# AdamBeedell/MLX8-WS-Audio-Transformer

Measured on AMD Instinct MI355X. Metric: 4s@16kHz clips/sec through mel+Whisper-small encoder, higher is better.
Workload: dtype fp16; 1 GPU; int16 PCM [B,64000] in HBM -> Whisper log-mel [B,80,3000] -> Whisper-small encoder -> hidden [B,1500,768] fp32; mode=parity (clip zero-padded to 30 s, as the reference computes), precision=f16f8, fp16_exact_projection_matrices=0 of 48 (found by the library at upload), parallelism=dp1 (clip shards, no data-path collective)

## Files before the change

### include/awt.h

```cpp
#ifndef AWT_H_
#define AWT_H_

#include <stddef.h>
#include <stdint.h>

#ifdef __cplusplus
extern "C" {
#endif

typedef enum awt_status {
  AWT_OK = 0,
  AWT_ERR_INVALID = -1,
  AWT_ERR_HIP = -2,
  AWT_ERR_WORKSPACE = -3,
  AWT_ERR_STATE = -4,
  AWT_ERR_VALUE = -5
} awt_status;

typedef struct awt_ctx awt_ctx;
typedef struct awt_encoder awt_encoder;

const char* awt_last_error(void);
const char* awt_version(void);

int awt_ctx_create(int device, awt_ctx** out);
void awt_ctx_destroy(awt_ctx* c);

size_t awt_logmel_workspace_bytes(int B);
int awt_logmel_whisper(awt_ctx* c, const void* pcm, int pcm_is_i16, int64_t pcm_stride, const int32_t* n_valid,
                       int max_valid, int B, int n_frames_out, float* out, void* workspace, size_t ws_bytes,
                       void* stream);
int awt_logmel_whisper_mels(awt_ctx* c, const void* pcm, int pcm_is_i16, int64_t pcm_stride, const int32_t* n_valid,
                            int max_valid, int B, int n_frames_out, int n_mels, float* out, void* workspace, size_t ws_bytes,
                            void* stream);
int awt_logmel_whisper_signal(awt_ctx* c, const void* pcm, int pcm_is_i16, int64_t pcm_stride, const int32_t* n_valid,
                              int max_valid, int B, int n_signal, int n_mels, float* out, void* workspace, size_t ws_bytes,
                              void* stream);

int awt_logmel_generic(awt_ctx* c, const float* pcm, int64_t pcm_stride, int B, int n_samples, int sample_rate,
                       int n_fft, int hop, int n_mels, float f_min, float f_max, float log_eps, float* out,
                       void* stream);

int awt_logmel_prepare(awt_ctx* c, int n_fft, int n_mels, float f_min, float f_max, int sample_rate, int slaney);
int awt_resample_prepare(awt_ctx* c, int sr_in, int sr_out);
int64_t awt_resampled_length(int n_in, int sr_in, int sr_out);
int awt_prepare_waveform(awt_ctx* c, const void* pcm, int pcm_is_i16, int channels, int64_t channel_stride,
                         int64_t sample_stride, int n_in, int sr_in, int sr_out, float* out, int n_out, void* stream);

typedef struct awt_encoder_cfg {
  int32_t d_model;
  int32_t n_layers;
  int32_t n_heads;
  int32_t ffn_dim;
  int32_t n_mels;
  int32_t n_ctx;
  int32_t mfma_terms;
  int32_t lora_rank;
  float lora_alpha;
  uint32_t lora_targets;
  int32_t chunk_clips;
  int32_t training;
  int32_t backward_terms;
  int32_t train_base;
} awt_encoder_cfg;

enum { AWT_LORA_Q = 1, AWT_LORA_K = 2, AWT_LORA_V = 4, AWT_LORA_OUT = 8, AWT_LORA_FC1 = 16, AWT_LORA_FC2 = 32 };

int awt_encoder_create(awt_ctx* c, const awt_encoder_cfg* cfg, awt_encoder** out);
void awt_encoder_destroy(awt_encoder* e);

int awt_encoder_set_weight(awt_encoder* e, const char* hf_name, const float* data, const int64_t* shape, int rank,
                           void* stream);

int awt_encoder_exact16_matrices(const awt_encoder* e, int* n_exact, int* n_total);

size_t awt_encoder_workspace_bytes(const awt_encoder* e, int B);

int awt_encoder_forward(awt_encoder* e, const float* input_features, int B, int n_frames, float* last_hidden_state,
                        void* workspace, size_t ws_bytes, void* stream);

int awt_encoder_set_grad_scale_log2(awt_encoder* e, int k);
size_t awt_encoder_train_workspace_bytes(const awt_encoder* e, int B);
size_t awt_encoder_lora_grad_count(const awt_encoder* e);
int awt_encoder_forward_train(awt_encoder* e, const float* input_features, int B, int n_frames, float* last_hidden_state,
                              void* saved, size_t saved_bytes, void* stream);
int awt_encoder_backward(awt_encoder* e, const float* d_last_hidden_state, int B, void* saved, size_t saved_bytes,
                         float* lora_grads, size_t n_grads, void* stream);
enum { AWT_BWD_ACCUMULATE = 1, AWT_BWD_ALLREDUCE = 2 };
int awt_encoder_backward_ex(awt_encoder* e, const float* d_last_hidden_state, int B, void* saved, size_t saved_bytes,
                            float* lora_grads, size_t n_grads, uint32_t flags, void* stream);

size_t awt_encoder_base_grad_count(const awt_encoder* e);
int awt_encoder_base_grad_params(const awt_encoder* e);
int awt_encoder_base_grad_param(const awt_encoder* e, int index, const char** name, size_t* offset, int64_t* shape , int* rank);

typedef struct awt_comm awt_comm;
enum { AWT_COMM_ID_BYTES = 128 };
int awt_comm_unique_id(void* id_out );
int awt_comm_create(awt_ctx* c, const void* id , int rank, int world, awt_comm** out);
void awt_comm_destroy(awt_comm* m);
int awt_comm_world(const awt_comm* m);
int awt_allreduce_sum_f32(awt_comm* m, float* buf, size_t n, void* stream);
int awt_allreduce_mean_f32(awt_comm* m, float* buf, size_t n, void* stream);
int awt_comm_bucket_stats(awt_comm* m, int enable, double* ms, int64_t* bytes, int max, int* n_out);
int awt_encoder_set_comm(awt_encoder* e, awt_comm* m, int groups);

size_t awt_audio_encode_workspace_bytes(const awt_encoder* e, int B);
int awt_audio_encode(awt_encoder* e, const void* pcm, int pcm_is_i16, int64_t pcm_stride, const int32_t* n_valid,
                     int max_valid, int B, float* input_features_out, float* last_hidden_state, void* workspace,
                     size_t ws_bytes, void* stream);

int awt_op_linear(awt_ctx* c, const float* x , const float* w , const float* bias ,
                  float* y , int M, int N, int K, int terms, void* workspace, size_t ws_bytes, void* stream);
size_t awt_op_linear_workspace_bytes(int M, int N, int K);
int awt_op_layernorm(awt_ctx* c, const float* x , const float* gamma, const float* beta, float* y, int M, int d,
                     float eps, void* stream);
int awt_op_attention(awt_ctx* c, const float* q, const float* k, const float* v, float* o, int B, int H, int S,
                     int terms, void* workspace, size_t ws_bytes, void* stream);
size_t awt_op_attention_workspace_bytes(int B, int H, int S);

typedef struct awt_weight awt_weight;
int awt_weight_create(awt_ctx* c, const float* w, const float* bias, int N, int K, int precision, int with_transpose, void* stream,
                      awt_weight** out);
void awt_weight_destroy(awt_weight* w);
int awt_weight_padded_rows(const awt_weight* w);
size_t awt_linear_workspace_bytes(const awt_weight* w, int M, int backward);
int awt_linear_forward(awt_ctx* c, const awt_weight* w, const float* x, const float* resid, float* y, int M, void* workspace,
                       size_t ws_bytes, void* stream);
int awt_linear_backward_input(awt_ctx* c, const awt_weight* w, const float* dy, float* dx, int M, void* workspace, size_t ws_bytes,
                              void* stream);
size_t awt_bmm_packed_bytes(int batch, int N, int K);
int awt_bmm_pack(awt_ctx* c, const float* b, int64_t ldb, int64_t stride_b, int batch, int N, int K, void* packed, size_t packed_bytes, void* stream);
size_t awt_bmm_workspace_bytes(int batch, int M, int K);
int awt_bmm(awt_ctx* c, const float* a, int64_t lda, int64_t stride_a, const void* packed_b, const float* resid, float* out, int64_t ldo,
            int64_t stride_o, int batch, int M, int N, int K, void* workspace, size_t ws_bytes, void* stream);
int awt_bmm_pack_kmajor(awt_ctx* c, const float* b1, const float* b2, int K1, int64_t ldb, int64_t stride_b, int batch, int N, int K, void* packed,
                        size_t packed_bytes, void* stream);
int awt_bmm_kmajor(awt_ctx* c, const float* a1, const float* a2, int K1, int64_t lda, int64_t stride_a, const void* packed_b, const float* resid, float* out,
                   int64_t ldo, int64_t stride_o, int batch, int M, int N, int K, void* workspace, size_t ws_bytes, void* stream);
int awt_op_softmax_rows(awt_ctx* c, const float* s, float* p, int rows, int cols, int64_t ld, float scale, void* stream);
int awt_op_softmax_rows_backward(awt_ctx* c, const float* p, const float* dp, float* ds, int rows, int cols, int64_t ld, float scale, void* stream);
int awt_op_embed(awt_ctx* c, const int64_t* ids, const float* tok, const float* pos, float* x, int M, int L, int d, int pos0, int vocab,
                 void* stream);
int awt_op_gelu(awt_ctx* c, const float* x, float* y, int64_t n, void* stream);
int awt_op_gelu_backward(awt_ctx* c, const float* x, const float* dy, float* dx, int64_t n, void* stream);
int awt_op_layernorm_backward(awt_ctx* c, const float* dy, const float* x, const float* gamma, const float* dres, float* dx, int M, int d,
                              float eps, void* stream);
size_t awt_op_param_grad_workspace_bytes(int M, int d);
int awt_op_layernorm_param_grad(awt_ctx* c, const float* dy, const float* x, float* dgamma, float* dbeta, int M, int d, float eps,
                                void* workspace, size_t ws_bytes, void* stream);
int awt_op_column_sums(awt_ctx* c, const float* a, float* sums, int M, int d, void* workspace, size_t ws_bytes, void* stream);
size_t awt_op_weight_grad_workspace_bytes(int M, int rows_x, int ldy, int ldx, int N, int K);
int awt_op_weight_grad(awt_ctx* c, const float* dy, int ldy, int ycol, int N, const float* x, int rows_x, int ldx, int xcol, int K, int M,
                       int rows_out, int rows_in, int row_mul, int row_add, int terms, float scale, int accumulate, float* out, int64_t sn,
                       int64_t sk, void* workspace, size_t ws_bytes, void* stream);
int awt_op_cross_entropy(awt_ctx* c, const float* logits, const int64_t* labels, int M, int vocab, int ld, float* loss, float* dlogits,
                         void* scratch, void* stream);
int awt_op_attention_small(awt_ctx* c, const float* q, int ldq, const float* k, int ldk, const float* v, int ldv, float* o, int ldo,
                           float* lse, int B, int H, int Lq, int Sk, int causal, int causal_off, void* stream);
int awt_op_attention_small_backward(awt_ctx* c, const float* q, int ldq, const float* k, int ldk, const float* v, int ldv, const float* o,
                                    const float* dout, int ldo, const float* lse, float* delta, float* dq, float* dk, float* dv, int B,
                                    int H, int Lq, int Sk, int causal, int causal_off, void* stream);
int awt_op_attention_small_dropout(awt_ctx* c, const float* q, int ldq, const float* k, int ldk, const float* v, int ldv, float* o, int ldo,
                                   float* lse, int B, int H, int Lq, int Sk, int causal, int causal_off, float drop_p, uint64_t seed, void* stream);
int awt_op_attention_small_backward_dropout(awt_ctx* c, const float* q, int ldq, const float* k, int ldk, const float* v, int ldv, const float* o,
                                            const float* dout, int ldo, const float* lse, float* delta, float* dq, float* dk, float* dv, int B,
                                            int H, int Lq, int Sk, int causal, int causal_off, float drop_p, uint64_t seed, void* stream);

int awt_op_attention_cached(awt_ctx* c, const float* q, int ldq, const float* k, const float* v, int ldkv, int64_t kv_batch_stride, float* o,
                            int ldo, int B, int H, int Lq, int T, void* stream);
size_t awt_select_tokens_workspace_bytes(int rows, int vocab, int k);
int awt_op_select_tokens(awt_ctx* c, const float* logits, int ld, int rows, int vocab, int beams, const uint32_t* banned, const float* beam_scores,
                         int log_softmax, int k, float* top_scores, int64_t* top_tokens, int32_t* top_parent, void* workspace, size_t ws_bytes,
                         void* stream);
typedef struct awt_ts_rules {
  const int64_t* history;
  int64_t hist_ld;
  int begin, cur_len;
  int eos_token_id, no_timestamps_token_id;
  int max_initial_timestamp_index;
} awt_ts_rules;
size_t awt_select_tokens_ts_workspace_bytes(int rows, int vocab, int k);
int awt_op_select_tokens_ts(awt_ctx* c, const float* logits, int ld, int rows, int vocab, int beams, const uint32_t* banned, const float* beam_scores,
                            int log_softmax, int k, const awt_ts_rules* rules, float* top_scores, int64_t* top_tokens, int32_t* top_parent,
                            void* workspace, size_t ws_bytes, void* stream);
int awt_op_kv_gather(awt_ctx* c, const float* src, float* dst, const int32_t* parent, int layers, int src_rows, int dst_rows, int T, int Tmax,
                     int width, void* stream);

int awt_op_alignment_weights(awt_ctx* c, const float* q, int n_slots, int rows, int Tmax, int d, int group, const float* cross_kv, int n_layers,
                             int S, const int32_t* heads, int n_sel, const int32_t* src_row, int clips, int t0, int T, float* out, int frames,
                             void* stream);
int awt_op_alignment_matrix(awt_ctx* c, const float* weights, int clips, int n_sel, int T, int frames, const int32_t* num_frames, int width,
                            float* out, void* stream);
size_t awt_dtw_workspace_bytes(int clips, int T, int frames);
int awt_op_dtw(awt_ctx* c, const float* matrix, int clips, int T, int frames, const int32_t* num_frames, int negate, int32_t* jump_frame,
               int32_t* text_idx, int32_t* time_idx, int32_t* path_start, void* workspace, size_t ws_bytes, void* stream);

int awt_tuning_set(const char* key, int value);

enum { AWT_PROF_LOGMEL = 0, AWT_PROF_GEMM = 1, AWT_PROF_ATTENTION = 2, AWT_PROF_LAYERNORM = 3, AWT_PROF_OTHER = 4,
       AWT_PROF_ATTENTION_BWD = 5,
       AWT_PROF_WGRAD = 6,
       AWT_PROF_NCLASSES = 7 };
int awt_prof_enable(awt_ctx* c, int mask);
int awt_prof_collect(awt_ctx* c, int klass, double* total_ms, int64_t* launches, double* flops);

#ifdef __cplusplus
}
#endif
#endif
```

### mlx8-ws-audio-transformer_amd/_lib.py

```python
from __future__ import annotations

import ctypes as C
import os
import re
import threading
from typing import Optional

import torch

HERE = os.path.dirname(os.path.abspath(__file__))
LIB_PATH = os.environ.get("AWT_LIB") or os.path.join(HERE, "libawt.so")
HEADER_PATH = os.path.join(os.path.dirname(HERE), "include", "awt.h")

AWT_OK = 0
AWT_ERR_VALUE = -5


class AwtError(RuntimeError):
    def __init__(self, code: int, msg: str):
        super().__init__(f"libawt error {code}: {msg}")
        self.code = code
        self.msg = msg


class EncoderCfg(C.Structure):
    _fields_ = [("d_model", C.c_int32), ("n_layers", C.c_int32), ("n_heads", C.c_int32), ("ffn_dim", C.c_int32),
                ("n_mels", C.c_int32), ("n_ctx", C.c_int32), ("mfma_terms", C.c_int32), ("lora_rank", C.c_int32),
                ("lora_alpha", C.c_float), ("lora_targets", C.c_uint32), ("chunk_clips", C.c_int32), ("training", C.c_int32), ("backward_terms", C.c_int32),
                ("train_base", C.c_int32)]


MFMA_PER_PAIR = {"bf16": 1, "fp16": 1, "bf16x3": 3, "fp16x3": 3, "f16f8": 2}
BWD_ACCUMULATE, BWD_ALLREDUCE = 1, 2
COMM_ID_BYTES = 128
LORA_BITS = {"q_proj": 1, "k_proj": 2, "v_proj": 4, "out_proj": 8, "fc1": 16, "fc2": 32}
PROF_CLASSES = {"logmel": 0, "gemm": 1, "attention": 2, "layernorm": 3, "other": 4, "attention_bwd": 5,
                "wgrad": 6}

_vp, _i, _i64, _sz, _f = C.c_void_p, C.c_int, C.c_int64, C.c_size_t, C.c_float
_SIGNATURES = {
    "awt_last_error": (C.c_char_p, []),
    "awt_version": (C.c_char_p, []),
    "awt_ctx_create": (_i, [_i, C.POINTER(_vp)]),
    "awt_ctx_destroy": (None, [_vp]),
    "awt_logmel_workspace_bytes": (_sz, [_i]),
    "awt_logmel_whisper": (_i, [_vp, _vp, _i, _i64, _vp, _i, _i, _i, _vp, _vp, _sz, _vp]),
    "awt_logmel_whisper_mels": (_i, [_vp, _vp, _i, _i64, _vp, _i, _i, _i, _i, _vp, _vp, _sz, _vp]),
    "awt_logmel_whisper_signal": (_i, [_vp, _vp, _i, _i64, _vp, _i, _i, _i, _i, _vp, _vp, _sz, _vp]),
    "awt_logmel_generic": (_i, [_vp, _vp, _i64, _i, _i, _i, _i, _i, _i, _f, _f, _f, _vp, _vp]),
    "awt_logmel_prepare": (_i, [_vp, _i, _i, _f, _f, _i, _i]),
    "awt_resample_prepare": (_i, [_vp, _i, _i]),
    "awt_resampled_length": (_i64, [_i, _i, _i]),
    "awt_prepare_waveform": (_i, [_vp, _vp, _i, _i, _i64, _i64, _i, _i, _i, _vp, _i, _vp]),
    "awt_encoder_create": (_i, [_vp, C.POINTER(EncoderCfg), C.POINTER(_vp)]),
    "awt_encoder_destroy": (None, [_vp]),
    "awt_encoder_set_weight": (_i, [_vp, C.c_char_p, _vp, C.POINTER(_i64), _i, _vp]),
    "awt_encoder_exact16_matrices": (_i, [_vp, C.POINTER(_i), C.POINTER(_i)]),
    "awt_encoder_workspace_bytes": (_sz, [_vp, _i]),
    "awt_encoder_forward": (_i, [_vp, _vp, _i, _i, _vp, _vp, _sz, _vp]),
    "awt_encoder_train_workspace_bytes": (_sz, [_vp, _i]),
    "awt_encoder_lora_grad_count": (_sz, [_vp]),
    "awt_encoder_base_grad_count": (_sz, [_vp]),
    "awt_encoder_base_grad_params": (_i, [_vp]),
    "awt_encoder_base_grad_param": (_i, [_vp, _i, C.POINTER(C.c_char_p), C.POINTER(_sz), C.POINTER(_i64), C.POINTER(_i)]),
    "awt_encoder_forward_train": (_i, [_vp, _vp, _i, _i, _vp, _vp, _sz, _vp]),
    "awt_encoder_backward": (_i, [_vp, _vp, _i, _vp, _sz, _vp, _sz, _vp]),
    "awt_encoder_backward_ex": (_i, [_vp, _vp, _i, _vp, _sz, _vp, _sz, C.c_uint32, _vp]),
    "awt_comm_unique_id": (_i, [_vp]),
    "awt_comm_create": (_i, [_vp, _vp, _i, _i, C.POINTER(_vp)]),
    "awt_comm_destroy": (None, [_vp]),
    "awt_comm_world": (_i, [_vp]),
    "awt_allreduce_sum_f32": (_i, [_vp, _vp, _sz, _vp]),
    "awt_allreduce_mean_f32": (_i, [_vp, _vp, _sz, _vp]),
    "awt_comm_bucket_stats": (_i, [_vp, _i, C.POINTER(C.c_double), C.POINTER(C.c_int64), _i, C.POINTER(_i)]),
    "awt_encoder_set_comm": (_i, [_vp, _vp, _i]),
    "awt_audio_encode_workspace_bytes": (_sz, [_vp, _i]),
    "awt_audio_encode": (_i, [_vp, _vp, _i, _i64, _vp, _i, _i, _vp, _vp, _vp, _sz, _vp]),
    "awt_op_linear": (_i, [_vp, _vp, _vp, _vp, _vp, _i, _i, _i, _i, _vp, _sz, _vp]),
    "awt_op_linear_workspace_bytes": (_sz, [_i, _i, _i]),
    "awt_op_layernorm": (_i, [_vp, _vp, _vp, _vp, _vp, _i, _i, _f, _vp]),
    "awt_op_attention": (_i, [_vp, _vp, _vp, _vp, _vp, _i, _i, _i, _i, _vp, _sz, _vp]),
    "awt_op_attention_workspace_bytes": (_sz, [_i, _i, _i]),
    "awt_weight_create": (_i, [_vp, _vp, _vp, _i, _i, _i, _i, _vp, C.POINTER(_vp)]),
    "awt_weight_destroy": (None, [_vp]),
    "awt_weight_padded_rows": (_i, [_vp]),
    "awt_linear_workspace_bytes": (_sz, [_vp, _i, _i]),
    "awt_linear_forward": (_i, [_vp, _vp, _vp, _vp, _vp, _i, _vp, _sz, _vp]),
    "awt_linear_backward_input": (_i, [_vp, _vp, _vp, _vp, _i, _vp, _sz, _vp]),
    "awt_encoder_set_grad_scale_log2": (_i, [_vp, _i]),
    "awt_bmm_packed_bytes": (_sz, [_i, _i, _i]),
    "awt_bmm_pack": (_i, [_vp, _vp, _i64, _i64, _i, _i, _i, _vp, _sz, _vp]),
    "awt_bmm_workspace_bytes": (_sz, [_i, _i, _i]),
    "awt_bmm": (_i, [_vp, _vp, _i64, _i64, _vp, _vp, _vp, _i64, _i64, _i, _i, _i, _i, _vp, _sz, _vp]),
    "awt_bmm_pack_kmajor": (_i, [_vp, _vp, _vp, _i, _i64, _i64, _i, _i, _i, _vp, _sz, _vp]),
    "awt_bmm_kmajor": (_i, [_vp, _vp, _vp, _i, _i64, _i64, _vp, _vp, _vp, _i64, _i64, _i, _i, _i, _i, _vp, _sz, _vp]),
    "awt_op_softmax_rows": (_i, [_vp, _vp, _vp, _i, _i, _i64, _f, _vp]),
    "awt_op_softmax_rows_backward": (_i, [_vp, _vp, _vp, _vp, _i, _i, _i64, _f, _vp]),
    "awt_op_embed": (_i, [_vp, _vp, _vp, _vp, _vp, _i, _i, _i, _i, _i, _vp]),
    "awt_op_gelu": (_i, [_vp, _vp, _vp, _i64, _vp]),
    "awt_op_gelu_backward": (_i, [_vp, _vp, _vp, _vp, _i64, _vp]),
    "awt_op_layernorm_backward": (_i, [_vp, _vp, _vp, _vp, _vp, _vp, _i, _i, _f, _vp]),
    "awt_op_param_grad_workspace_bytes": (_sz, [_i, _i]),
    "awt_op_layernorm_param_grad": (_i, [_vp, _vp, _vp, _vp, _vp, _i, _i, _f, _vp, _sz, _vp]),
    "awt_op_column_sums": (_i, [_vp, _vp, _vp, _i, _i, _vp, _sz, _vp]),
    "awt_op_weight_grad_workspace_bytes": (_sz, [_i, _i, _i, _i, _i, _i]),
    "awt_op_weight_grad": (_i, [_vp, _vp, _i, _i, _i, _vp, _i, _i, _i, _i, _i, _i, _i, _i, _i, _i, _f, _i, _vp, _i64, _i64, _vp, _sz, _vp]),
    "awt_op_cross_entropy": (_i, [_vp, _vp, _vp, _i, _i, _i, _vp, _vp, _vp, _vp]),
    "awt_op_attention_small": (_i, [_vp, _vp, _i, _vp, _i, _vp, _i, _vp, _i, _vp, _i, _i, _i, _i, _i, _i, _vp]),
    "awt_op_attention_small_backward": (_i, [_vp, _vp, _i, _vp, _i, _vp, _i, _vp, _vp, _i, _vp, _vp, _vp, _vp, _vp, _i, _i, _i, _i, _i, _i, _vp]),
    "awt_op_attention_small_dropout": (_i, [_vp, _vp, _i, _vp, _i, _vp, _i, _vp, _i, _vp, _i, _i, _i, _i, _i, _i, C.c_float, C.c_uint64, _vp]),
    "awt_op_attention_small_backward_dropout": (_i, [_vp, _vp, _i, _vp, _i, _vp, _i, _vp, _vp, _i, _vp, _vp, _vp, _vp, _vp, _i, _i, _i, _i, _i, _i, C.c_float, C.c_uint64, _vp]),
    "awt_op_attention_cached": (_i, [_vp, _vp, _i, _vp, _vp, _i, _i64, _vp, _i, _i, _i, _i, _i, _vp]),
    "awt_select_tokens_workspace_bytes": (_sz, [_i, _i, _i]),
    "awt_op_select_tokens": (_i, [_vp, _vp, _i, _i, _i, _i, _vp, _vp, _i, _i, _vp, _vp, _vp, _vp, _sz, _vp]),
    "awt_select_tokens_ts_workspace_bytes": (_sz, [_i, _i, _i]),
    "awt_op_select_tokens_ts": (_i, [_vp, _vp, _i, _i, _i, _i, _vp, _vp, _i, _i, _vp, _vp, _vp, _vp, _vp, _sz, _vp]),
    "awt_op_kv_gather": (_i, [_vp, _vp, _vp, _vp, _i, _i, _i, _i, _i, _i, _vp]),
    "awt_op_alignment_weights": (_i, [_vp, _vp, _i, _i, _i, _i, _i, _vp, _i, _i, _vp, _i, _vp, _i, _i, _i, _vp, _i, _vp]),
    "awt_op_alignment_matrix": (_i, [_vp, _vp, _i, _i, _i, _i, _vp, _i, _vp, _vp]),
    "awt_dtw_workspace_bytes": (_sz, [_i, _i, _i]),
    "awt_op_dtw": (_i, [_vp, _vp, _i, _i, _i, _vp, _i, _vp, _vp, _vp, _vp, _vp, _sz, _vp]),
    "awt_tuning_set": (_i, [C.c_char_p, _i]),
    "awt_prof_enable": (_i, [_vp, _i]),
    "awt_prof_collect": (_i, [_vp, _i, C.POINTER(C.c_double), C.POINTER(_i64), C.POINTER(C.c_double)]),
}

_lib = None
_lock = threading.Lock()
_ctx = {}


def declared_symbols() -> list:
    text = open(HEADER_PATH).read()
    text = re.sub(r"/\*.*?\*/", "", text, flags=re.S)
    return sorted(set(re.findall(r"\b(awt_[a-z0-9_]+)\s*\(", text)))


def lib() -> C.CDLL:
    global _lib
    with _lock:
        if _lib is None:
            if not os.path.exists(LIB_PATH):
                raise ImportError(f"{LIB_PATH} is missing: run `python -m mlx8_ws_audio_transformer_amd.build` "
                                  "(there is no CPU fallback for this path)")
            l = C.CDLL(LIB_PATH)
            for name, (res, args) in _SIGNATURES.items():
                fn = getattr(l, name)
                fn.restype = res
                fn.argtypes = args
            _lib = l
    return _lib


def check(rc: int) -> None:
    if rc != AWT_OK:
        msg = lib().awt_last_error().decode("utf-8", "replace")
        if rc == AWT_ERR_VALUE:
            raise ValueError(msg)
        raise AwtError(rc, msg)


def ctx(device: Optional[torch.device] = None) -> int:
    if not torch.cuda.is_available():
        raise RuntimeError("mlx8_ws_audio_transformer_amd needs an MI355X (gfx950) GPU: torch.cuda.is_available() is False "
                           "and this package has no CPU fallback")
    idx = torch.cuda.current_device() if device is None or device.index is None else device.index
    with _lock:
        h = _ctx.get(idx)
    if h is None:
        out = _vp()
        check(lib().awt_ctx_create(idx, C.byref(out)))
        with _lock:
            _ctx[idx] = out.value
        h = out.value
    return h


def ptr(t: Optional[torch.Tensor]) -> Optional[int]:
    if t is None:
        return None
    if not t.is_cuda or not t.is_contiguous():
        raise ValueError("libawt needs contiguous device tensors")
    return t.data_ptr()


def stream_handle() -> int:
    return torch.cuda.current_stream().cuda_stream


def workspace(nbytes: int, device) -> torch.Tensor:
    return torch.empty(max(int(nbytes), 256), dtype=torch.uint8, device=device)


def prof_enable(on, classes=None) -> None:
    mask = 0
    if on:
        for k in (classes or [c for c in PROF_CLASSES if c != "wgrad"]):
            mask |= 1 << PROF_CLASSES[k]
    check(lib().awt_prof_enable(ctx(), mask))


def prof_collect(klass: str):
    ms, n, fl = C.c_double(), _i64(), C.c_double()
    check(lib().awt_prof_collect(ctx(), PROF_CLASSES[klass], C.byref(ms), C.byref(n), C.byref(fl)))
    return ms.value, n.value, fl.value


def tuning_set(key: str, value: int) -> None:
    check(lib().awt_tuning_set(key.encode(), int(value)))
```

### mlx8-ws-audio-transformer_amd/csrc/awt_api.hip

```cpp
#include <string.h>
#include <algorithm>
#include <string>
#include <vector>

#include "common.h"
#include "comm.h"
#include "wgrad.h"

static thread_local std::string g_err;
void awt_set_error(const std::string& msg) { g_err = msg; }
int awt_fail(int code, const std::string& msg) { g_err = msg; return code; }
extern "C" const char* awt_last_error(void) { return g_err.c_str(); }
extern "C" const char* awt_version(void) { return "awt 0.1 (gfx950)"; }

struct awt_prof_state {
  struct Span { hipEvent_t a, b; };
  std::vector<Span> spans[AWT_PROF_NCLASSES];
  std::vector<Span> pool;
  double flops[AWT_PROF_NCLASSES] = {};
  Span open[AWT_PROF_NCLASSES];
};

void awt_prof_begin(awt_ctx* c, int klass, hipStream_t s, double flops) {
  awt_prof_state* p = c->prof;
  awt_prof_state::Span sp;
  if (!p->pool.empty()) { sp = p->pool.back(); p->pool.pop_back(); }
  else { (void)hipEventCreate(&sp.a); (void)hipEventCreate(&sp.b); }
  (void)hipEventRecord(sp.a, s);
  p->open[klass] = sp;
  p->flops[klass] += flops;
}
void awt_prof_end(awt_ctx* c, int klass, hipStream_t s) {
  awt_prof_state* p = c->prof;
  (void)hipEventRecord(p->open[klass].b, s);
  p->spans[klass].push_back(p->open[klass]);
}

static int g_pp_mask = 12;
extern "C" int awt_tuning_set(const char* key, int value) {
  AWT_REQUIRE(key, AWT_ERR_INVALID, "tuning_set: null key");
  if (!strcmp(key, "gemm_tile")) {
    AWT_REQUIRE(value == 0 || value == 64 || value == 128 || value == 256, AWT_ERR_INVALID, "tuning_set: gemm_tile must be 0 (auto), 64, 128 or 256");
    awt_gemm_force_tile(value);
    return AWT_OK;
  }
  if (!strcmp(key, "gemm_gm")) {
    AWT_REQUIRE(value >= 0 && value <= 64, AWT_ERR_INVALID, "tuning_set: gemm_gm must be 0 (default) .. 64");
    awt_gemm_set_gm(value);
    return AWT_OK;
  }
  if (!strcmp(key, "gemm_pp")) {
    AWT_REQUIRE(value >= 0 && value <= 2, AWT_ERR_INVALID, "tuning_set: gemm_pp must be 0 (off), 1 (automatic, default) or 2 (wherever supported)");
    awt_gemm_set_pp_mode(value);
    return AWT_OK;
  }
  if (!strcmp(key, "gemm_pp_mask")) {
    AWT_REQUIRE(value >= 0 && value <= 15, AWT_ERR_INVALID, "tuning_set: gemm_pp_mask is a bit set 0 .. 15 (1 qkv, 2 out_proj, 4 fc1, 8 fc2; fc2 only together with fc1)");
    g_pp_mask = value;
    return AWT_OK;
  }
  if (!strcmp(key, "gemm_mfma16")) {
    AWT_REQUIRE(value == 0 || value == 1, AWT_ERR_INVALID, "tuning_set: gemm_mfma16 must be 1 (default: the f16f8 GEMM's 16 x 16 MFMA form where it applies) or 0 (32 x 32 only)");
    awt_gemm_set_mfma16(value);
    return AWT_OK;
  }
  if (!strcmp(key, "attn_shape")) {
    AWT_REQUIRE(value == 0 || (value >= 4 && value <= 6), AWT_ERR_INVALID, "tuning_set: attn_shape must be 0 (auto), 4, 5 or 6");
    awt_attn_force_shape(value);
    return AWT_OK;
  }
  if (!strcmp(key, "attn_qt")) {
    AWT_REQUIRE(value >= 0 && value <= 2, AWT_ERR_INVALID, "tuning_set: attn_qt must be 0 (auto), 1 or 2");
    awt_attn_force_qt(value);
    return AWT_OK;
  }
  AWT_REQUIRE(false, AWT_ERR_INVALID, "tuning_set: unknown key");
}

extern "C" int awt_prof_enable(awt_ctx* c, int on) {
  AWT_REQUIRE(c, AWT_ERR_INVALID, "prof_enable: null ctx");
  if (!c->prof) c->prof = new awt_prof_state();
  c->prof_on = on;
  return AWT_OK;
}
extern "C" int awt_prof_collect(awt_ctx* c, int klass, double* total_ms, int64_t* launches, double* flops) {
  AWT_REQUIRE(c && c->prof && klass >= 0 && klass < AWT_PROF_NCLASSES, AWT_ERR_INVALID, "prof_collect: bad argument");
  awt_prof_state* p = c->prof;
  double ms = 0;
  for (auto& sp : p->spans[klass]) {
    AWT_HIP_CHECK(hipEventSynchronize(sp.b));
    float t = 0;
    AWT_HIP_CHECK(hipEventElapsedTime(&t, sp.a, sp.b));
    ms += t;
    p->pool.push_back(sp);
  }
  if (total_ms) *total_ms = ms;
  if (launches) *launches = (int64_t)p->spans[klass].size();
  if (flops) *flops = p->flops[klass];
  p->spans[klass].clear();
  p->flops[klass] = 0;
  return AWT_OK;
}

extern "C" int awt_ctx_create(int device, awt_ctx** out) {
  AWT_REQUIRE(out, AWT_ERR_INVALID, "ctx_create: null out");
  int n = 0;
  AWT_HIP_CHECK(hipGetDeviceCount(&n));
  AWT_REQUIRE(device >= 0 && device < n, AWT_ERR_INVALID, "ctx_create: no such device");
  AWT_HIP_CHECK(hipSetDevice(device));
  hipDeviceProp_t prop;
  AWT_HIP_CHECK(hipGetDeviceProperties(&prop, device));
  AWT_REQUIRE(strncmp(prop.gcnArchName, "gfx950", 6) == 0, AWT_ERR_INVALID,
              std::string("libawt is built for gfx950 (MI355X) only; device is ") + prop.gcnArchName);
  awt_ctx* c = new awt_ctx();
  c->device = device;
  if (hipMalloc(&c->zeros, 256) != hipSuccess || hipMemset(c->zeros, 0, 256) != hipSuccess) {
    delete c;
    AWT_REQUIRE(false, AWT_ERR_HIP, "ctx_create: could not allocate the zero page");
  }
  int rc = logmel_prepare_impl(c, 400, 80, 0.0, 8000.0, 16000, 1);
  if (!rc) rc = logmel_prepare_impl(c, 400, 128, 0.0, 8000.0, 16000, 1);
  if (rc) { awt_ctx_destroy(c); return rc; }
  *out = c;
  return AWT_OK;
}
extern "C" int awt_logmel_prepare(awt_ctx* c, int n_fft, int n_mels, float f_min, float f_max, int sample_rate, int slaney) {
  return logmel_prepare_impl(c, n_fft, n_mels, (double)f_min, (double)f_max, sample_rate, slaney);
}
extern "C" int awt_resample_prepare(awt_ctx* c, int sr_in, int sr_out) { return resample_prepare_impl(c, sr_in, sr_out); }
extern "C" void awt_ctx_destroy(awt_ctx* c) {
  if (!c) return;
  awt_free_tables(c);
  if (c->zeros) (void)hipFree(c->zeros);
  if (c->prof) {
    for (int k = 0; k < AWT_PROF_NCLASSES; ++k)
      for (auto& sp : c->prof->spans[k]) { (void)hipEventDestroy(sp.a); (void)hipEventDestroy(sp.b); }
    for (auto& sp : c->prof->pool) { (void)hipEventDestroy(sp.a); (void)hipEventDestroy(sp.b); }
    delete c->prof;
  }
  delete c;
}

extern "C" int awt_logmel_whisper(awt_ctx* c, const void* pcm, int pcm_is_i16, int64_t pcm_stride, const int32_t* n_valid,
                                  int max_valid, int B, int n_frames_out, float* out, void* workspace, size_t ws_bytes,
                                  void* stream) {
  return logmel_whisper_impl(c, pcm, pcm_is_i16, pcm_stride, n_valid, max_valid, B, n_frames_out, 80, out, workspace, ws_bytes,
                             (hipStream_t)stream);
}
extern "C" int awt_logmel_whisper_mels(awt_ctx* c, const void* pcm, int pcm_is_i16, int64_t pcm_stride, const int32_t* n_valid,
                                       int max_valid, int B, int n_frames_out, int n_mels, float* out, void* workspace, size_t ws_bytes,
                                       void* stream) {
  return logmel_whisper_impl(c, pcm, pcm_is_i16, pcm_stride, n_valid, max_valid, B, n_frames_out, n_mels, out, workspace, ws_bytes,
                             (hipStream_t)stream);
}
extern "C" int awt_logmel_whisper_signal(awt_ctx* c, const void* pcm, int pcm_is_i16, int64_t pcm_stride, const int32_t* n_valid,
                                         int max_valid, int B, int n_signal, int n_mels, float* out, void* workspace, size_t ws_bytes,
                                         void* stream) {
  return logmel_whisper_impl(c, pcm, pcm_is_i16, pcm_stride, n_valid, max_valid, B, 0, n_mels, out, workspace, ws_bytes, (hipStream_t)stream,
                             n_signal);
}
extern "C" int awt_logmel_generic(awt_ctx* c, const float* pcm, int64_t pcm_stride, int B, int n_samples, int sample_rate,
                                  int n_fft, int hop, int n_mels, float f_min, float f_max, float log_eps, float* out,
                                  void* stream) {
  return logmel_generic_impl(c, pcm, pcm_stride, B, n_samples, sample_rate, n_fft, hop, n_mels, f_min, f_max, log_eps, out,
                             (hipStream_t)stream);
}

extern "C" int64_t awt_resampled_length(int n_in, int sr_in, int sr_out) {
  if (n_in <= 0 || sr_in <= 0 || sr_out <= 0) return 0;
  return resampled_length(n_in, sr_in, sr_out);
}
extern "C" int awt_prepare_waveform(awt_ctx* c, const void* pcm, int pcm_is_i16, int channels, int64_t channel_stride,
                                    int64_t sample_stride, int n_in, int sr_in, int sr_out, float* out, int n_out, void* stream) {
  return prepare_waveform_impl(c, pcm, pcm_is_i16, channels, channel_stride, sample_stride, n_in, sr_in, sr_out, out, n_out,
                               (hipStream_t)stream);
}

namespace {

struct Planes {
  bf16_t* hi = nullptr; bf16_t* lo = nullptr; uint8_t* x8 = nullptr; int64_t rows = 0, ld = 0;
  int* d_inexact = nullptr; bool exact16 = false;
  int64_t s_rows = 0;
  bf16_t* s16 = nullptr; uint8_t* s8 = nullptr;
  char* pp = nullptr;
};
struct Linear {
  Planes w; float* bias = nullptr; int N = 0, K = 0;
};
struct LoraGroup {
  bool active = false;
  Planes a;
  Planes b;
  Planes bT;
  Planes aT;
  int kp = 0;
};
struct Layer {
  Linear qkv, out, fc1, fc2;
  Planes qkvT, outT, fc1T, fc2T;
  Planes fc1T8, fc2T8;
  Planes fc1_8, fc2_8;
  float *ln1_g = nullptr, *ln1_b = nullptr, *ln2_g = nullptr, *ln2_b = nullptr;
  LoraGroup lq, lo_, l1, l2;
};

int conv1_k(int n_mels) { return (3 * n_mels + 63) / 64 * 64; }
constexpr size_t kAlign = 256;
size_t align_up(size_t x) { return (x + kAlign - 1) & ~(kAlign - 1); }

}

struct awt_encoder {
  awt_ctx* ctx = nullptr;
  awt_encoder_cfg cfg{};
  int planes = 1;
  int prec = PREC_BF16X3;
  Linear conv1, conv2;
  float* pos = nullptr;
  float *lnf_g = nullptr, *lnf_b = nullptr;
  std::vector<Layer> layers;
  std::vector<void*> allocs;
  std::vector<std::string> seen;
  int chunk = 16;
  awt_comm* comm = nullptr;
  int comm_groups = 2;
  bool mlp_f8 = false;
  float* wt_tmp = nullptr;
  int grad_scale_log2 = 0;
  bool train_base = false;
  Planes conv2T[3];
  struct GradEntry { std::string name; size_t offset; int64_t shape[3]; int rank; };
  std::vector<GradEntry> glayout;
  size_t g_head = 0, g_per_layer = 0;
};

namespace {

int dev_alloc(awt_encoder* e, void** p, size_t bytes) {
  AWT_HIP_CHECK(hipMalloc(p, bytes));
  AWT_HIP_CHECK(hipMemset(*p, 0, bytes));
  e->allocs.push_back(*p);
  return AWT_OK;
}
int alloc_planes(awt_encoder* e, Planes* pl, int64_t rows, int64_t ld) {
  pl->rows = rows; pl->ld = ld;
  int rc = dev_alloc(e, (void**)&pl->hi, (size_t)rows * ld * 2); if (rc) return rc;
  if (e->planes == 2) { rc = dev_alloc(e, (void**)&pl->lo, (size_t)rows * ld * 2); if (rc) return rc; }
  if (e->prec == PREC_F16F8) {
    pl->x8 = (uint8_t*)pl->lo + (size_t)rows * ld;
    pl->s_rows = (rows + 255) / 256 * 256;
    rc = dev_alloc(e, (void**)&pl->s16, (size_t)pl->s_rows * ld * 2); if (rc) return rc;
    rc = dev_alloc(e, (void**)&pl->s8, (size_t)pl->s_rows * ld * 2); if (rc) return rc;
  }
  return AWT_OK;
}
int alloc_planes_f8(awt_encoder* e, Planes* pl, int64_t rows, int64_t ld) {
  pl->rows = rows; pl->ld = ld;
  int rc = dev_alloc(e, (void**)&pl->hi, (size_t)rows * ld * 2); if (rc) return rc;
  rc = dev_alloc(e, (void**)&pl->lo, (size_t)rows * ld * 2); if (rc) return rc;
  pl->x8 = (uint8_t*)pl->lo + (size_t)rows * ld;
  pl->s_rows = (rows + 255) / 256 * 256;
  rc = dev_alloc(e, (void**)&pl->s16, (size_t)pl->s_rows * ld * 2); if (rc) return rc;
  rc = dev_alloc(e, (void**)&pl->s8, (size_t)pl->s_rows * ld * 2); if (rc) return rc;
  return AWT_OK;
}
int alloc_linear(awt_encoder* e, Linear* l, int N, int K) {
  l->N = N; l->K = K;
  int rc = alloc_planes(e, &l->w, N, K); if (rc) return rc;
  return dev_alloc(e, (void**)&l->bias, (size_t)N * 4);
}
int alloc_lora(awt_encoder* e, LoraGroup* g, int slots, int K_in, int N_out) {
  g->active = true;
  g->kp = (int)(((int64_t)slots * e->cfg.lora_rank + 63) / 64 * 64);
  int rc = alloc_planes(e, &g->a, 128, K_in); if (rc) return rc;
  rc = alloc_planes(e, &g->b, N_out, g->kp); if (rc) return rc;
  if (e->cfg.training) {
    rc = alloc_planes(e, &g->bT, 128, N_out); if (rc) return rc;
    rc = alloc_planes(e, &g->aT, K_in, g->kp); if (rc) return rc;
  }
  return AWT_OK;
}

struct Workspace {
  float* x; bf16_t *ln[2], *qkv[2], *att[2], *ff[2], *u[2], *a1[2], *h1[2];
  size_t bytes;
};

Workspace carve(const awt_encoder* e, char* base, int Bc) {
  const awt_encoder_cfg& c = e->cfg;
  const size_t P = e->planes, S = c.n_ctx, T = 2 * S, d = c.d_model, f = c.ffn_dim;
  const size_t M = (size_t)Bc * S, Mt = (size_t)Bc * T;
  Workspace w{};
  size_t off = 0;
  auto take = [&](size_t bytes) { char* p = base ? base + off : nullptr; off += align_up(bytes); return p; };
  w.x = (float*)take(M * d * 4);
  for (size_t p = 0; p < P; ++p) w.ln[p] = (bf16_t*)take(M * d * 2);
  for (size_t p = 0; p < P; ++p) w.u[p] = (bf16_t*)take(M * 128 * 2);
  const size_t layer_start = off;
  for (size_t p = 0; p < P; ++p) w.qkv[p] = (bf16_t*)take(3 * M * d * 2);
  for (size_t p = 0; p < P; ++p) w.att[p] = (bf16_t*)take(M * d * 2);
  for (size_t p = 0; p < P; ++p) w.ff[p] = (bf16_t*)take(M * f * 2);
  const size_t layer_end = off;
  off = layer_start;
  for (size_t p = 0; p < P; ++p) w.a1[p] = (bf16_t*)take(Mt * conv1_k(c.n_mels) * 2);
  for (size_t p = 0; p < P; ++p) w.h1[p] = (bf16_t*)take(Mt * d * 2);
  w.bytes = std::max(off, layer_end);
  if (e->prec == PREC_F16F8 && !c.training) w.bytes += align_up((size_t)256 * std::max(f, (size_t)conv1_k(c.n_mels)) * 4);
  return w;
}

Act make_act(bf16_t* p0, bf16_t* p1, size_t elems, int prec) {
  Act a;
  a.p16 = p0;
  if (prec == PREC_F16F8) { a.hi8 = (uint8_t*)p1; a.lo8 = a.hi8 ? a.hi8 + elems : nullptr; }
  else a.lo16 = p1;
  return a;
}
Act act_offset(const Act& a, int64_t elems) {
  Act r;
  r.p16 = a.p16 + elems;
  r.lo16 = a.lo16 ? a.lo16 + elems : nullptr;
  r.hi8 = a.hi8 ? a.hi8 + elems : nullptr;
  r.lo8 = a.lo8 ? a.lo8 + elems : nullptr;
  return r;
}
void set_out(GemmOut& o, const Act& a) { o.hi = a.p16; o.lo = a.lo16; o.hi8 = a.hi8; o.lo8 = a.lo8; o.ilv = a.ilv; }
Act make_ilv(bf16_t* p0) { Act a; a.ilv = (char*)p0; return a; }

GemmSeg seg_plain(const Act& a, int64_t lda, const Planes& w, int64_t wcol, int K, int M) {
  GemmSeg s{};
  s.a_hi = a.p16; s.a_lo = a.lo16; s.a8 = a.hi8; s.al8 = a.lo8; s.lda = lda;
  s.w_hi = w.hi; s.w_lo = w.lo; s.w8 = (const uint8_t*)w.lo; s.wl8 = w.x8;
  s.w_ksteps = (int)(w.ld / 32); s.w_k0 = (int)(wcol / 32); s.K = K;
  s.rows_out = M; s.rows_in = M; s.row_mul = 1; s.row_add = 0;
  s.w_exact16 = w.exact16 ? 1 : 0;
  s.a_ilv = a.ilv; s.w_pp = w.pp;
  s.ws16 = w.s16; s.ws8 = w.s8; s.ws_rows = (int)w.s_rows;
  return s;
}
GemmSeg seg_plain(const bf16_t* a_hi, const bf16_t* a_lo, int64_t lda, const Planes& w, int64_t wcol, int K, int M) {
  Act a; a.p16 = const_cast<bf16_t*>(a_hi); a.lo16 = const_cast<bf16_t*>(a_lo);
  return seg_plain(a, lda, w, wcol, K, M);
}

int linear_with_lora(awt_encoder* e, bf16_t* const u[2], bf16_t* const in[2], int64_t ld_in, const Linear& lin, const LoraGroup& lg,
                     int M, GemmEpilogue epi, GemmOut out, hipStream_t s) {
  const int terms = e->prec;
  const Act ain = make_act(in[0], in[1], (size_t)M * ld_in, terms);
  GemmSeg segs[2];
  int nseg = 1;
  segs[0] = seg_plain(ain, ld_in, lin.w, 0, lin.K, M);
  if (lg.active) {
    GemmSeg us = seg_plain(ain, ld_in, lg.a, 0, lin.K, M);
    const Act au = make_act(u[0], u[1], (size_t)M * 128, terms);
    GemmOut uo{};
    set_out(uo, au); uo.ldo = lg.kp; uo.n_valid = lg.kp;
    uo.scale = e->cfg.lora_alpha / (float)e->cfg.lora_rank;
    int rc = launch_gemm(e->ctx, M, 128, &us, 1, terms, EPI_BF16, uo, s); if (rc) return rc;
    segs[1] = seg_plain(au, lg.kp, lg.b, 0, lg.kp, M);
    nseg = 2;
  }
  out.bias = lin.bias;
  out.n_valid = lin.N;
  return launch_gemm(e->ctx, M, lin.N, segs, nseg, terms, epi, out, s);
}

int linear_pp(awt_encoder* e, bf16_t* in0, const Linear& lin, int M, GemmEpilogue epi, GemmOut out, hipStream_t s) {
  GemmSeg sg = seg_plain(make_ilv(in0), lin.K, lin.w, 0, lin.K, M);
  out.bias = lin.bias;
  out.n_valid = lin.N;
  return launch_gemm_pp(e->ctx, M, lin.N, sg, epi, out, s);
}
bool use_pp(const awt_encoder* e, const Linear& lin, const LoraGroup& lg, int M, int epi) {
  const int mode = awt_gemm_pp_mode();
  if (mode == 0 || e->prec != PREC_F16F8 || !lin.w.pp || lg.active || !gemm_pp_supported(M, lin.N, lin.K, epi)) return false;
  if (mode == 2) return true;
  const int64_t t = (int64_t)((M + 255) / 256) * (lin.N / 256), c = gemm_pp_slots();
  return !lin.w.exact16 && c > 0 && t >= c && ((t + c - 1) / c) * c * 5 <= t * 6;
}

struct LayerBufs {
  float *x_in, *x_mid, *x_out;
  bf16_t *ln1[2], *qkv[2], *att[2], *ln2[2], *pre[2], *ff[2], *u[2];
  bf16_t *uo[2], *u1[2], *u2[2];
  float* lse;
};

struct TrainWs {
  std::vector<LayerBufs> layer;
  bf16_t *a1[2], *h1[2], *ff[2];
  bf16_t* pre1[2];
  float* x_final;
  float *dx_a, *dx_b, *dln, *delta, *partial;
  bf16_t *dxp[2], *dpre[2], *datt[2], *dqkv[2], *du[2];
  size_t partial_bytes, bytes;
};

TrainWs carve_train(const awt_encoder* e, char* base, int B) {
  const awt_encoder_cfg& c = e->cfg;
  const size_t P = e->planes, S = c.n_ctx, T = 2 * S, d = c.d_model, f = c.ffn_dim, H = c.n_heads;
  const size_t M = (size_t)B * S, Mt = (size_t)B * T;
  TrainWs w{};
  size_t off = 0;
  auto take = [&](size_t bytes) { char* p = base ? base + off : nullptr; off += align_up(bytes); return p; };
  auto planes = [&](bf16_t* (&dst)[2], size_t elems) { dst[0] = dst[1] = nullptr; for (size_t p = 0; p < P; ++p) dst[p] = (bf16_t*)take(elems * 2); };
  w.layer.resize(c.n_layers);
  float* x = (float*)take(M * d * 4);
  for (int li = 0; li < c.n_layers; ++li) {
    LayerBufs& L = w.layer[li];
    L.x_in = x;
    L.x_mid = (float*)take(M * d * 4);
    L.x_out = (float*)take(M * d * 4);
    x = L.x_out;
    planes(L.ln1, M * d); planes(L.qkv, 3 * M * d); planes(L.att, M * d); planes(L.ln2, M * d); planes(L.pre, M * f);
    planes(L.u, M * 128);
    const bool has_o = e->layers[li].lo_.active, has_1 = e->layers[li].l1.active, has_2 = e->layers[li].l2.active;
    if (has_o) planes(L.uo, M * 128); else { L.uo[0] = L.u[0]; L.uo[1] = L.u[1]; }
    if (has_1) planes(L.u1, M * 128); else { L.u1[0] = L.u[0]; L.u1[1] = L.u[1]; }
    if (has_2) { planes(L.u2, M * 128); planes(L.ff, M * f); } else { L.u2[0] = L.u[0]; L.u2[1] = L.u[1]; L.ff[0] = L.ff[1] = nullptr; }
    if (e->train_base) planes(L.ff, M * f);
    L.lse = (float*)take((size_t)B * H * S * 4);
  }
  w.x_final = x;
  if (e->train_base) w.ff[0] = w.ff[1] = nullptr;
  else planes(w.ff, M * f);
  w.pre1[0] = w.pre1[1] = nullptr;
  if (e->train_base) { planes(w.a1, Mt * conv1_k(e->cfg.n_mels)); planes(w.h1, Mt * d); planes(w.pre1, Mt * d); }
  const size_t mark = off;
  if (!e->train_base) { planes(w.a1, Mt * conv1_k(e->cfg.n_mels)); planes(w.h1, Mt * d); }
  const size_t conv_end = off;
  off = mark;
  w.dx_a = (float*)take(M * d * 4); w.dx_b = (float*)take(M * d * 4); w.dln = (float*)take(M * d * 4);
  w.delta = (float*)take((size_t)B * H * S * 4);
  planes(w.dxp, M * d); planes(w.dpre, M * f); planes(w.datt, M * d); planes(w.dqkv, 3 * M * d); planes(w.du, M * 128);
  w.partial_bytes = outer_reduce_partial_bytes((int)M, c.lora_rank > 0 ? c.lora_rank : 1, 1024);
  if (e->train_base) {
    const int Mi = (int)M, Mti = (int)Mt, di = (int)d, fi = (int)f;
    size_t pb = std::max({wgrad_partial_bytes(Mi, 3 * di, di), wgrad_partial_bytes(Mi, di, di), wgrad_partial_bytes(Mi, fi, di), wgrad_partial_bytes(Mi, di, fi),
                          wgrad_partial_bytes(Mti, di, c.n_mels), param_grad_partial_bytes(Mti, di)});
    w.partial_bytes = std::max(w.partial_bytes, pb);
  }
  w.partial = (float*)take(w.partial_bytes);
  w.bytes = std::max(off, conv_end);
  for (int li = 0; li < c.n_layers; ++li) for (int p = 0; p < 2; ++p) if (!w.layer[li].ff[p]) w.layer[li].ff[p] = w.ff[p];
  return w;
}

int conv_stem(awt_encoder* e, const float* mel, int Bc, bf16_t* const a1[2], bf16_t* const h1[2], float* x, hipStream_t s, bf16_t* const* pre1 = nullptr) {
  const awt_encoder_cfg& c = e->cfg;
  const int S = c.n_ctx, T = 2 * S, d = c.d_model, terms = e->prec;
  const int M = Bc * S, Mt = Bc * T;
  const int k1 = conv1_k(c.n_mels);
  const Act aa1 = make_act(a1[0], a1[1], (size_t)Mt * k1, terms), ah1 = make_act(h1[0], h1[1], (size_t)Mt * d, terms);
  int rc = launch_im2col_conv1(e->ctx, mel, Bc, c.n_mels, T, k1, aa1, terms, s); if (rc) return rc;
  {
    GemmSeg sg = seg_plain(aa1, k1, e->conv1.w, 0, k1, Mt);
    GemmOut o{}; set_out(o, ah1); o.ldo = d; o.bias = e->conv1.bias; o.n_valid = d;
    if (pre1) { o.hi2 = pre1[0]; o.lo2 = pre1[1]; }
    rc = launch_gemm(e->ctx, Mt, d, &sg, 1, terms, pre1 ? EPI_BF16_GELU_SAVE : EPI_BF16_GELU, o, s); if (rc) return rc;
  }
  GemmSeg sg[3];
  for (int dt = 0; dt < 3; ++dt) {
    sg[dt] = seg_plain(ah1, d, e->conv2.w, (int64_t)dt * d, d, M);
    sg[dt].rows_out = S; sg[dt].rows_in = T; sg[dt].row_mul = 2; sg[dt].row_add = dt - 1;
  }
  GemmOut o{}; o.f32 = x; o.ldo = d; o.bias = e->conv2.bias; o.n_valid = d; o.pos = e->pos; o.rows_pos = S;
  return launch_gemm(e->ctx, M, d, sg, 3, terms, EPI_F32_GELU_POS, o, s);
}

int encoder_layer(awt_encoder* e, Layer& L, const LayerBufs& b, int Bc, bool save, hipStream_t s) {
  const awt_encoder_cfg& c = e->cfg;
  const int S = c.n_ctx, d = c.d_model, f = c.ffn_dim, H = c.n_heads, terms = e->prec;
  const int M = Bc * S;
  const int64_t plane = (int64_t)M * d;
  const bool pp_qkv = !save && (g_pp_mask & 1) && use_pp(e, L.qkv, L.lq, M, EPI_QKV), pp_out = !save && (g_pp_mask & 2) && use_pp(e, L.out, L.lo_, M, EPI_F32_RESID);
  const bool pp_fc1 = !save && (g_pp_mask & 4) && use_pp(e, L.fc1, L.l1, M, EPI_BF16_GELU), pp_fc2 = pp_fc1 && (g_pp_mask & 8) && use_pp(e, L.fc2, L.l2, M, EPI_F32_RESID);
  auto feeds = [&](Act a, const Linear& lin, const LoraGroup& lg) { if (terms == PREC_F16F8 && lin.w.exact16 && !lg.active) a.hi8 = nullptr; return a; };
  const Act aqkv = make_act(b.qkv[0], b.qkv[1], 3 * (size_t)plane, terms);
  const Act aatt = pp_out ? make_ilv(b.att[0]) : feeds(make_act(b.att[0], b.att[1], (size_t)plane, terms), L.out, L.lo_);
  int rc = launch_layernorm(e->ctx, b.x_in, L.ln1_g, L.ln1_b, M, d, 1e-5f, nullptr,
                            pp_qkv ? make_ilv(b.ln1[0]) : feeds(make_act(b.ln1[0], b.ln1[1], (size_t)plane, terms), L.qkv, L.lq), terms, s); if (rc) return rc;
  {
    GemmOut o{}; set_out(o, aqkv); o.scale = 0.125f * 1.4426950408889634f;
    o.S = S; o.H = H; o.plane_stride = plane;
    o.skip_v8 = terms == PREC_F16F8 && !attention_f16f8_reads_v8(save);
    rc = pp_qkv ? linear_pp(e, b.ln1[0], L.qkv, M, EPI_QKV, o, s) : linear_with_lora(e, b.u, b.ln1, d, L.qkv, L.lq, M, EPI_QKV, o, s);
    if (rc) return rc;
  }
  if (terms == PREC_F16F8) {
    const Act ak = act_offset(aqkv, plane), av = act_offset(aqkv, 2 * plane);
    rc = launch_attention_f16f8(e->ctx, F8Planes{aqkv.p16, aqkv.hi8, aqkv.lo8}, F8Planes{ak.p16, ak.hi8, ak.lo8}, F8Planes{av.p16, av.hi8, av.lo8},
                                F8Planes{aatt.p16, aatt.hi8, aatt.lo8}, nullptr, save ? b.lse : nullptr, Bc, H, S, s, aatt.ilv);
  } else {
    rc = launch_attention(e->ctx, b.qkv[0], b.qkv[1], b.qkv[0] + plane, b.qkv[1] ? b.qkv[1] + plane : nullptr, b.qkv[0] + 2 * plane,
                          b.qkv[1] ? b.qkv[1] + 2 * plane : nullptr, b.att[0], b.att[1], nullptr, save ? b.lse : nullptr, Bc, H, S, terms, s);
  }
  if (rc) return rc;
  {
    GemmOut o{}; o.f32 = b.x_mid; o.resid = b.x_in; o.ldo = d;
    rc = pp_out ? linear_pp(e, b.att[0], L.out, M, EPI_F32_RESID, o, s) : linear_with_lora(e, b.uo, b.att, d, L.out, L.lo_, M, EPI_F32_RESID, o, s);
    if (rc) return rc;
  }
  if (save && e->mlp_f8) {
    const Act aln2 = make_act(b.ln2[0], b.ln2[1], (size_t)plane, PREC_F16F8), aff = make_act(b.ff[0], b.ff[1], (size_t)M * f, PREC_F16F8);
    rc = launch_layernorm(e->ctx, b.x_mid, L.ln2_g, L.ln2_b, M, d, 1e-5f, nullptr, aln2, PREC_F16F8, s); if (rc) return rc;
    GemmSeg s1 = seg_plain(aln2, d, L.fc1_8, 0, d, M);
    GemmOut o1{}; set_out(o1, aff); o1.ldo = f; o1.n_valid = f; o1.bias = L.fc1.bias; o1.hi2 = b.pre[0]; o1.lo2 = b.pre[1]; o1.scale = 1.0f;
    rc = launch_gemm(e->ctx, M, f, &s1, 1, PREC_F16F8, EPI_BF16_GELU_SAVE, o1, s); if (rc) return rc;
    GemmSeg s2 = seg_plain(aff, f, L.fc2_8, 0, f, M);
    GemmOut o2{}; o2.f32 = b.x_out; o2.resid = b.x_mid; o2.ldo = d; o2.n_valid = d; o2.bias = L.fc2.bias;
    return launch_gemm(e->ctx, M, d, &s2, 1, PREC_F16F8, EPI_F32_RESID, o2, s);
  }
  rc = launch_layernorm(e->ctx, b.x_mid, L.ln2_g, L.ln2_b, M, d, 1e-5f, nullptr,
                        pp_fc1 ? make_ilv(b.ln2[0]) : feeds(make_act(b.ln2[0], b.ln2[1], (size_t)plane, terms), L.fc1, L.l1), terms, s); if (rc) return rc;
  {
    GemmOut o{}; set_out(o, pp_fc2 ? make_ilv(b.ff[0]) : feeds(make_act(b.ff[0], b.ff[1], (size_t)M * f, terms), L.fc2, L.l2)); o.ldo = f; o.hi2 = b.pre[0]; o.lo2 = b.pre[1];
    rc = pp_fc1 ? linear_pp(e, b.ln2[0], L.fc1, M, EPI_BF16_GELU, o, s)
                : linear_with_lora(e, b.u1, b.ln2, d, L.fc1, L.l1, M, save ? EPI_BF16_GELU_SAVE : EPI_BF16_GELU, o, s);
    if (rc) return rc;
  }
  GemmOut o{}; o.f32 = b.x_out; o.resid = b.x_mid; o.ldo = d;
  return pp_fc2 ? linear_pp(e, b.ff[0], L.fc2, M, EPI_F32_RESID, o, s) : linear_with_lora(e, b.u2, b.ff, f, L.fc2, L.l2, M, EPI_F32_RESID, o, s);
}

int forward_chunk(awt_encoder* e, const float* mel, int Bc, float* hidden, char* ws_base, hipStream_t s) {
  const awt_encoder_cfg& c = e->cfg;
  const int M = Bc * c.n_ctx, d = c.d_model;
  const bool two = e->planes == 2;
  Workspace w = carve(e, ws_base, Bc);
  bf16_t* a1[2] = {w.a1[0], two ? w.a1[1] : nullptr};
  bf16_t* h1[2] = {w.h1[0], two ? w.h1[1] : nullptr};
  int rc = conv_stem(e, mel, Bc, a1, h1, w.x, s); if (rc) return rc;
  LayerBufs b{};
  b.x_in = b.x_mid = b.x_out = w.x;
  for (int p = 0; p < 2; ++p) {
    const bool on = p == 0 || two;
    b.ln1[p] = b.ln2[p] = on ? w.ln[p] : nullptr; b.qkv[p] = on ? w.qkv[p] : nullptr; b.att[p] = on ? w.att[p] : nullptr;
    b.ff[p] = on ? w.ff[p] : nullptr; b.u[p] = b.uo[p] = b.u1[p] = b.u2[p] = on ? w.u[p] : nullptr; b.pre[p] = nullptr;
  }
  for (int li = 0; li < c.n_layers; ++li) { rc = encoder_layer(e, e->layers[li], b, Bc, false, s); if (rc) return rc; }
  return launch_layernorm(e->ctx, w.x, e->lnf_g, e->lnf_b, M, d, 1e-5f, hidden, Act{}, e->prec, s);
}

bool parse_layer(const char* name, int* idx, const char** rest) {
  if (strncmp(name, "layers.", 7) != 0) return false;
  char* end = nullptr;
  long v = strtol(name + 7, &end, 10);
  if (end == name + 7 || *end != '.') return false;
  *idx = (int)v; *rest = end + 1;
  return true;
}

int check_shape(const char* name, const int64_t* shape, int rank, std::initializer_list<int64_t> want) {
  bool ok = rank == (int)want.size();
  int i = 0;
  for (int64_t w : want) { if (ok && shape[i] != w) ok = false; ++i; }
  if (!ok) {
    std::string m = std::string("set_weight: ") + name + " has shape [";
    for (int j = 0; j < rank; ++j) m += (j ? "," : "") + std::to_string(shape[j]);
    m += "], expected [";
    i = 0;
    for (int64_t w : want) m += (i++ ? "," : "") + std::to_string(w);
    return awt_fail(AWT_ERR_INVALID, m + "]");
  }
  return AWT_OK;
}

int copy_f32(float* dst, const float* src, size_t n, hipStream_t s) {
  AWT_HIP_CHECK(hipMemcpyAsync(dst, src, n * 4, hipMemcpyDeviceToDevice, s));
  return AWT_OK;
}

}

namespace {
void build_grad_layout(awt_encoder* e) {
  const awt_encoder_cfg& c = e->cfg;
  const int64_t d = c.d_model, f = c.ffn_dim;
  size_t off = 0;
  auto add = [&](const std::string& name, std::initializer_list<int64_t> shape) {
    awt_encoder::GradEntry g{name, off, {1, 1, 1}, (int)shape.size()};
    int i = 0; size_t n = 1;
    for (int64_t v : shape) { g.shape[i++] = v; n *= (size_t)v; }
    e->glayout.push_back(g);
    off += n;
  };
  add("conv1.weight", {d, c.n_mels, 3}); add("conv1.bias", {d}); add("conv2.weight", {d, d, 3}); add("conv2.bias", {d});
  add("layer_norm.weight", {d}); add("layer_norm.bias", {d});
  e->g_head = off;
  for (int li = 0; li < c.n_layers; ++li) {
    const std::string p = "layers." + std::to_string(li) + ".";
    add(p + "self_attn.q_proj.weight", {d, d}); add(p + "self_attn.k_proj.weight", {d, d}); add(p + "self_attn.v_proj.weight", {d, d});
    add(p + "self_attn.q_proj.bias", {d}); add(p + "self_attn.v_proj.bias", {d});
    add(p + "self_attn.out_proj.weight", {d, d}); add(p + "self_attn.out_proj.bias", {d});
    add(p + "self_attn_layer_norm.weight", {d}); add(p + "self_attn_layer_norm.bias", {d});
    add(p + "fc1.weight", {f, d}); add(p + "fc1.bias", {f}); add(p + "fc2.weight", {d, f}); add(p + "fc2.bias", {d});
    add(p + "final_layer_norm.weight", {d}); add(p + "final_layer_norm.bias", {d});
    if (li == 0) e->g_per_layer = off - e->g_head;
  }
}
}

extern "C" size_t awt_encoder_base_grad_count(const awt_encoder* e) {
  if (!e || !e->train_base) return 0;
  return e->g_head + (size_t)e->cfg.n_layers * e->g_per_layer;
}
extern "C" int awt_encoder_base_grad_params(const awt_encoder* e) { return (e && e->train_base) ? (int)e->glayout.size() : 0; }
extern "C" int awt_encoder_base_grad_param(const awt_encoder* e, int index, const char** name, size_t* offset, int64_t* shape, int* rank) {
  AWT_REQUIRE(e && e->train_base, AWT_ERR_STATE, "encoder_base_grad_param: encoder was not created with cfg.train_base");
  AWT_REQUIRE(index >= 0 && index < (int)e->glayout.size() && name && offset && shape && rank, AWT_ERR_INVALID, "encoder_base_grad_param: bad argument");
  const awt_encoder::GradEntry& g = e->glayout[index];
  *name = g.name.c_str(); *offset = g.offset; *rank = g.rank;
  for (int i = 0; i < 3; ++i) shape[i] = g.shape[i];
  return AWT_OK;
}

extern "C" int awt_encoder_create(awt_ctx* c, const awt_encoder_cfg* cfg, awt_encoder** out) {
  AWT_REQUIRE(c && cfg && out, AWT_ERR_INVALID, "encoder_create: null argument");
  AWT_REQUIRE(cfg->d_model > 0 && cfg->d_model % 128 == 0 && cfg->d_model <= 1280, AWT_ERR_INVALID, "encoder_create: d_model must be a multiple of 128, <= 1280");
  AWT_REQUIRE(cfg->n_heads > 0 && cfg->d_model == cfg->n_heads * 64, AWT_ERR_INVALID, "encoder_create: head_dim (d_model / n_heads) must be 64");
  AWT_REQUIRE(cfg->ffn_dim > 0 && cfg->ffn_dim % 128 == 0, AWT_ERR_INVALID, "encoder_create: ffn_dim must be a multiple of 128");
  AWT_REQUIRE(cfg->n_mels > 0 && cfg->n_mels % 8 == 0 && cfg->n_mels <= 128, AWT_ERR_INVALID, "encoder_create: n_mels must be a multiple of 8, <= 128");
  AWT_REQUIRE(cfg->n_layers > 0 && cfg->n_ctx > 0, AWT_ERR_INVALID, "encoder_create: n_layers and n_ctx must be positive");
  AWT_REQUIRE(prec_known(cfg->mfma_terms), AWT_ERR_INVALID,
              "encoder_create: mfma_terms must be 1 (bf16), 2 (fp16), 3 (bf16x3), 4 (fp16x3) or 5 (f16f8)");
  AWT_REQUIRE(!cfg->training || cfg->mfma_terms == PREC_BF16 || cfg->mfma_terms == PREC_BF16X3, AWT_ERR_INVALID,
              "encoder_create: training keeps its activations as bf16 planes: mfma_terms must be 1 or 3 (gradients do not fit fp16's range unscaled)");
  AWT_REQUIRE(cfg->backward_terms == 0 || cfg->backward_terms == cfg->mfma_terms || ((cfg->backward_terms == 1 || cfg->backward_terms == PREC_F16F8) && cfg->mfma_terms == 3),
              AWT_ERR_INVALID, "encoder_create: backward_terms must be 0 (= mfma_terms), mfma_terms, 1, or 5 (f16f8 MLP backward) with mfma_terms = 3");
  AWT_REQUIRE(cfg->backward_terms != PREC_F16F8 || (cfg->training && !(cfg->lora_targets & (AWT_LORA_FC1 | AWT_LORA_FC2))), AWT_ERR_INVALID,
              "encoder_create: backward_terms = 5 runs the MLP's backward GEMMs in f16f8: training mode, and no adapters on fc1 / fc2");
  AWT_REQUIRE(cfg->lora_rank >= 0 && cfg->lora_rank <= 32, AWT_ERR_INVALID, "encoder_create: lora_rank must be in 0..32");
  AWT_REQUIRE(cfg->lora_rank == 0 || cfg->lora_targets != 0, AWT_ERR_INVALID, "encoder_create: lora_rank > 0 needs lora_targets");
  AWT_REQUIRE(!cfg->training || cfg->lora_rank > 0 || cfg->train_base, AWT_ERR_INVALID, "encoder_create: training mode needs adapters (lora_rank > 0) or train_base");
  AWT_REQUIRE(!cfg->train_base || cfg->training, AWT_ERR_INVALID, "encoder_create: train_base needs training mode");
  AWT_REQUIRE(!cfg->train_base || cfg->lora_rank == 0, AWT_ERR_INVALID, "encoder_create: train_base trains the base weights themselves: no adapters in this mode (lora_rank must be 0)");
  AWT_REQUIRE(!cfg->train_base || cfg->backward_terms != PREC_F16F8, AWT_ERR_INVALID,
              "encoder_create: train_base forms its weight gradients from bf16 planes: backward_terms = 5 (f16f8 MLP backward) is not available in this mode");
  awt_encoder* e = new awt_encoder();
  e->ctx = c; e->cfg = *cfg; e->prec = cfg->mfma_terms; e->planes = (cfg->mfma_terms == PREC_BF16 || cfg->mfma_terms == PREC_F16) ? 1 : 2;
  e->chunk = cfg->chunk_clips > 0 ? cfg->chunk_clips : 64;
  e->mlp_f8 = cfg->backward_terms == PREC_F16F8;
  e->train_base = cfg->train_base != 0;
  const int d = cfg->d_model, f = cfg->ffn_dim;
  int rc = alloc_linear(e, &e->conv1, d, conv1_k(cfg->n_mels));
  if (!rc && e->mlp_f8) rc = dev_alloc(e, (void**)&e->wt_tmp, (size_t)f * d * 4);
  if (!rc && e->train_base) rc = dev_alloc(e, (void**)&e->wt_tmp, (size_t)d * d * 4);
  for (int dt = 0; dt < 3 && !rc && e->train_base; ++dt) rc = alloc_planes(e, &e->conv2T[dt], d, d);
  if (!rc) rc = alloc_linear(e, &e->conv2, d, 3 * d);
  if (!rc) rc = dev_alloc(e, (void**)&e->pos, (size_t)cfg->n_ctx * d * 4);
  if (!rc) rc = dev_alloc(e, (void**)&e->lnf_g, (size_t)d * 4);
  if (!rc) rc = dev_alloc(e, (void**)&e->lnf_b, (size_t)d * 4);
  e->layers.resize(cfg->n_layers);
  const bool lora = cfg->lora_rank > 0;
  for (int i = 0; i < cfg->n_layers && !rc; ++i) {
    Layer& L = e->layers[i];
    rc = alloc_linear(e, &L.qkv, 3 * d, d);
    if (!rc) rc = alloc_linear(e, &L.out, d, d);
    if (!rc) rc = alloc_linear(e, &L.fc1, f, d);
    if (!rc) rc = alloc_linear(e, &L.fc2, d, f);
    if ((e->prec == PREC_F16F8 || e->prec == PREC_F16X3) && !cfg->training)
      for (Linear* lin : {&L.qkv, &L.out, &L.fc1, &L.fc2}) if (!rc) rc = dev_alloc(e, (void**)&lin->w.d_inexact, 4 * sizeof(int));
    if (e->prec == PREC_F16F8 && !cfg->training)
      for (Linear* lin : {&L.qkv, &L.out, &L.fc1, &L.fc2})
        if (!rc && lin->N % 256 == 0 && lin->K % 64 == 0 && lin->K >= 128) rc = dev_alloc(e, (void**)&lin->w.pp, gemm_pp_weight_bytes(lin->N, lin->K));
    if (cfg->training) {
      if (!rc) rc = alloc_planes(e, &L.qkvT, d, 3 * d);
      if (!rc) rc = alloc_planes(e, &L.outT, d, d);
      if (!rc) rc = alloc_planes(e, &L.fc1T, d, f);
      if (!rc) rc = alloc_planes(e, &L.fc2T, f, d);
      if (!rc && e->mlp_f8) rc = alloc_planes_f8(e, &L.fc1T8, d, f);
      if (!rc && e->mlp_f8) rc = alloc_planes_f8(e, &L.fc2T8, f, d);
      if (!rc && e->mlp_f8) rc = alloc_planes_f8(e, &L.fc1_8, f, d);
      if (!rc && e->mlp_f8) rc = alloc_planes_f8(e, &L.fc2_8, d, f);
    }
    float** lnp[4] = {&L.ln1_g, &L.ln1_b, &L.ln2_g, &L.ln2_b};
    for (int k = 0; k < 4 && !rc; ++k) rc = dev_alloc(e, (void**)lnp[k], (size_t)d * 4);
    if (lora && !rc && (cfg->lora_targets & (AWT_LORA_Q | AWT_LORA_K | AWT_LORA_V))) rc = alloc_lora(e, &L.lq, 3, d, 3 * d);
    if (lora && !rc && (cfg->lora_targets & AWT_LORA_OUT)) rc = alloc_lora(e, &L.lo_, 1, d, d);
    if (lora && !rc && (cfg->lora_targets & AWT_LORA_FC1)) rc = alloc_lora(e, &L.l1, 1, d, f);
    if (lora && !rc && (cfg->lora_targets & AWT_LORA_FC2)) rc = alloc_lora(e, &L.l2, 1, f, d);
  }
  if (rc) { awt_encoder_destroy(e); return rc; }
  if (e->train_base) build_grad_layout(e);
  *out = e;
  return AWT_OK;
}

extern "C" void awt_encoder_destroy(awt_encoder* e) {
  if (!e) return;
  for (void* p : e->allocs) (void)hipFree(p);
  delete e;
}

extern "C" int awt_encoder_set_weight(awt_encoder* e, const char* name, const float* data, const int64_t* shape, int rank,
                                      void* stream) {
  AWT_REQUIRE(e && name && data && shape && rank >= 1 && rank <= 3, AWT_ERR_INVALID, "set_weight: bad argument");
  hipStream_t s = (hipStream_t)stream;
  const awt_encoder_cfg& c = e->cfg;
  const int d = c.d_model, f = c.ffn_dim, r = c.lora_rank;
  int rc = AWT_ERR_INVALID;
  auto pack = [&](const Planes& pl, int N, int C, int taps, int row_off, int col_off) {
    return launch_pack_weight(e->ctx, data, N, C, taps, pl.ld, row_off, col_off, 1.0f, pl.hi, pl.lo, pl.x8, e->prec, s, nullptr, pl.s16, pl.s8);
  };
  std::string nm(name);
  if (nm == "conv1.weight") { rc = check_shape(name, shape, rank, {d, c.n_mels, 3}); if (!rc) rc = pack(e->conv1.w, d, c.n_mels, 3, 0, 0); }
  else if (nm == "conv1.bias") { rc = check_shape(name, shape, rank, {d}); if (!rc) rc = copy_f32(e->conv1.bias, data, d, s); }
  else if (nm == "conv2.weight") {
    rc = check_shape(name, shape, rank, {d, d, 3}); if (!rc) rc = pack(e->conv2.w, d, d, 3, 0, 0);
    for (int dt = 0; dt < 3 && !rc && e->train_base; ++dt) {
      rc = launch_conv_tap(e->ctx, data, d, d, dt, e->wt_tmp, s);
      if (!rc) rc = launch_pack_weight_t(e->ctx, e->wt_tmp, d, d, e->conv2T[dt].ld, 0, 0, 1.0f, e->conv2T[dt].hi, e->conv2T[dt].lo, s);
    }
  }
  else if (nm == "conv2.bias") { rc = check_shape(name, shape, rank, {d}); if (!rc) rc = copy_f32(e->conv2.bias, data, d, s); }
  else if (nm == "embed_positions.weight") { rc = check_shape(name, shape, rank, {c.n_ctx, d}); if (!rc) rc = copy_f32(e->pos, data, (size_t)c.n_ctx * d, s); }
  else if (nm == "layer_norm.weight") { rc = check_shape(name, shape, rank, {d}); if (!rc) rc = copy_f32(e->lnf_g, data, d, s); }
  else if (nm == "layer_norm.bias") { rc = check_shape(name, shape, rank, {d}); if (!rc) rc = copy_f32(e->lnf_b, data, d, s); }
  else {
    int li = -1; const char* rest = nullptr;
    if (!parse_layer(name, &li, &rest) || li < 0 || li >= c.n_layers)
      return awt_fail(AWT_ERR_INVALID, std::string("set_weight: unknown parameter ") + name);
    Layer& L = e->layers[li];
    std::string rs(rest);
    struct Proj { const char* key; Linear* lin; int row_off; int N; int K; LoraGroup* lg; int slot; uint32_t bit; Planes* wT; Planes* wT8; Planes* w8; };
    Proj projs[] = {
        {"self_attn.q_proj", &L.qkv, 0, d, d, &L.lq, 0, AWT_LORA_Q, &L.qkvT, nullptr, nullptr},   {"self_attn.k_proj", &L.qkv, d, d, d, &L.lq, 1, AWT_LORA_K, &L.qkvT, nullptr, nullptr},
        {"self_attn.v_proj", &L.qkv, 2 * d, d, d, &L.lq, 2, AWT_LORA_V, &L.qkvT, nullptr, nullptr}, {"self_attn.out_proj", &L.out, 0, d, d, &L.lo_, 0, AWT_LORA_OUT, &L.outT, nullptr, nullptr},
        {"fc1", &L.fc1, 0, f, d, &L.l1, 0, AWT_LORA_FC1, &L.fc1T, &L.fc1T8, &L.fc1_8},            {"fc2", &L.fc2, 0, d, f, &L.l2, 0, AWT_LORA_FC2, &L.fc2T, &L.fc2T8, &L.fc2_8}};
    const float lscale = r > 0 ? c.lora_alpha / (float)r : 0.f;
    bool found = false;
    for (const Proj& p : projs) {
      const std::string key(p.key);
      if (rs == key + ".weight") {
        found = true; rc = check_shape(name, shape, rank, {p.N, p.K});
        if (!rc && (e->prec == PREC_F16F8 || e->prec == PREC_F16X3) && !c.training && p.lin->w.d_inexact) {
          Planes& pl = p.lin->w;
          int* flag = pl.d_inexact + p.row_off / p.N;
          int host[4] = {0, 0, 0, 0};
          if (hipMemsetAsync(flag, 0, sizeof(int), s) != hipSuccess) rc = awt_fail(AWT_ERR_HIP, "set_weight: flag reset failed");
          if (!rc) rc = launch_pack_weight(e->ctx, data, p.N, p.K, 1, pl.ld, p.row_off, 0, 1.0f, pl.hi, pl.lo, pl.x8, e->prec, s, flag, pl.s16, pl.s8);
          if (!rc && (hipMemcpyAsync(host, pl.d_inexact, sizeof(host), hipMemcpyDeviceToHost, s) != hipSuccess || hipStreamSynchronize(s) != hipSuccess))
            rc = awt_fail(AWT_ERR_HIP, "set_weight: flag read-back failed");
          if (!rc) pl.exact16 = !(host[0] | host[1] | host[2] | host[3]);
        } else if (!rc) rc = pack(p.lin->w, p.N, p.K, 1, p.row_off, 0);
        if (!rc && p.lin->w.pp) rc = launch_pack_weight_pp(e->ctx, data, p.N, p.K, p.row_off, p.lin->w.pp, s);
        if (!rc && c.training)
          rc = launch_pack_weight_t(e->ctx, data, p.N, p.K, p.wT->ld, 0, p.row_off, 1.0f, p.wT->hi, p.wT->lo, s);
        if (!rc && e->mlp_f8 && p.wT8) {
          rc = launch_transpose_f32(e->ctx, data, p.N, p.K, e->wt_tmp, s);
          if (!rc) rc = launch_pack_weight(e->ctx, e->wt_tmp, p.K, p.N, 1, p.wT8->ld, 0, 0, 1.0f, p.wT8->hi, p.wT8->lo, p.wT8->x8, PREC_F16F8, s, nullptr, p.wT8->s16, p.wT8->s8);
          if (!rc) rc = launch_pack_weight(e->ctx, data, p.N, p.K, 1, p.w8->ld, 0, 0, 1.0f, p.w8->hi, p.w8->lo, p.w8->x8, PREC_F16F8, s, nullptr, p.w8->s16, p.w8->s8);
        }
      }
      else if (rs == key + ".bias") {
        found = true;
        if (key == "self_attn.k_proj") return awt_fail(AWT_ERR_INVALID, "set_weight: k_proj has no bias (HF:modeling_whisper.py:279)");
        rc = check_shape(name, shape, rank, {p.N}); if (!rc) rc = copy_f32(p.lin->bias + p.row_off, data, p.N, s);
      } else if (rs == key + ".lora_A" || rs == key + ".lora_B") {
        found = true;
        if (r == 0 || !(c.lora_targets & p.bit) || !p.lg->active)
          return awt_fail(AWT_ERR_STATE, std::string("set_weight: ") + name + " given but this adapter is not enabled in awt_encoder_cfg");
        if (rs.back() == 'A') {
          rc = check_shape(name, shape, rank, {r, p.K}); if (!rc) rc = pack(p.lg->a, r, p.K, 1, p.slot * r, 0);
          if (!rc && c.training) rc = launch_pack_weight_t(e->ctx, data, r, p.K, p.lg->aT.ld, 0, p.slot * r, lscale, p.lg->aT.hi, p.lg->aT.lo, s);
        } else {
          rc = check_shape(name, shape, rank, {p.N, r}); if (!rc) rc = pack(p.lg->b, p.N, r, 1, p.row_off, p.slot * r);
          if (!rc && c.training) rc = launch_pack_weight_t(e->ctx, data, p.N, r, p.lg->bT.ld, p.slot * r, p.row_off, 1.0f, p.lg->bT.hi, p.lg->bT.lo, s);
        }
      }
      if (found) break;
    }
    if (!found) {
      struct Vec { const char* key; float* dst; };
      Vec vecs[] = {{"self_attn_layer_norm.weight", L.ln1_g}, {"self_attn_layer_norm.bias", L.ln1_b},
                    {"final_layer_norm.weight", L.ln2_g}, {"final_layer_norm.bias", L.ln2_b}};
      for (const Vec& v : vecs)
        if (rs == v.key) { found = true; rc = check_shape(name, shape, rank, {d}); if (!rc) rc = copy_f32(v.dst, data, d, s); break; }
    }
    if (!found) return awt_fail(AWT_ERR_INVALID, std::string("set_weight: unknown parameter ") + name);
  }
  if (rc == AWT_OK && std::find(e->seen.begin(), e->seen.end(), nm) == e->seen.end()) e->seen.push_back(nm);
  return rc;
}

static int require_weights(const awt_encoder* e) {
  size_t base = 0;
  for (const std::string& n : e->seen) if (n.find("lora_") == std::string::npos) ++base;
  const size_t want = 7 + 15 * (size_t)e->cfg.n_layers;
  if (base < want)
    return awt_fail(AWT_ERR_STATE, "encoder: " + std::to_string(base) + " of " + std::to_string(want) + " parameters uploaded; call awt_encoder_set_weight for every state-dict key first");
  return AWT_OK;
}

extern "C" int awt_encoder_exact16_matrices(const awt_encoder* e, int* n_exact, int* n_total) {
  AWT_REQUIRE(e && n_exact && n_total, AWT_ERR_INVALID, "encoder_exact16_matrices: null argument");
  int ex = 0, tot = 0;
  for (const Layer& L : e->layers)
    for (const Linear* lin : {&L.qkv, &L.out, &L.fc1, &L.fc2}) { ++tot; if (lin->w.exact16) ++ex; }
  *n_exact = ex; *n_total = tot;
  return AWT_OK;
}

extern "C" size_t awt_encoder_workspace_bytes(const awt_encoder* e, int B) {
  if (!e || B <= 0) return 0;
  return carve(e, nullptr, std::min(B, e->chunk)).bytes;
}

extern "C" int awt_encoder_forward(awt_encoder* e, const float* mel, int B, int n_frames, float* hidden, void* workspace,
                                   size_t ws_bytes, void* stream) {
  AWT_REQUIRE(e && mel && hidden && workspace && B > 0, AWT_ERR_INVALID, "encoder_forward: bad argument");
  const int T = 2 * e->cfg.n_ctx;
  if (n_frames != T)
    return awt_fail(AWT_ERR_VALUE, "Whisper expects the mel input features to be of length " + std::to_string(T) + ", but found " +
                                       std::to_string(n_frames) + ". Make sure to pad the input mel features to " + std::to_string(T) + ".");
  int rc = require_weights(e); if (rc) return rc;
  AWT_REQUIRE(ws_bytes >= awt_encoder_workspace_bytes(e, B), AWT_ERR_WORKSPACE, "encoder_forward: workspace too small");
  AWT_REQUIRE(((uintptr_t)workspace & 255) == 0 && ((uintptr_t)mel & 15) == 0 && ((uintptr_t)hidden & 15) == 0, AWT_ERR_INVALID,
              "encoder_forward: workspace must be 256-byte aligned, tensors 16-byte aligned");
  hipStream_t s = (hipStream_t)stream;
  for (int b0 = 0; b0 < B; b0 += e->chunk) {
    const int Bc = std::min(e->chunk, B - b0);
    rc = forward_chunk(e, mel + (size_t)b0 * e->cfg.n_mels * T, Bc, hidden + (size_t)b0 * e->cfg.n_ctx * e->cfg.d_model,
                       (char*)workspace, s);
    if (rc) return rc;
  }
  return AWT_OK;
}

extern "C" size_t awt_audio_encode_workspace_bytes(const awt_encoder* e, int B) {
  if (!e || B <= 0) return 0;
  const int Bc = std::min(B, e->chunk);
  return carve(e, nullptr, Bc).bytes + align_up((size_t)Bc * e->cfg.n_mels * 2 * e->cfg.n_ctx * 4) + awt_logmel_workspace_bytes(Bc);
}

extern "C" int awt_audio_encode(awt_encoder* e, const void* pcm, int pcm_is_i16, int64_t pcm_stride, const int32_t* n_valid,
                                int max_valid, int B, float* features_out, float* hidden, void* workspace, size_t ws_bytes,
                                void* stream) {
  AWT_REQUIRE(e && pcm && hidden && workspace && B > 0, AWT_ERR_INVALID, "audio_encode: bad argument");
  AWT_REQUIRE(e->cfg.n_mels == 80 || e->cfg.n_mels == 128, AWT_ERR_INVALID, "audio_encode: the Whisper front-end has 80 or 128 (large-v3) mel bins");
  int rc = require_weights(e); if (rc) return rc;
  AWT_REQUIRE(ws_bytes >= awt_audio_encode_workspace_bytes(e, B), AWT_ERR_WORKSPACE, "audio_encode: workspace too small");
  AWT_REQUIRE(((uintptr_t)workspace & 255) == 0, AWT_ERR_INVALID, "audio_encode: workspace must be 256-byte aligned");
  hipStream_t s = (hipStream_t)stream;
  const int T = 2 * e->cfg.n_ctx;
  const int chunk = std::min(B, e->chunk);
  char* base = (char*)workspace;
  const size_t enc_bytes = carve(e, nullptr, chunk).bytes;
  float* mel_buf = (float*)(base + enc_bytes);
  void* lm_ws = base + enc_bytes + align_up((size_t)chunk * e->cfg.n_mels * T * 4);
  const size_t esz = pcm_is_i16 ? 2 : 4;
  for (int b0 = 0; b0 < B; b0 += chunk) {
    const int Bc = std::min(chunk, B - b0);
    float* mel = features_out ? features_out + (size_t)b0 * e->cfg.n_mels * T : mel_buf;
    rc = logmel_whisper_impl(e->ctx, (const char*)pcm + (size_t)b0 * pcm_stride * esz, pcm_is_i16, pcm_stride,
                             n_valid ? n_valid + b0 : nullptr, max_valid, Bc, T, e->cfg.n_mels, mel, lm_ws, awt_logmel_workspace_bytes(Bc), s);
    if (rc) return rc;
    rc = forward_chunk(e, mel, Bc, hidden + (size_t)b0 * e->cfg.n_ctx * e->cfg.d_model, base, s);
    if (rc) return rc;
  }
  return AWT_OK;
}

extern "C" size_t awt_op_linear_workspace_bytes(int M, int N, int K) {
  const size_t npad = ((size_t)N + 255) / 256 * 256;
  return 2 * align_up((size_t)M * K * 2) + 2 * align_up((size_t)N * K * 2) + 256 + 2 * align_up(npad * K * 2);
}
extern "C" int awt_op_linear(awt_ctx* c, const float* x, const float* w, const float* bias, float* y, int M, int N, int K,
                             int terms, void* workspace, size_t ws_bytes, void* stream) {
  AWT_REQUIRE(prec_known(terms), AWT_ERR_INVALID, "op_linear: terms must be 1 (bf16), 2 (fp16), 3 (bf16x3), 4 (fp16x3) or 5 (f16f8)");
  AWT_REQUIRE(c && x && w && y && workspace, AWT_ERR_INVALID, "op_linear: null argument");
  AWT_REQUIRE(M > 0 && N > 0 && N % 128 == 0 && K > 0 && K % 64 == 0, AWT_ERR_INVALID, "op_linear: N % 128 == 0 and K % 64 == 0 required");
  AWT_REQUIRE(ws_bytes >= awt_op_linear_workspace_bytes(M, N, K), AWT_ERR_WORKSPACE, "op_linear: workspace too small");
  hipStream_t s = (hipStream_t)stream;
  char* base = (char*)workspace;
  bf16_t* xh = (bf16_t*)base;                 base += align_up((size_t)M * K * 2);
  bf16_t* xl = (bf16_t*)base;                 base += align_up((size_t)M * K * 2);
  bf16_t* wh = (bf16_t*)base;                 base += align_up((size_t)N * K * 2);
  bf16_t* wl = (bf16_t*)base;
  if (terms == PREC_F16F8 && awt_gemm_pp_mode() == 2 && gemm_pp_supported(M, N, K, EPI_F32)) {
    Act ai; ai.ilv = (char*)xh;
    int rcp = launch_split_planes(c, x, (int64_t)M * K, 1.0f, terms, kF8Act, nullptr, nullptr, nullptr, nullptr, s, ai.ilv); if (rcp) return rcp;
    if (hipMemsetAsync(wh, 0, gemm_pp_weight_bytes(N, K), s) != hipSuccess) return awt_fail(AWT_ERR_HIP, "op_linear: weight image reset failed");
    rcp = launch_pack_weight_pp(c, w, N, K, 0, (char*)wh, s); if (rcp) return rcp;
    Planes pwp; pwp.pp = (char*)wh; pwp.rows = N; pwp.ld = K;
    GemmSeg sgp = seg_plain(ai, K, pwp, 0, K, M);
    GemmOut op{}; op.f32 = y; op.ldo = N; op.bias = bias; op.n_valid = N;
    return launch_gemm_pp(c, M, N, sgp, EPI_F32, op, s);
  }
  const Act ax = make_act(xh, xl, (size_t)M * K, terms);
  int rc = launch_split_planes(c, x, (int64_t)M * K, 1.0f, terms, kF8Act, xh, xl, ax.hi8, ax.lo8, s); if (rc) return rc;
  Planes pw; pw.hi = wh; pw.lo = wl; pw.x8 = (uint8_t*)wl + (size_t)N * K; pw.rows = N; pw.ld = K;
  if (terms == PREC_F16F8 || terms == PREC_F16X3) {
    int* flag = (int*)((char*)wl + align_up((size_t)N * K * 2));
    int host = 1;
    if (hipMemsetAsync(flag, 0, sizeof(int), s) != hipSuccess) return awt_fail(AWT_ERR_HIP, "op_linear: flag reset failed");
    if (terms == PREC_F16F8) {
      pw.s_rows = ((int64_t)N + 255) / 256 * 256;
      pw.s16 = (bf16_t*)((char*)flag + 256); pw.s8 = (uint8_t*)pw.s16 + align_up((size_t)pw.s_rows * K * 2);
      if (N % 256 != 0) {
        if (hipMemsetAsync(pw.s16, 0, 2 * align_up((size_t)pw.s_rows * K * 2), s) != hipSuccess) return awt_fail(AWT_ERR_HIP, "op_linear: weight copy reset failed");
      }
    }
    rc = launch_pack_weight(c, w, N, K, 1, K, 0, 0, 1.0f, wh, wl, pw.x8, terms, s, flag, pw.s16, pw.s8); if (rc) return rc;
    if (hipMemcpyAsync(&host, flag, sizeof(int), hipMemcpyDeviceToHost, s) != hipSuccess || hipStreamSynchronize(s) != hipSuccess)
      return awt_fail(AWT_ERR_HIP, "op_linear: flag read-back failed");
    pw.exact16 = host == 0;
  } else {
    rc = launch_pack_weight(c, w, N, K, 1, K, 0, 0, 1.0f, wh, wl, pw.x8, terms, s); if (rc) return rc;
  }
  GemmSeg sg = seg_plain(ax, K, pw, 0, K, M);
  GemmOut o{}; o.f32 = y; o.ldo = N; o.bias = bias; o.n_valid = N;
  return launch_gemm(c, M, N, &sg, 1, terms, EPI_F32, o, s);
}

extern "C" int awt_op_layernorm(awt_ctx* c, const float* x, const float* gamma, const float* beta, float* y, int M, int d,
                                float eps, void* stream) {
  return launch_layernorm(c, x, gamma, beta, M, d, eps, y, Act{}, PREC_BF16X3, (hipStream_t)stream);
}

extern "C" size_t awt_op_attention_workspace_bytes(int B, int H, int S) { return 6 * align_up((size_t)B * H * S * 64 * 2); }
extern "C" int awt_op_attention(awt_ctx* c, const float* q, const float* k, const float* v, float* o, int B, int H, int S,
                                int terms, void* workspace, size_t ws_bytes, void* stream) {
  AWT_REQUIRE(prec_known(terms), AWT_ERR_INVALID, "op_attention: terms must be 1 (bf16), 2 (fp16), 3 (bf16x3), 4 (fp16x3) or 5 (f16f8)");
  AWT_REQUIRE(c && q && k && v && o && workspace, AWT_ERR_INVALID, "op_attention: null argument");
  AWT_REQUIRE(ws_bytes >= awt_op_attention_workspace_bytes(B, H, S), AWT_ERR_WORKSPACE, "op_attention: workspace too small");
  hipStream_t s = (hipStream_t)stream;
  const int64_t n = (int64_t)B * H * S * 64;
  const size_t pb = align_up((size_t)n * 2);
  bf16_t* pl[6];
  for (int i = 0; i < 6; ++i) pl[i] = (bf16_t*)((char*)workspace + i * pb);
  const float* src[3] = {q, k, v};
  const int f8exp[3] = {kF8Q, kF8KV, kF8KV};
  for (int i = 0; i < 3; ++i) {
    uint8_t* b8 = (uint8_t*)pl[2 * i + 1];
    int rc = launch_split_planes(c, src[i], n, i == 0 ? 1.4426950408889634f : 1.0f, terms, f8exp[i], pl[2 * i], pl[2 * i + 1], b8, b8 + n, s);
    if (rc) return rc;
  }
  if (terms == PREC_F16F8) {
    F8Planes P[3];
    for (int i = 0; i < 3; ++i) P[i] = F8Planes{pl[2 * i], (uint8_t*)pl[2 * i + 1], (uint8_t*)pl[2 * i + 1] + n};
    return launch_attention_f16f8(c, P[0], P[1], P[2], F8Planes{nullptr, nullptr, nullptr}, o, nullptr, B, H, S, s);
  }
  return launch_attention(c, pl[0], pl[1], pl[2], pl[3], pl[4], pl[5], nullptr, nullptr, o, nullptr, B, H, S, terms, s);
}

extern "C" int awt_encoder_set_grad_scale_log2(awt_encoder* e, int k) {
  AWT_REQUIRE(e && e->cfg.training, AWT_ERR_STATE, "encoder_set_grad_scale_log2: encoder was not created with cfg.training");
  AWT_REQUIRE(k >= -60 && k <= 60, AWT_ERR_INVALID, "encoder_set_grad_scale_log2: k must be in -60 .. 60");
  e->grad_scale_log2 = k;
  return AWT_OK;
}

extern "C" size_t awt_encoder_train_workspace_bytes(const awt_encoder* e, int B) {
  if (!e || B <= 0 || !e->cfg.training) return 0;
  return carve_train(e, nullptr, B).bytes;
}

namespace {
size_t lora_grads_per_layer(const awt_encoder_cfg& c) {
  const size_t r = c.lora_rank, d = c.d_model, f = c.ffn_dim;
  size_t n = 0;
  for (uint32_t bit : {AWT_LORA_Q, AWT_LORA_K, AWT_LORA_V, AWT_LORA_OUT}) if (c.lora_targets & bit) n += 2 * r * d;
  if (c.lora_targets & AWT_LORA_FC1) n += r * d + f * r;
  if (c.lora_targets & AWT_LORA_FC2) n += r * f + d * r;
  return n;
}
}

extern "C" size_t awt_encoder_lora_grad_count(const awt_encoder* e) {
  if (!e || e->cfg.lora_rank <= 0) return 0;
  return (size_t)e->cfg.n_layers * lora_grads_per_layer(e->cfg);
}

extern "C" int awt_encoder_forward_train(awt_encoder* e, const float* mel, int B, int n_frames, float* hidden, void* saved,
                                         size_t saved_bytes, void* stream) {
  AWT_REQUIRE(e && mel && hidden && saved && B > 0, AWT_ERR_INVALID, "encoder_forward_train: bad argument");
  AWT_REQUIRE(e->cfg.training, AWT_ERR_STATE, "encoder_forward_train: encoder was not created with cfg.training");
  const int T = 2 * e->cfg.n_ctx;
  if (n_frames != T)
    return awt_fail(AWT_ERR_VALUE, "Whisper expects the mel input features to be of length " + std::to_string(T) + ", but found " +
                                       std::to_string(n_frames) + ". Make sure to pad the input mel features to " + std::to_string(T) + ".");
  int rc = require_weights(e); if (rc) return rc;
  AWT_REQUIRE(saved_bytes >= awt_encoder_train_workspace_bytes(e, B), AWT_ERR_WORKSPACE, "encoder_forward_train: saved buffer too small");
  AWT_REQUIRE(((uintptr_t)saved & 255) == 0, AWT_ERR_INVALID, "encoder_forward_train: saved buffer must be 256-byte aligned");
  hipStream_t s = (hipStream_t)stream;
  TrainWs w = carve_train(e, (char*)saved, B);
  rc = conv_stem(e, mel, B, w.a1, w.h1, w.layer[0].x_in, s, e->train_base ? w.pre1 : nullptr); if (rc) return rc;
  for (int li = 0; li < e->cfg.n_layers; ++li) { rc = encoder_layer(e, e->layers[li], w.layer[li], B, true, s); if (rc) return rc; }
  return launch_layernorm(e->ctx, w.x_final, e->lnf_g, e->lnf_b, B * e->cfg.n_ctx, e->cfg.d_model, 1e-5f, hidden, Act{}, e->prec, s);
}

extern "C" int awt_encoder_set_comm(awt_encoder* e, awt_comm* m, int groups) {
  AWT_REQUIRE(e, AWT_ERR_INVALID, "encoder_set_comm: null encoder");
  AWT_REQUIRE(groups >= 1, AWT_ERR_INVALID, "encoder_set_comm: groups must be >= 1");
  AWT_REQUIRE(!m || m->ctx == e->ctx, AWT_ERR_INVALID, "encoder_set_comm: communicator and encoder belong to different contexts");
  e->comm = m;
  e->comm_groups = std::min(std::min(groups, 4), e->cfg.n_layers);
  return AWT_OK;
}

extern "C" int awt_encoder_backward(awt_encoder* e, const float* d_hidden, int B, void* saved, size_t saved_bytes, float* lora_grads,
                                    size_t n_grads, void* stream) {
  return awt_encoder_backward_ex(e, d_hidden, B, saved, saved_bytes, lora_grads, n_grads, 0u, stream);
}

extern "C" int awt_encoder_backward_ex(awt_encoder* e, const float* d_hidden, int B, void* saved, size_t saved_bytes, float* lora_grads,
                                       size_t n_grads, uint32_t flags, void* stream) {
  AWT_REQUIRE(e && d_hidden && saved && lora_grads && B > 0, AWT_ERR_INVALID, "encoder_backward: bad argument");
  AWT_REQUIRE(!(flags & ~(uint32_t)(AWT_BWD_ACCUMULATE | AWT_BWD_ALLREDUCE)), AWT_ERR_INVALID, "encoder_backward: unknown flag");
  AWT_REQUIRE(!(flags & AWT_BWD_ALLREDUCE) || e->comm, AWT_ERR_STATE, "encoder_backward: AWT_BWD_ALLREDUCE needs awt_encoder_set_comm first");
  const int accumulate = (flags & AWT_BWD_ACCUMULATE) ? 1 : 0;
  const bool exchange = (flags & AWT_BWD_ALLREDUCE) != 0;
  AWT_REQUIRE(e->cfg.training, AWT_ERR_STATE, "encoder_backward: encoder was not created with cfg.training");
  AWT_REQUIRE(saved_bytes >= awt_encoder_train_workspace_bytes(e, B), AWT_ERR_WORKSPACE, "encoder_backward: saved buffer too small");
// ... 207 lines not shown
```

### mlx8-ws-audio-transformer_amd/csrc/common.h

```cpp
#pragma once
#include <hip/hip_runtime.h>
#include <stdint.h>
#include <string>

#include "../../include/awt.h"

typedef unsigned short bf16_t;
typedef short bf16x8 __attribute__((ext_vector_type(8)));
typedef short bf16x4 __attribute__((ext_vector_type(4)));
typedef float f32x4 __attribute__((ext_vector_type(4)));
typedef float f32x16 __attribute__((ext_vector_type(16)));
typedef double f64x4 __attribute__((ext_vector_type(4)));

typedef _Float16 f16x8 __attribute__((ext_vector_type(8)));
typedef int i32x8 __attribute__((ext_vector_type(8)));
typedef int i32x2 __attribute__((ext_vector_type(2)));

#define AWT_WAVE 64

enum { PREC_BF16 = 1, PREC_F16 = 2, PREC_BF16X3 = 3, PREC_F16X3 = 4, PREC_F16F8 = 5 };
__host__ __device__ constexpr bool prec_known(int p) { return p >= PREC_BF16 && p <= PREC_F16F8; }
__host__ __device__ constexpr bool prec_is_f16(int p) { return p == PREC_F16 || p == PREC_F16X3 || p == PREC_F16F8; }
__host__ __device__ constexpr int prec_products(int p) { return (p == PREC_BF16 || p == PREC_F16) ? 1 : 3; }
constexpr int kF8Act = -2;
// ... 100 lines not shown
  const float y = 1.0f - p * t * __expf(-ax * ax);
  return copysignf(y, x);
}
__device__ __forceinline__ float gelu_erf(float x) {
  const float t = fabsf(x) * 0.70710678118654752440f, tc = fminf(t, 4.2f);
  float q = fmaf(-0.00010022104106610641f, tc, 0.0004615735961124301f);
  q = fmaf(q, tc, 0.0023022345267236233f);
  q = fmaf(q, tc, -0.029452508315443993f);
  q = fmaf(q, tc, 0.14896366000175476f);
  q = fmaf(q, tc, 0.9183286428451538f);
  q = fmaf(q, tc, 1.6279137134552002f);
  const float e = __builtin_amdgcn_exp2f(fmaf(tc - t, 12.5f, -tc * q));
  const float h = 0.5f * x;
  return fmaf(-fabsf(h), e, h + fabsf(h));
}

__host__ __device__ __forceinline__ int64_t w_frag_index(int n, int k, int ksteps) {
  const int nt = n >> 4, r = n & 15, ks = k >> 5, kq = (k & 31) >> 3, j = k & 7;
  return (((int64_t)nt * ksteps + ks) * 64 + (kq * 16 + r)) * 8 + j;
}

__host__ __device__ __forceinline__ int64_t w16f8_index(int n, int k, int ksteps16) {
  const int nt = n >> 5, r = n & 31, ks = k >> 4, h = (k & 15) >> 3, j = k & 7;
  return (((int64_t)nt * ksteps16 + ks) * 64 + (h * 32 + r)) * 8 + j;
}
__host__ __device__ __forceinline__ int64_t w8_index(int n, int k, int ktiles64) {
  const int nt = n >> 5, r = n & 31, kt = k >> 6, h = (k & 63) >> 5, b = k & 31;
  return (((int64_t)nt * ktiles64 + kt) * 64 + (h * 32 + r)) * 32 + b;
}

__host__ __device__ __forceinline__ int64_t w8s_index(int n, int k, int ktiles64, int is_hi8) {
  const int nt = n >> 4, r = n & 15, kt = k >> 6, kb = ((k & 63) >> 5) + (is_hi8 ? 2 : 0), b = k & 31;
  return (((int64_t)nt * ktiles64 + kt) * 64 + (kb * 16 + r)) * 32 + b;
}

struct Act { bf16_t* p16 = nullptr; bf16_t* lo16 = nullptr; uint8_t* hi8 = nullptr; uint8_t* lo8 = nullptr; char* ilv = nullptr; };
__device__ __forceinline__ void store_ilv4(char* ilv, int64_t off, uint2 h16, unsigned hi8, unsigned lo8) {
  char* line = ilv + (off >> 6) * 256;
  const int e = (int)(off & 63);
  *reinterpret_cast<uint2*>(line + e * 2) = h16;
  *reinterpret_cast<unsigned*>(line + 128 + e) = hi8;
  *reinterpret_cast<unsigned*>(line + 192 + e) = lo8;
}
template <int PREC, int S = kF8Act, bool SAT = false>
__device__ __forceinline__ void store_act4(const Act& o, int64_t off, const float (&v)[4]) {
  if constexpr (PREC == PREC_F16F8) {
    uint2 h16; unsigned hi8, lo8;
    f16f8x4<S, SAT>(v, h16, hi8, lo8);
    if (o.ilv) { store_ilv4(o.ilv, off, h16, hi8, lo8); return; }
    *reinterpret_cast<uint2*>(o.p16 + off) = h16;
    if (o.hi8) *reinterpret_cast<unsigned*>(o.hi8 + off) = hi8;
    *reinterpret_cast<unsigned*>(o.lo8 + off) = lo8;
  } else {
    bf16_t h[4], l[4];
#pragma unroll
    for (int t = 0; t < 4; ++t) split16<PREC == PREC_F16X3>(v[t], h[t], l[t]);
    *reinterpret_cast<uint2*>(o.p16 + off) = make_uint2(pack2(h[0], h[1]), pack2(h[2], h[3]));
    if (o.lo16) *reinterpret_cast<uint2*>(o.lo16 + off) = make_uint2(pack2(l[0], l[1]), pack2(l[2], l[3]));
  }
}

void awt_set_error(const std::string& msg);
int awt_fail(int code, const std::string& msg);

#define AWT_HIP_CHECK(expr)                                                                      \
  do {                                                                                           \
    hipError_t _e = (expr);                                                                      \
    if (_e != hipSuccess)                                                                        \
      return awt_fail(AWT_ERR_HIP, std::string(#expr) + ": " + hipGetErrorString(_e));           \
  } while (0)

#define AWT_REQUIRE(cond, code, msg)         \
  do {                                       \
    if (!(cond)) return awt_fail(code, msg); \
  } while (0)

struct awt_prof_state;
struct awt_ctx {
  int device = 0;
  int prof_on = 0;
  awt_prof_state* prof = nullptr;
  struct Table;
  Table* tables = nullptr;
  void* zeros = nullptr;
};

#define AWT_ONCE_PER_DEVICE(set)                                   \
  do {                                                             \
    static unsigned long long _done = 0;                           \
    int _dev = 0;                                                  \
    AWT_HIP_CHECK(hipGetDevice(&_dev));                            \
    if (!((_done >> (_dev & 63)) & 1ull)) {                        \
      set;                                                         \
      _done |= 1ull << (_dev & 63);                                \
    }                                                              \
  } while (0)

template <auto Kernel, class... Args>
int launch_kernel(dim3 grid, dim3 block, int lds, hipStream_t s, const Args&... args) {
  AWT_ONCE_PER_DEVICE(AWT_HIP_CHECK(hipFuncSetAttribute((const void*)Kernel, hipFuncAttributeMaxDynamicSharedMemorySize, lds)));
  hipLaunchKernelGGL(Kernel, grid, block, lds, s, args...);
  AWT_HIP_CHECK(hipGetLastError());
  return AWT_OK;
}

void awt_prof_begin(awt_ctx* c, int klass, hipStream_t s, double flops);
void awt_prof_end(awt_ctx* c, int klass, hipStream_t s);

struct ProfScope {
  awt_ctx* c; int klass; hipStream_t s;
  ProfScope(awt_ctx* c_, int k, hipStream_t s_, double flops = 0.0) : c(c_), klass(k), s(s_) {
    if (c && (c->prof_on >> klass) & 1) awt_prof_begin(c, klass, s, flops);
  }
  ~ProfScope() { if (c && (c->prof_on >> klass) & 1) awt_prof_end(c, klass, s); }
};

struct GemmSeg {
  const bf16_t* a_hi; const bf16_t* a_lo; int64_t lda;
  const bf16_t* w_hi; const bf16_t* w_lo; int w_ksteps, w_k0;
  const uint8_t* a8; const uint8_t* al8; const uint8_t* w8; const uint8_t* wl8;
  int w_exact16;
  const char* a_ilv; const char* w_pp;
  const bf16_t* ws16; const uint8_t* ws8;
  int ws_rows;
  int K;
  int rows_out, rows_in, row_mul, row_add;
};

enum GemmEpilogue {
  EPI_F32 = 0,
  EPI_F32_RESID = 1,
  EPI_BF16 = 2,
  EPI_BF16_GELU = 3,
  EPI_QKV = 4,
  EPI_F32_GELU_POS = 5,
  EPI_BF16_GELU_SAVE = 6,
  EPI_BF16_DGELU = 7
};

struct GemmOut {
  float* f32; const float* resid; int64_t ldo;
  bf16_t* hi; bf16_t* lo;
  uint8_t* hi8; uint8_t* lo8;
  char* ilv;
  bf16_t* hi2; bf16_t* lo2;
  const bf16_t* pre_hi; const bf16_t* pre_lo;
  const float* bias;
  const float* pos; int rows_pos;
  float scale;
  int n_valid;
  int S, H;
  int64_t plane_stride;
  int skip_v8;
};

int launch_gemm(awt_ctx* c, int M, int N, const GemmSeg* segs, int nseg, int prec, GemmEpilogue epi, const GemmOut& out,
                hipStream_t s);
bool gemm_pp_supported(int M, int N, int K, int epi);
int gemm_pp_slots();
int launch_gemm_pp(awt_ctx* c, int M, int N, const GemmSeg& seg, GemmEpilogue epi, const GemmOut& out, hipStream_t s);
size_t gemm_pp_weight_bytes(int N, int K);
int launch_pack_weight_pp(awt_ctx* c, const float* src, int N, int K, int row_off, char* dst, hipStream_t s);
int awt_gemm_pp_mode();
void awt_gemm_set_pp_mode(int v);
void awt_gemm_set_mfma16(int v);

int launch_layernorm(awt_ctx* c, const float* x, const float* gamma, const float* beta, int M, int d, float eps,
                     float* out_f32, const Act& out, int prec, hipStream_t s);
int launch_attention(awt_ctx* c, const bf16_t* q_hi, const bf16_t* q_lo, const bf16_t* k_hi, const bf16_t* k_lo,
                     const bf16_t* v_hi, const bf16_t* v_lo, bf16_t* o_hi, bf16_t* o_lo, float* o_f32, float* lse, int B, int H,
                     int S, int terms, hipStream_t s);
int launch_split_f32(awt_ctx* c, const float* x, int64_t n, float scale, bf16_t* hi, bf16_t* lo, hipStream_t s);
struct F8Planes { bf16_t* p16; uint8_t* hi8; uint8_t* lo8; };
int launch_split_planes(awt_ctx* c, const float* x, int64_t n, float scale, int prec, int f8_exp, bf16_t* p16, bf16_t* lo16, uint8_t* hi8,
                        uint8_t* lo8, hipStream_t s, char* ilv = nullptr);
int launch_attention_f16f8(awt_ctx* c, const F8Planes& q, const F8Planes& k, const F8Planes& v, const F8Planes& o, float* o_f32,
                           float* lse, int B, int H, int S, hipStream_t s, char* o_ilv = nullptr);
int launch_pack_weight(awt_ctx* c, const float* src, int N, int C, int taps, int64_t ld, int row_off, int col_off, float scale,
                       bf16_t* hi, bf16_t* lo, uint8_t* lo8, int prec, hipStream_t s, int* inexact = nullptr,
                       bf16_t* s16 = nullptr, uint8_t* s8 = nullptr);
int launch_im2col_conv1(awt_ctx* c, const float* mel, int B, int C, int T, int K_dst, const Act& out, int prec, hipStream_t s);

int logmel_whisper_impl(awt_ctx* c, const void* pcm, int pcm_is_i16, int64_t pcm_stride, const int32_t* n_valid,
                        int max_valid, int B, int n_frames_out, int n_mels, float* out, void* workspace, size_t ws_bytes, hipStream_t s,
                        int n_signal = 0);
int logmel_generic_impl(awt_ctx* c, const float* pcm, int64_t pcm_stride, int B, int n_samples, int sample_rate, int n_fft,
                        int hop, int n_mels, float f_min, float f_max, float log_eps, float* out, hipStream_t s);
int prepare_waveform_impl(awt_ctx* c, const void* pcm, int pcm_is_i16, int channels, int64_t channel_stride, int64_t sample_stride,
                          int n_in, int sr_in, int sr_out, float* out, int n_out, hipStream_t s);
int64_t resampled_length(int n_in, int sr_in, int sr_out);
int logmel_prepare_impl(awt_ctx* c, int n_fft, int n_mels, double f_min, double f_max, int sample_rate, int slaney);
int resample_prepare_impl(awt_ctx* c, int sr_in, int sr_out);
void awt_free_tables(awt_ctx* c);
void awt_attn_force_shape(int v);
void awt_attn_force_qt(int v);
void awt_gemm_set_gm(int v);
bool attention_f16f8_reads_v8(bool with_lse);
void awt_gemm_force_tile(int t);

int launch_attention_bwd(awt_ctx* c, const bf16_t* q_hi, const bf16_t* q_lo, const bf16_t* k_hi, const bf16_t* k_lo,
                         const bf16_t* v_hi, const bf16_t* v_lo, const bf16_t* o_hi, const bf16_t* o_lo, const bf16_t* do_hi,
                         const bf16_t* do_lo, const float* lse2, float* delta, bf16_t* g_hi, bf16_t* g_lo, int B, int H, int S,
                         float qscale, int terms, int grad_terms, hipStream_t s);
int launch_layernorm_bwd(awt_ctx* c, const float* dy, const float* x, const float* gamma, const float* dres, int M, int d, float eps,
                         float* dx, bf16_t* dx_hi, bf16_t* dx_lo, hipStream_t s, float gscale = 1.0f, const Act* out8 = nullptr);
int launch_transpose_f32(awt_ctx* c, const float* src, int N, int C, float* dst, hipStream_t s);
int launch_pack_weight_t(awt_ctx* c, const float* src, int N, int C, int64_t ld, int row_off, int col_off, float scale, bf16_t* hi,
                         bf16_t* lo, hipStream_t s);
int launch_outer_reduce(awt_ctx* c, const bf16_t* x_hi, const bf16_t* x_lo, int64_t ldx, int xcol, int r, const bf16_t* y_hi,
                        const bf16_t* y_lo, int64_t ldy, int ycol, int ny, int M, float scale, float* out, int64_t sj, int64_t sn,
                        float* partial, size_t partial_bytes, int accumulate, hipStream_t s);
size_t outer_reduce_partial_bytes(int M, int r, int ny);
```

### mlx8-ws-audio-transformer_amd/csrc/elementwise.hip

```cpp
#include "common.h"
#include "gemm_pp.h"

namespace {

__device__ __forceinline__ float4 ldg_once(const float4* p) {
  const f32x4 t = __builtin_nontemporal_load(reinterpret_cast<const f32x4*>(p));
  return make_float4(t[0], t[1], t[2], t[3]);
}

constexpr int kLnMaxChunks = 5;

template <int PREC>
__global__ __launch_bounds__(256) void layernorm_kernel(const float* __restrict__ x, const float* __restrict__ gamma,
                                                        const float* __restrict__ beta, int M, int d, float eps,
                                                        float* out_f32, Act out) {
  const int lane = threadIdx.x & 63;
  const int row = blockIdx.x * 4 + (threadIdx.x >> 6);
  if (row >= M) return;
  const int nchunk = d >> 2;
  const float4* xr = reinterpret_cast<const float4*>(x + (int64_t)row * d);
  float4 v[kLnMaxChunks];
  float sum = 0.f;
#pragma unroll
  for (int i = 0; i < kLnMaxChunks; ++i) {
    const int c = lane + 64 * i;
    if (c < nchunk) v[i] = ldg_once(xr + c);
    else v[i] = make_float4(0.f, 0.f, 0.f, 0.f);
    sum += (v[i].x + v[i].y) + (v[i].z + v[i].w);
  }
#pragma unroll
  for (int o = 32; o > 0; o >>= 1) sum += __shfl_xor(sum, o);
  const float mean = sum / (float)d;
  float sq = 0.f;
#pragma unroll
  for (int i = 0; i < kLnMaxChunks; ++i) {
    const int c = lane + 64 * i;
    if (c < nchunk) {
      const float a = v[i].x - mean, b = v[i].y - mean, cc = v[i].z - mean, dd = v[i].w - mean;
      sq += (a * a + b * b) + (cc * cc + dd * dd);
    }
  }
#pragma unroll
  for (int o = 32; o > 0; o >>= 1) sq += __shfl_xor(sq, o);
  const float rstd = 1.0f / sqrtf(sq / (float)d + eps);
  const float4* g4 = reinterpret_cast<const float4*>(gamma);
  const float4* b4 = reinterpret_cast<const float4*>(beta);
#pragma unroll
  for (int i = 0; i < kLnMaxChunks; ++i) {
    const int c = lane + 64 * i;
    if (c >= nchunk) continue;
    const float4 g = g4[c], bb = b4[c];
    float y[4] = {(v[i].x - mean) * rstd * g.x + bb.x, (v[i].y - mean) * rstd * g.y + bb.y,
                  (v[i].z - mean) * rstd * g.z + bb.z, (v[i].w - mean) * rstd * g.w + bb.w};
    if (out_f32) reinterpret_cast<float4*>(out_f32 + (int64_t)row * d)[c] = make_float4(y[0], y[1], y[2], y[3]);
    else store_act4<PREC>(out, (int64_t)row * d + 4 * c, y);
  }
}

__global__ __launch_bounds__(256) void split_kernel(const float* __restrict__ x, int64_t n4, float scale, bf16_t* hi, bf16_t* lo) {
  for (int64_t i = (int64_t)blockIdx.x * blockDim.x + threadIdx.x; i < n4; i += (int64_t)gridDim.x * blockDim.x) {
    const float4 v = reinterpret_cast<const float4*>(x)[i];
    bf16_t h[4], l[4];
    split_bf16(v.x * scale, h[0], l[0]); split_bf16(v.y * scale, h[1], l[1]); split_bf16(v.z * scale, h[2], l[2]); split_bf16(v.w * scale, h[3], l[3]);
    reinterpret_cast<uint2*>(hi)[i] = make_uint2(pack2(h[0], h[1]), pack2(h[2], h[3]));
    if (lo) reinterpret_cast<uint2*>(lo)[i] = make_uint2(pack2(l[0], l[1]), pack2(l[2], l[3]));
  }
}

template <int PREC>
__global__ __launch_bounds__(256) void split_planes_kernel(const float* __restrict__ x, int64_t n4, float scale, float f8_scale, bf16_t* p16,
                                                           bf16_t* lo16, uint8_t* hi8, uint8_t* lo8, char* ilv) {
  for (int64_t i = (int64_t)blockIdx.x * blockDim.x + threadIdx.x; i < n4; i += (int64_t)gridDim.x * blockDim.x) {
    const float4 q = reinterpret_cast<const float4*>(x)[i];
    const float v[4] = {q.x * scale, q.y * scale, q.z * scale, q.w * scale};
    bf16_t h[4], l[4];
    if constexpr (PREC == PREC_F16F8) {
      float lo[4];
#pragma unroll
      for (int t = 0; t < 4; ++t) { h[t] = f32_to_f16(v[t]); lo[t] = (v[t] - f16_to_f32(h[t])) * (f8_scale * pow2f(kF8Lo)); }
      const uint2 h16 = make_uint2(pack2(h[0], h[1]), pack2(h[2], h[3]));
      const unsigned b_hi = fp8x4<0>(v[0] * f8_scale, v[1] * f8_scale, v[2] * f8_scale, v[3] * f8_scale), b_lo = fp8x4<0>(lo[0], lo[1], lo[2], lo[3]);
      if (ilv) { store_ilv4(ilv, i * 4, h16, b_hi, b_lo); continue; }
      reinterpret_cast<uint2*>(p16)[i] = h16;
      reinterpret_cast<unsigned*>(hi8)[i] = b_hi;
      reinterpret_cast<unsigned*>(lo8)[i] = b_lo;
    } else {
#pragma unroll
      for (int t = 0; t < 4; ++t) split16<PREC == PREC_F16X3>(v[t], h[t], l[t]);
      reinterpret_cast<uint2*>(p16)[i] = make_uint2(pack2(h[0], h[1]), pack2(h[2], h[3]));
      if (lo16) reinterpret_cast<uint2*>(lo16)[i] = make_uint2(pack2(l[0], l[1]), pack2(l[2], l[3]));
    }
  }
}

template <int PREC>
__global__ __launch_bounds__(256) void pack_weight_kernel(const float* __restrict__ src, int N, int C, int taps, int64_t ld,
                                                          int row_off, int col_off, float scale, bf16_t* hi, bf16_t* lo, uint8_t* lo8,
                                                          int* inexact, bf16_t* s16, uint8_t* s8) {
  const int K = C * taps;
  bool any_inexact = false;
  const int64_t total = (int64_t)N * K;
  for (int64_t i = (int64_t)blockIdx.x * blockDim.x + threadIdx.x; i < total; i += (int64_t)gridDim.x * blockDim.x) {
    const int n = (int)(i / K), k = (int)(i - (int64_t)n * K);
    const int dt = k / C, c = k - dt * C;
    const float v = src[((int64_t)n * C + c) * taps + dt] * scale;
    if constexpr (PREC == PREC_F16F8) {
      const bf16_t h = f32_to_f16(v);
      hi[w16f8_index(row_off + n, col_off + k, (int)(ld >> 4))] = h;
      const int64_t o8 = w8_index(row_off + n, col_off + k, (int)(ld >> 6));
      reinterpret_cast<uint8_t*>(lo)[o8] = (uint8_t)(fp8x4<kF8Wgt>(v, 0.f, 0.f, 0.f) & 0xFF);
      lo8[o8] = (uint8_t)(fp8x4<kF8Wgt + kF8Lo>(v - f16_to_f32(h), 0.f, 0.f, 0.f) & 0xFF);
      if (s16) {
        s16[w_frag_index(row_off + n, col_off + k, (int)(ld >> 5))] = h;
        s8[w8s_index(row_off + n, col_off + k, (int)(ld >> 6), 1)] = reinterpret_cast<uint8_t*>(lo)[o8];
        s8[w8s_index(row_off + n, col_off + k, (int)(ld >> 6), 0)] = lo8[o8];
      }
      any_inexact |= (v != f16_to_f32(h));
    } else {
      bf16_t h, l; split16<PREC == PREC_F16X3>(v, h, l);
      if (PREC == PREC_F16X3) any_inexact |= ((l & 0x7FFF) != 0);
      const int64_t o = w_frag_index(row_off + n, col_off + k, (int)(ld >> 5));
      hi[o] = h;
      if (lo) lo[o] = l;
    }
  }
  if ((PREC == PREC_F16F8 || PREC == PREC_F16X3) && inexact && __builtin_amdgcn_ballot_w64(any_inexact) != 0 && (threadIdx.x & 63) == 0) atomicOr(inexact, 1);
}

__global__ __launch_bounds__(256) void pack_weight_pp_kernel(const float* __restrict__ src, int N, int K, int row_off, char* dst) {
  const int nk = K >> 5;
  const int64_t total = (int64_t)N * (K >> 2);
  for (int64_t i = (int64_t)blockIdx.x * blockDim.x + threadIdx.x; i < total; i += (int64_t)gridDim.x * blockDim.x) {
    const int n = (int)(i / (K >> 2)), k = (int)(i - (int64_t)n * (K >> 2)) * 4;
    const float4 q = *reinterpret_cast<const float4*>(src + (int64_t)n * K + k);
    const float v[4] = {q.x, q.y, q.z, q.w};
    uint2 h16; unsigned hi8, lo8;
    f16f8x4<kF8Wgt>(v, h16, hi8, lo8);
    const int row = row_off + n, bn = row >> 8, nin = row & 255, sgrp = (nin >> 5) & 1, grp = k >> 6, e = k & 63;
    char* rx = dst + pp::w_region_offset(bn, 2 * grp, sgrp, nk);
    char* ry = dst + pp::w_region_offset(bn, 2 * grp + 1, sgrp, nk);
    *reinterpret_cast<uint2*>(rx + pp::w_row_offset(nin, e >> 3) + (e & 7) * 2) = h16;
    *reinterpret_cast<unsigned*>(ry + pp::w_row_offset(nin, e >> 4) + (e & 15)) = lo8;
    *reinterpret_cast<unsigned*>(ry + pp::w_row_offset(nin, 4 + (e >> 4)) + (e & 15)) = hi8;
  }
}

constexpr int kImTile = 64;
template <int PREC>
__global__ __launch_bounds__(256) void im2col_conv1_kernel(const float* __restrict__ mel, int C, int T, int K_dst, Act out) {
  extern __shared__ __attribute__((aligned(16))) char smem[];
  float* tile = reinterpret_cast<float*>(smem);
  const int pitch = kImTile + 3;
  const int b = blockIdx.y, t0 = blockIdx.x * kImTile;
  const float* mb = mel + (int64_t)b * C * T;
  for (int i = threadIdx.x; i < C * (kImTile + 2); i += 256) {
    const int c = i / (kImTile + 2), tt = i - c * (kImTile + 2);
    const int t = t0 + tt - 1;
    tile[c * pitch + tt] = (t >= 0 && t < T) ? mb[(int64_t)c * T + t] : 0.f;
  }
  __syncthreads();
  const int groups = K_dst / 8;
  const int cg = C / 8;
  for (int i = threadIdx.x; i < kImTile * groups; i += 256) {
    const int tl = i / groups, g = i - tl * groups;
    const int t = t0 + tl;
    if (t >= T) continue;
    const int dt = g / cg, c0 = (g - dt * cg) * 8;
    float v[2][4];
#pragma unroll
    for (int j = 0; j < 8; ++j) v[j >> 2][j & 3] = dt < 3 ? tile[(c0 + j) * pitch + tl + dt] : 0.f;
    const int64_t off = ((int64_t)b * T + t) * K_dst + g * 8;
    store_act4<PREC>(out, off, v[0]);
    store_act4<PREC>(out, off + 4, v[1]);
  }
}

__global__ __launch_bounds__(256) void layernorm_bwd_kernel(const float* __restrict__ dy, const float* __restrict__ x,
                                                            const float* __restrict__ gamma, const float* dres, int M, int d,
                                                            float eps, float* dx, bf16_t* dx_hi, bf16_t* dx_lo, float gscale, Act out8) {
  const int lane = threadIdx.x & 63;
  const int row = blockIdx.x * 4 + (threadIdx.x >> 6);
  if (row >= M) return;
  const int nchunk = d >> 2;
  const float4* xr = reinterpret_cast<const float4*>(x + (int64_t)row * d);
  const float4* dyr = reinterpret_cast<const float4*>(dy + (int64_t)row * d);
  const float4* g4 = reinterpret_cast<const float4*>(gamma);
  float4 v[kLnMaxChunks], g[kLnMaxChunks];
  float sum = 0.f;
#pragma unroll
  for (int i = 0; i < kLnMaxChunks; ++i) {
    const int c = lane + 64 * i;
    v[i] = c < nchunk ? ldg_once(xr + c) : make_float4(0.f, 0.f, 0.f, 0.f);
    sum += (v[i].x + v[i].y) + (v[i].z + v[i].w);
  }
#pragma unroll
  for (int o = 32; o > 0; o >>= 1) sum += __shfl_xor(sum, o);
  const float mean = sum / (float)d;
  float sq = 0.f;
#pragma unroll
  for (int i = 0; i < kLnMaxChunks; ++i) {
    const int c = lane + 64 * i;
    if (c < nchunk) {
      v[i].x -= mean; v[i].y -= mean; v[i].z -= mean; v[i].w -= mean;
      sq += (v[i].x * v[i].x + v[i].y * v[i].y) + (v[i].z * v[i].z + v[i].w * v[i].w);
    }
  }
#pragma unroll
  for (int o = 32; o > 0; o >>= 1) sq += __shfl_xor(sq, o);
  const float rstd = 1.0f / sqrtf(sq / (float)d + eps);
  float s1 = 0.f, s2 = 0.f;
#pragma unroll
  for (int i = 0; i < kLnMaxChunks; ++i) {
    const int c = lane + 64 * i;
    g[i] = make_float4(0.f, 0.f, 0.f, 0.f);
    if (c < nchunk) {
      const float4 gy = ldg_once(dyr + c), gm = g4[c];
      v[i].x *= rstd; v[i].y *= rstd; v[i].z *= rstd; v[i].w *= rstd;
      g[i] = make_float4(gy.x * gscale * gm.x, gy.y * gscale * gm.y, gy.z * gscale * gm.z, gy.w * gscale * gm.w);
      s1 += (g[i].x + g[i].y) + (g[i].z + g[i].w);
      s2 += (g[i].x * v[i].x + g[i].y * v[i].y) + (g[i].z * v[i].z + g[i].w * v[i].w);
    }
  }
#pragma unroll
  for (int o = 32; o > 0; o >>= 1) { s1 += __shfl_xor(s1, o); s2 += __shfl_xor(s2, o); }
  const float c1 = s1 / (float)d, c2 = s2 / (float)d;
#pragma unroll
  for (int i = 0; i < kLnMaxChunks; ++i) {
    const int c = lane + 64 * i;
    if (c >= nchunk) continue;
    float y[4] = {rstd * (g[i].x - c1 - v[i].x * c2), rstd * (g[i].y - c1 - v[i].y * c2),
                  rstd * (g[i].z - c1 - v[i].z * c2), rstd * (g[i].w - c1 - v[i].w * c2)};
    if (dres) {
      const float4 r = ldg_once(reinterpret_cast<const float4*>(dres + (int64_t)row * d) + c);
      y[0] += r.x; y[1] += r.y; y[2] += r.z; y[3] += r.w;
    }
    reinterpret_cast<float4*>(dx + (int64_t)row * d)[c] = make_float4(y[0], y[1], y[2], y[3]);
    if (dx_hi) {
      bf16_t hi[4], lo[4];
#pragma unroll
      for (int j = 0; j < 4; ++j) split_bf16(y[j], hi[j], lo[j]);
      reinterpret_cast<uint2*>(dx_hi + (int64_t)row * d)[c] = make_uint2(pack2(hi[0], hi[1]), pack2(hi[2], hi[3]));
      if (dx_lo) reinterpret_cast<uint2*>(dx_lo + (int64_t)row * d)[c] = make_uint2(pack2(lo[0], lo[1]), pack2(lo[2], lo[3]));
    }
    if (out8.p16) store_act4<PREC_F16F8, kF8Act, true>(out8, (int64_t)row * d + 4 * c, y);
  }
}

__global__ __launch_bounds__(256) void transpose_f32_kernel(const float* __restrict__ src, int N, int C, float* __restrict__ dst) {
  __shared__ float tile[32][33];
  const int n0 = blockIdx.x * 32, c0 = blockIdx.y * 32;
  const int tx = threadIdx.x & 31, ty = threadIdx.x >> 5;
  for (int r = ty; r < 32; r += 8) {
    const int n = n0 + r, c = c0 + tx;
    tile[r][tx] = (n < N && c < C) ? src[(int64_t)n * C + c] : 0.f;
  }
  __syncthreads();
  for (int r = ty; r < 32; r += 8) {
    const int c = c0 + r, n = n0 + tx;
    if (c < C && n < N) dst[(int64_t)c * N + n] = tile[tx][r];
  }
}

__global__ __launch_bounds__(256) void pack_weight_t_kernel(const float* __restrict__ src, int N, int C, int64_t ld, int row_off,
                                                            int col_off, float scale, bf16_t* hi, bf16_t* lo) {
  __shared__ float tile[32][33];
  const int n0 = blockIdx.x * 32, c0 = blockIdx.y * 32;
  const int tx = threadIdx.x & 31, ty = threadIdx.x >> 5;
  for (int r = ty; r < 32; r += 8) {
    const int n = n0 + r, c = c0 + tx;
    tile[r][tx] = (n < N && c < C) ? src[(int64_t)n * C + c] : 0.f;
  }
  __syncthreads();
  for (int r = ty; r < 32; r += 8) {
    const int c = c0 + r, n = n0 + tx;
    if (c < C && n < N) {
      bf16_t h, l; split_bf16(tile[tx][r] * scale, h, l);
      const int64_t o = w_frag_index(row_off + c, col_off + n, (int)(ld >> 5));
      hi[o] = h;
      if (lo) lo[o] = l;
    }
  }
}

constexpr int kOrRows = 256;
constexpr int kOrMaxBlocks = 512;
template <int R>
__global__ __launch_bounds__(256) void outer_reduce_kernel(const bf16_t* x_hi, const bf16_t* x_lo, int64_t ldx, int xcol,
                                                           const bf16_t* y_hi, const bf16_t* y_lo, int64_t ldy, int ycol, int ny, int M,
                                                           float* partial) {
  __shared__ float xs[kOrRows][R];
  const int n = threadIdx.x * 4;
  float acc[R][4];
#pragma unroll
  for (int j = 0; j < R; ++j) { acc[j][0] = acc[j][1] = acc[j][2] = acc[j][3] = 0.f; }
  const int nslab = (M + kOrRows - 1) / kOrRows;
  for (int slab = blockIdx.x; slab < nslab; slab += gridDim.x) {
    const int m0 = slab * kOrRows;
    const int rows = min(kOrRows, M - m0);
    __syncthreads();
    for (int i = threadIdx.x; i < rows * R; i += 256) {
      const int mm = i / R, j = i - mm * R;
      const int64_t o = (int64_t)(m0 + mm) * ldx + xcol + j;
      xs[mm][j] = bf16_to_f32(x_hi[o]) + (x_lo ? bf16_to_f32(x_lo[o]) : 0.f);
    }
    __syncthreads();
    if (n < ny) {
      auto load_y = [&](int mm, float (&y)[4]) {
        const int64_t o = (int64_t)(m0 + mm) * ldy + ycol + n;
        const uint2 yh = *reinterpret_cast<const uint2*>(y_hi + o);
        uint2 yl = make_uint2(0u, 0u);
        if (y_lo) yl = *reinterpret_cast<const uint2*>(y_lo + o);
        y[0] = bf16_to_f32((bf16_t)(yh.x & 0xFFFF)) + bf16_to_f32((bf16_t)(yl.x & 0xFFFF));
        y[1] = bf16_to_f32((bf16_t)(yh.x >> 16)) + bf16_to_f32((bf16_t)(yl.x >> 16));
        y[2] = bf16_to_f32((bf16_t)(yh.y & 0xFFFF)) + bf16_to_f32((bf16_t)(yl.y & 0xFFFF));
        y[3] = bf16_to_f32((bf16_t)(yh.y >> 16)) + bf16_to_f32((bf16_t)(yl.y >> 16));
      };
      auto fma_row = [&](int mm, const float (&y)[4]) {
#pragma unroll
        for (int j = 0; j < R; ++j) {
          const float xv = xs[mm][j];
          acc[j][0] += xv * y[0]; acc[j][1] += xv * y[1]; acc[j][2] += xv * y[2]; acc[j][3] += xv * y[3];
        }
      };
      int mm = 0;
      for (; mm + 4 <= rows; mm += 4) {
        float y0[4], y1[4], y2[4], y3[4];
        load_y(mm, y0); load_y(mm + 1, y1); load_y(mm + 2, y2); load_y(mm + 3, y3);
        fma_row(mm, y0); fma_row(mm + 1, y1); fma_row(mm + 2, y2); fma_row(mm + 3, y3);
      }
      for (; mm < rows; ++mm) { float y[4]; load_y(mm, y); fma_row(mm, y); }
    }
  }
  if (n < ny) {
    float* p = partial + (int64_t)blockIdx.x * R * ny;
#pragma unroll
    for (int j = 0; j < R; ++j) *reinterpret_cast<float4*>(p + (int64_t)j * ny + n) = make_float4(acc[j][0], acc[j][1], acc[j][2], acc[j][3]);
  }
}

__global__ __launch_bounds__(256) void outer_reduce_final_kernel(const float* __restrict__ partial, int nslab, int R, int r, int ny, float scale,
                                                                 float* out, int64_t sj, int64_t sn, int accumulate) {
  __shared__ float red[8][32];
  const int col = threadIdx.x & 31, grp = threadIdx.x >> 5;
  const int idx = blockIdx.x * 32 + col;
  const bool live = idx < r * ny;
  const int j = live ? idx / ny : 0, n = live ? idx - j * ny : 0;
  const float* p = partial + (int64_t)j * ny + n;
  const int64_t step = (int64_t)R * ny;
  float a0 = 0.f, a1 = 0.f, a2 = 0.f, a3 = 0.f;
  int s = grp;
  for (; s + 24 < nslab; s += 32) {
    a0 += p[(int64_t)s * step]; a1 += p[(int64_t)(s + 8) * step]; a2 += p[(int64_t)(s + 16) * step]; a3 += p[(int64_t)(s + 24) * step];
  }
  for (; s < nslab; s += 8) a0 += p[(int64_t)s * step];
  red[grp][col] = (a0 + a1) + (a2 + a3);
  __syncthreads();
  if (grp == 0 && live) {
    const float acc = ((red[0][col] + red[1][col]) + (red[2][col] + red[3][col])) + ((red[4][col] + red[5][col]) + (red[6][col] + red[7][col]));
    float* o = out + j * sj + n * sn;
    *o = accumulate ? *o + acc * scale : acc * scale;
  }
}

}

int launch_layernorm(awt_ctx* c, const float* x, const float* gamma, const float* beta, int M, int d, float eps,
                     float* out_f32, const Act& out, int prec, hipStream_t s) {
  AWT_REQUIRE(x && gamma && beta && (out_f32 || out.p16 || out.ilv), AWT_ERR_INVALID, "layernorm: null argument");
  AWT_REQUIRE(out_f32 || prec != PREC_F16F8 || out.lo8 || out.ilv, AWT_ERR_INVALID, "layernorm: f16f8 output needs its lo8 plane (hi8 may be null: not consumed)");
  AWT_REQUIRE(!out.ilv || out_f32 || (prec == PREC_F16F8 && d % 64 == 0), AWT_ERR_INVALID, "layernorm: split lines are an f16f8 format of whole 64-element line pairs");
  AWT_REQUIRE(M > 0 && d > 0 && d % 4 == 0 && d <= 64 * 4 * kLnMaxChunks, AWT_ERR_INVALID, "layernorm: d must be a multiple of 4 and <= 1280");
  ProfScope prof(c, AWT_PROF_LAYERNORM, s, 0.0);
  const dim3 grid((M + 3) / 4), block(256);
  if (prec == PREC_F16F8) hipLaunchKernelGGL(layernorm_kernel<PREC_F16F8>, grid, block, 0, s, x, gamma, beta, M, d, eps, out_f32, out);
  else if (prec == PREC_F16X3 || prec == PREC_F16) hipLaunchKernelGGL(layernorm_kernel<PREC_F16X3>, grid, block, 0, s, x, gamma, beta, M, d, eps, out_f32, out);
  else hipLaunchKernelGGL(layernorm_kernel<PREC_BF16X3>, grid, block, 0, s, x, gamma, beta, M, d, eps, out_f32, out);
  AWT_HIP_CHECK(hipGetLastError());
  return AWT_OK;
}

int launch_split_f32(awt_ctx* c, const float* x, int64_t n, float scale, bf16_t* hi, bf16_t* lo, hipStream_t s) {
  AWT_REQUIRE(x && hi && n > 0 && n % 4 == 0, AWT_ERR_INVALID, "split: n must be a positive multiple of 4");
  ProfScope prof(c, AWT_PROF_OTHER, s, 0.0);
  const int64_t n4 = n / 4;
  int grid = (int)((n4 + 255) / 256); if (grid > 4096) grid = 4096;
  hipLaunchKernelGGL(split_kernel, dim3(grid), dim3(256), 0, s, x, n4, scale, hi, lo);
  AWT_HIP_CHECK(hipGetLastError());
  return AWT_OK;
}

int launch_split_planes(awt_ctx* c, const float* x, int64_t n, float scale, int prec, int f8_exp, bf16_t* p16, bf16_t* lo16, uint8_t* hi8,
                        uint8_t* lo8, hipStream_t s, char* ilv) {
  AWT_REQUIRE(x && (p16 || ilv) && n > 0 && n % 4 == 0, AWT_ERR_INVALID, "split: n must be a positive multiple of 4");
  AWT_REQUIRE(prec_known(prec), AWT_ERR_INVALID, "split: unknown precision");
  AWT_REQUIRE(prec != PREC_F16F8 || (hi8 && lo8) || ilv, AWT_ERR_INVALID, "split: f16f8 needs both e4m3 planes");
  AWT_REQUIRE(!ilv || (prec == PREC_F16F8 && n % 64 == 0), AWT_ERR_INVALID, "split: split lines are an f16f8 format of whole 64-element line pairs");
  AWT_REQUIRE(f8_exp >= -20 && f8_exp <= 20, AWT_ERR_INVALID, "split: bad e4m3 exponent");
  ProfScope prof(c, AWT_PROF_OTHER, s, 0.0);
  const int64_t n4 = n / 4;
  int grid = (int)((n4 + 255) / 256); if (grid > 4096) grid = 4096;
  const float f8s = f8_exp >= 0 ? (float)(1u << f8_exp) : 1.0f / (float)(1u << -f8_exp);
  if (prec == PREC_F16F8) hipLaunchKernelGGL(split_planes_kernel<PREC_F16F8>, dim3(grid), dim3(256), 0, s, x, n4, scale, f8s, p16, lo16, hi8, lo8, ilv);
  else if (prec == PREC_F16X3 || prec == PREC_F16) hipLaunchKernelGGL(split_planes_kernel<PREC_F16X3>, dim3(grid), dim3(256), 0, s, x, n4, scale, f8s, p16, prec == PREC_F16 ? nullptr : lo16, hi8, lo8, nullptr);
  else hipLaunchKernelGGL(split_planes_kernel<PREC_BF16X3>, dim3(grid), dim3(256), 0, s, x, n4, scale, f8s, p16, prec == PREC_BF16 ? nullptr : lo16, hi8, lo8, nullptr);
  AWT_HIP_CHECK(hipGetLastError());
  return AWT_OK;
}

size_t gemm_pp_weight_bytes(int N, int K) { return (size_t)((N + 255) / 256 * 256) * K * 4; }
int launch_pack_weight_pp(awt_ctx* c, const float* src, int N, int K, int row_off, char* dst, hipStream_t s) {
  AWT_REQUIRE(src && dst && N > 0 && K > 0 && K % 64 == 0 && row_off >= 0, AWT_ERR_INVALID, "pack_weight_pp: K must be a multiple of 64");
  const int64_t total = (int64_t)N * (K / 4);
  int grid = (int)((total + 255) / 256); if (grid > 4096) grid = 4096;
  hipLaunchKernelGGL(pack_weight_pp_kernel, dim3(grid), dim3(256), 0, s, src, N, K, row_off, dst);
  AWT_HIP_CHECK(hipGetLastError());
  return AWT_OK;
}

int launch_pack_weight(awt_ctx* c, const float* src, int N, int C, int taps, int64_t ld, int row_off, int col_off, float scale,
                       bf16_t* hi, bf16_t* lo, uint8_t* lo8, int prec, hipStream_t s, int* inexact, bf16_t* s16, uint8_t* s8) {
  AWT_REQUIRE(src && hi && N > 0 && C > 0 && taps > 0 && ld >= col_off + (int64_t)C * taps && ld % 32 == 0, AWT_ERR_INVALID, "pack_weight: bad shape");
  AWT_REQUIRE(prec != PREC_F16F8 || (lo && lo8 && ld % 64 == 0), AWT_ERR_INVALID, "pack_weight: f16f8 needs both e4m3 planes and K a multiple of 64");
  const int64_t total = (int64_t)N * C * taps;
  int grid = (int)((total + 255) / 256); if (grid > 4096) grid = 4096;
  if (prec == PREC_F16F8) hipLaunchKernelGGL(pack_weight_kernel<PREC_F16F8>, dim3(grid), dim3(256), 0, s, src, N, C, taps, ld, row_off, col_off, scale, hi, lo, lo8, inexact, s8 ? s16 : nullptr, s8);
  else if (prec == PREC_F16X3 || prec == PREC_F16) hipLaunchKernelGGL(pack_weight_kernel<PREC_F16X3>, dim3(grid), dim3(256), 0, s, src, N, C, taps, ld, row_off, col_off, scale, hi, prec == PREC_F16 ? nullptr : lo, lo8, inexact, nullptr, nullptr);
  else hipLaunchKernelGGL(pack_weight_kernel<PREC_BF16X3>, dim3(grid), dim3(256), 0, s, src, N, C, taps, ld, row_off, col_off, scale, hi, lo, lo8, inexact, nullptr, nullptr);
  AWT_HIP_CHECK(hipGetLastError());
  return AWT_OK;
}

int launch_im2col_conv1(awt_ctx* c, const float* mel, int B, int C, int T, int K_dst, const Act& out, int prec, hipStream_t s) {
  AWT_REQUIRE(mel && out.p16 && B > 0 && C > 0 && C % 8 == 0 && T > 0 && K_dst % 8 == 0 && K_dst >= 3 * C, AWT_ERR_INVALID, "im2col: bad shape");
  AWT_REQUIRE(prec != PREC_F16F8 || (out.hi8 && out.lo8), AWT_ERR_INVALID, "im2col: f16f8 output needs both e4m3 planes");
  ProfScope prof(c, AWT_PROF_OTHER, s, 0.0);
  const size_t lds = (size_t)C * (kImTile + 3) * sizeof(float);
  const dim3 grid((T + kImTile - 1) / kImTile, B), block(256);
  if (prec == PREC_F16F8) hipLaunchKernelGGL(im2col_conv1_kernel<PREC_F16F8>, grid, block, lds, s, mel, C, T, K_dst, out);
  else if (prec == PREC_F16X3 || prec == PREC_F16) hipLaunchKernelGGL(im2col_conv1_kernel<PREC_F16X3>, grid, block, lds, s, mel, C, T, K_dst, out);
  else hipLaunchKernelGGL(im2col_conv1_kernel<PREC_BF16X3>, grid, block, lds, s, mel, C, T, K_dst, out);
  AWT_HIP_CHECK(hipGetLastError());
  return AWT_OK;
}

int launch_layernorm_bwd(awt_ctx* c, const float* dy, const float* x, const float* gamma, const float* dres, int M, int d, float eps,
                         float* dx, bf16_t* dx_hi, bf16_t* dx_lo, hipStream_t s, float gscale, const Act* out8) {
  AWT_REQUIRE(dy && x && gamma && dx, AWT_ERR_INVALID, "layernorm_bwd: null argument");
  AWT_REQUIRE(M > 0 && d > 0 && d % 4 == 0 && d <= 64 * 4 * kLnMaxChunks, AWT_ERR_INVALID, "layernorm_bwd: d must be a multiple of 4 and <= 1280");
  AWT_REQUIRE(!out8 || (out8->p16 && out8->hi8 && out8->lo8), AWT_ERR_INVALID, "layernorm_bwd: the f16f8 output needs all three planes");
  ProfScope prof(c, AWT_PROF_LAYERNORM, s, 0.0);
  hipLaunchKernelGGL(layernorm_bwd_kernel, dim3((M + 3) / 4), dim3(256), 0, s, dy, x, gamma, dres, M, d, eps, dx, dx_hi, dx_lo, gscale, out8 ? *out8 : Act{});
  AWT_HIP_CHECK(hipGetLastError());
  return AWT_OK;
}

int launch_transpose_f32(awt_ctx* c, const float* src, int N, int C, float* dst, hipStream_t s) {
  AWT_REQUIRE(src && dst && N > 0 && C > 0, AWT_ERR_INVALID, "transpose_f32: bad argument");
  hipLaunchKernelGGL(transpose_f32_kernel, dim3((N + 31) / 32, (C + 31) / 32), dim3(256), 0, s, src, N, C, dst);
  AWT_HIP_CHECK(hipGetLastError());
  return AWT_OK;
}

int launch_pack_weight_t(awt_ctx* c, const float* src, int N, int C, int64_t ld, int row_off, int col_off, float scale, bf16_t* hi,
                         bf16_t* lo, hipStream_t s) {
  AWT_REQUIRE(src && hi && N > 0 && C > 0 && ld >= col_off + N && ld % 32 == 0, AWT_ERR_INVALID, "pack_weight_t: bad shape");
  hipLaunchKernelGGL(pack_weight_t_kernel, dim3((N + 31) / 32, (C + 31) / 32), dim3(256), 0, s, src, N, C, ld, row_off, col_off, scale, hi, lo);
  AWT_HIP_CHECK(hipGetLastError());
  return AWT_OK;
}

size_t outer_reduce_partial_bytes(int M, int r, int ny) {
  const int R = r <= 8 ? 8 : (r <= 16 ? 16 : 32);
  ny = ny < 1024 ? ny : 1024;
  const int nslab = (M + kOrRows - 1) / kOrRows;
  return (size_t)(nslab < kOrMaxBlocks ? nslab : kOrMaxBlocks) * R * ny * sizeof(float);
}

static int launch_outer_reduce_1(awt_ctx* c, const bf16_t* x_hi, const bf16_t* x_lo, int64_t ldx, int xcol, int r, const bf16_t* y_hi,
                        const bf16_t* y_lo, int64_t ldy, int ycol, int ny, int M, float scale, float* out, int64_t sj, int64_t sn,
                        float* partial, size_t partial_bytes, int accumulate, hipStream_t s) {
  AWT_REQUIRE(x_hi && y_hi && out && partial && r > 0 && r <= 32 && ny > 0 && ny % 4 == 0 && ny <= 1024, AWT_ERR_INVALID, "outer_reduce: bad shape");
  AWT_REQUIRE(ldy % 4 == 0 && ycol % 4 == 0, AWT_ERR_INVALID, "outer_reduce: Y columns must be 8-byte aligned");
  AWT_REQUIRE(partial_bytes >= outer_reduce_partial_bytes(M, r, ny), AWT_ERR_WORKSPACE, "outer_reduce: partial buffer too small");
  ProfScope prof(c, AWT_PROF_OTHER, s, 0.0);
  const int nslab_all = (M + kOrRows - 1) / kOrRows;
  const int nslab = nslab_all < kOrMaxBlocks ? nslab_all : kOrMaxBlocks;
  const int R = r <= 8 ? 8 : (r <= 16 ? 16 : 32);
  AWT_REQUIRE(xcol + R <= ldx, AWT_ERR_INVALID, "outer_reduce: X block exceeds its row");
  if (R == 8) hipLaunchKernelGGL(outer_reduce_kernel<8>, dim3(nslab), dim3(256), 0, s, x_hi, x_lo, ldx, xcol, y_hi, y_lo, ldy, ycol, ny, M, partial);
  else if (R == 16) hipLaunchKernelGGL(outer_reduce_kernel<16>, dim3(nslab), dim3(256), 0, s, x_hi, x_lo, ldx, xcol, y_hi, y_lo, ldy, ycol, ny, M, partial);
  else hipLaunchKernelGGL(outer_reduce_kernel<32>, dim3(nslab), dim3(256), 0, s, x_hi, x_lo, ldx, xcol, y_hi, y_lo, ldy, ycol, ny, M, partial);
  AWT_HIP_CHECK(hipGetLastError());
  hipLaunchKernelGGL(outer_reduce_final_kernel, dim3((r * ny + 31) / 32), dim3(256), 0, s, partial, nslab, R, r, ny, scale, out, sj, sn, accumulate);
  AWT_HIP_CHECK(hipGetLastError());
  return AWT_OK;
}

int launch_outer_reduce(awt_ctx* c, const bf16_t* x_hi, const bf16_t* x_lo, int64_t ldx, int xcol, int r, const bf16_t* y_hi,
                        const bf16_t* y_lo, int64_t ldy, int ycol, int ny, int M, float scale, float* out, int64_t sj, int64_t sn,
                        float* partial, size_t partial_bytes, int accumulate, hipStream_t s) {
  for (int n0 = 0; n0 < ny; n0 += 1024) {
    const int nc = ny - n0 < 1024 ? ny - n0 : 1024;
    int rc = launch_outer_reduce_1(c, x_hi, x_lo, ldx, xcol, r, y_hi, y_lo, ldy, ycol + n0, nc, M, scale, out + (int64_t)n0 * sn, sj, sn,
                                   partial, partial_bytes, accumulate, s);
    if (rc) return rc;
  }
  return AWT_OK;
}
```

### mlx8-ws-audio-transformer_amd/csrc/gemm.hip

```cpp
#include <algorithm>
#include <type_traits>
#include "common.h"
#include "gemm_pp.h"

#ifndef AWT_GEMM_GM
#define AWT_GEMM_GM 8
#endif

namespace {

int g_gm = AWT_GEMM_GM;
constexpr int kMaxSeg = 3;
typedef int i32x4_t __attribute__((ext_vector_type(4)));

struct GemmArgs {
  int M, N, nseg, tiles_m, tiles_n;
  int gm;
  GemmSeg seg[kMaxSeg];
  GemmOut out;
  const bf16_t* zeros;
  int64_t bs_a, bs_w, bs_o;
};

struct Cfg64 { static constexpr int WM = 2, WN = 2, TM = 2, TN = 4; };
// ... 901 lines not shown
  const int c8 = (lane & 7) * 8, r8 = lane >> 3;
  const int em0 = m0, en = n0 + wc * 64 + c8;
  float4 b0 = make_float4(0.f, 0.f, 0.f, 0.f), b1 = b0;
  if (g.out.bias && en < g.out.n_valid) { b0 = *reinterpret_cast<const float4*>(g.out.bias + en); b1 = *reinterpret_cast<const float4*>(g.out.bias + en + 4); }
  constexpr bool SIDE = EPI == EPI_F32_RESID || EPI == EPI_F32_GELU_POS || EPI == EPI_BF16_DGELU;
  auto strips = [&](auto full_t) {
    constexpr bool FULL = decltype(full_t)::value;
    float4 side[4][2], side_next[4][2];
    auto load_sides = [&](float4 (&d)[4][2], int i) {
#pragma unroll
      for (int it = 0; it < 4; ++it) {
        d[it][0] = load_side4<EPI, FULL>(g.out, em0 + i * 32 + r8 + 8 * it, en, g.M);
        d[it][1] = load_side4<EPI, FULL>(g.out, em0 + i * 32 + r8 + 8 * it, en + 4, g.M);
      }
    };
    if constexpr (SIDE) load_sides(side, 0);
#pragma unroll
    for (int i = 0; i < TM / 2; ++i) {
#pragma unroll
      for (int rt = 0; rt < 2; ++rt)
#pragma unroll
        for (int ct = 0; ct < TN; ++ct)
#pragma unroll
          for (int reg = 0; reg < 4; ++reg) patch[(rt * 16 + 4 * kq + reg) * PITCH + ct * 16 + r16] = acc[2 * i + rt][ct][reg];
      __builtin_amdgcn_wave_barrier();
      asm volatile("s_waitcnt lgkmcnt(0)" ::: "memory");
      if constexpr (SIDE) { if (i + 1 < TM / 2) load_sides(side_next, i + 1); }
#pragma unroll
      for (int it = 0; it < 4; ++it) {
        const int rl = r8 + 8 * it;
        const float4 v0 = *reinterpret_cast<const float4*>(patch + rl * PITCH + c8), v1 = *reinterpret_cast<const float4*>(patch + rl * PITCH + c8 + 4);
        store_out8_f8<EPI, FULL>(g.out, em0 + i * 32 + rl, en, v0, v1, side[it][0], side[it][1], b0, b1, g.M);
      }
      if constexpr (SIDE) {
#pragma unroll
        for (int it = 0; it < 4; ++it) { side[it][0] = side_next[it][0]; side[it][1] = side_next[it][1]; }
      }
      __builtin_amdgcn_wave_barrier();
      asm volatile("s_waitcnt lgkmcnt(0)" ::: "memory");
    }
  };
  if (m0 + BM <= g.M && n0 + BN <= g.out.n_valid) strips(std::true_type{}); else strips(std::false_type{});
}

template <auto Kernel>
int launch_tiles(GemmArgs a, int bm, int bn, int threads, int lds, hipStream_t s, int batch = 1) {
  a.tiles_m = (a.M + bm - 1) / bm;
  a.tiles_n = (a.N + bn - 1) / bn;
  a.gm = g_gm;
  return launch_kernel<Kernel>(dim3(a.tiles_m * a.tiles_n, batch), dim3(threads), lds, s, a);
}

int g_mfma16 = 1;
template <int EPI>
int launch_f8s(GemmArgs a, hipStream_t s) {
  return launch_tiles<gemm_f8s_kernel<EPI, false>>(a, 128, 256, 256, 2 * (128 * 64 * 2 + 2 * 128 * 64), s);
}

template <int EPI, class CFG>
int launch_f8(GemmArgs a, hipStream_t s) {
  constexpr int BM = CFG::WM * CFG::TM * 32, BN = CFG::WN * CFG::TN * 32, NT = CFG::WM * CFG::WN * 64;
  constexpr int lds = 2 * (BM * 64 * 2 + 2 * BM * 64);
  if (a.nseg == 1 && a.seg[0].w_exact16) return launch_tiles<gemm_f8_kernel<EPI, CFG, false, true>>(a, BM, BN, NT, lds, s);
  if (a.nseg == 1) return launch_tiles<gemm_f8_kernel<EPI, CFG, false>>(a, BM, BN, NT, lds, s);
  return launch_tiles<gemm_f8_kernel<EPI, CFG, true>>(a, BM, BN, NT, lds, s);
}

template <int EPI, bool ILV>
__global__ __launch_bounds__(512, 2) void gemm_pp_kernel(pp::Args g, GemmOut out) {
  extern __shared__ __attribute__((aligned(16))) char smem[];
  const int lane = threadIdx.x & 63;
  const int wave = __builtin_amdgcn_readfirstlane(threadIdx.x >> 6);
  const int wr = wave >> 2, wc = wave & 3, r16 = lane & 15, kq = lane >> 4;
  float* patch = reinterpret_cast<float*>(smem + pp::PATCH_BASE + wave * 8192);
  const int c8 = (lane & 7) * 8, r8 = lane >> 3;
  constexpr bool SIDE = EPI == EPI_F32_RESID;
  pp::kloop<pp::FMT_F16F8S>(g, smem, [&](int tm, int tn, pp::Acc<pp::FMT_F16F8S>& accs) {
    auto& acc = accs.t;
    const int m0 = tm * pp::BM, n0 = tn * pp::BN;
    const int em0 = m0 + wr * 128, en = n0 + wc * 64 + c8;
    float4 b0 = make_float4(0.f, 0.f, 0.f, 0.f), b1 = b0;
    if (out.bias && en < out.n_valid) { b0 = *reinterpret_cast<const float4*>(out.bias + en); b1 = *reinterpret_cast<const float4*>(out.bias + en + 4); }
    auto strips = [&](auto full_t) {
      constexpr bool FULL = decltype(full_t)::value;
      float4 side[4][2], side_next[4][2];
      auto load_sides = [&](float4 (&d)[4][2], int i) {
#pragma unroll
        for (int it = 0; it < 4; ++it) {
          d[it][0] = load_side4<EPI, FULL>(out, em0 + i * 32 + r8 + 8 * it, en, g.M);
          d[it][1] = load_side4<EPI, FULL>(out, em0 + i * 32 + r8 + 8 * it, en + 4, g.M);
        }
      };
      if constexpr (SIDE) load_sides(side, 0);
#pragma unroll
      for (int i = 0; i < 4; ++i) {
#pragma unroll
        for (int rt = 0; rt < 2; ++rt)
#pragma unroll
          for (int ct = 0; ct < 4; ++ct)
#pragma unroll
            for (int reg = 0; reg < 4; ++reg) {
              const int row = rt * 16 + 4 * kq + reg;
              patch[row * 64 + (((ct * 16 + r16 + 16 * kq) & 63) ^ ((reg & 1) << 2))] = acc[2 * i + rt][ct][reg];
            }
        __builtin_amdgcn_wave_barrier();
        asm volatile("s_waitcnt lgkmcnt(0)" ::: "memory");
        if constexpr (SIDE) { if (i + 1 < 4) load_sides(side_next, i + 1); }
#pragma unroll
        for (int it = 0; it < 4; ++it) {
          const int rl = r8 + 8 * it, sw = (rl & 1) << 2, rot = 16 * ((rl >> 2) & 3);
          const float4 v0 = *reinterpret_cast<const float4*>(patch + rl * 64 + (((c8 + rot) & 63) ^ sw)), v1 = *reinterpret_cast<const float4*>(patch + rl * 64 + (((c8 + 4 + rot) & 63) ^ sw));
          store_out8_f8<EPI, FULL, ILV>(out, em0 + i * 32 + rl, en, v0, v1, side[it][0], side[it][1], b0, b1, g.M);
        }
        if constexpr (SIDE) {
#pragma unroll
          for (int it = 0; it < 4; ++it) { side[it][0] = side_next[it][0]; side[it][1] = side_next[it][1]; }
        }
        __builtin_amdgcn_wave_barrier();
        asm volatile("s_waitcnt lgkmcnt(0)" ::: "memory");
      }
    };
    if (m0 + pp::BM <= g.M && n0 + pp::BN <= out.n_valid) strips(std::true_type{}); else strips(std::false_type{});
  });
}

template <int EPI, bool ILV>
int launch_pp(const pp::Args& a, const GemmOut& o, int grid, hipStream_t s) {
  return launch_kernel<gemm_pp_kernel<EPI, ILV>>(dim3(grid), dim3(pp::NT), pp::LDS_BYTES, s, a, o);
}

int g_force_tile = 0;

template <int TERMS, int BK, int EPI, class CFG, bool F16 = false, bool WX = false>
int launch_one(GemmArgs a, hipStream_t s) {
  using T = Tile<TERMS, BK, CFG, WX>;
  return launch_tiles<gemm_kernel<TERMS, BK, EPI, CFG, F16, WX>>(a, T::BM, T::BN, T::THREADS, T::LDS_BYTES, s);
}
template <int TERMS, int BK, int EPI, class CFG>
int launch_batched_one(GemmArgs a, int batch, hipStream_t s) {
  using T = Tile<TERMS, BK, CFG, false>;
  return launch_tiles<gemm_kernel<TERMS, BK, EPI, CFG, false, false, true>>(a, T::BM, T::BN, T::THREADS, T::LDS_BYTES, s, batch);
}

constexpr int kSlots = 512;
int pick_tile(int M, int N, int batch = 1) {
  const int64_t panels = (int64_t)((M + 127) / 128) * batch;
  int tile = g_force_tile;
  if (!tile) tile = (N % 256 == 0 && panels * (N / 256) >= kSlots) ? 256 : (panels * (N / 128) >= kSlots ? 128 : 64);
  return (tile == 256 && N % 256 != 0) ? 128 : tile;
}

template <int EPI>
int launch_epi(GemmArgs a, int prec, hipStream_t s) {
  if (prec == PREC_F16F8) {
    const int n256 = (a.N + 255) / 256 * 256;
    const bool f8s_ok = g_mfma16 && a.nseg == 1 && a.seg[0].ws16 && a.seg[0].ws8 && a.seg[0].a8 && !a.seg[0].w_exact16 &&
                        (a.N % 256 == 0 || (a.seg[0].ws_rows >= n256 && (int64_t)n256 * 3 <= (int64_t)a.N * 4));
    const int64_t t256f = (int64_t)((a.M + 127) / 128) * (f8s_ok ? n256 / 256 : a.N / 256);
    int tile = g_force_tile;
    if (!tile) tile = ((a.N % 256 == 0 || f8s_ok) && t256f >= kSlots) ? 256 : 128;
    if (tile == 256 && f8s_ok) return launch_f8s<EPI>(a, s);
    if (tile == 256 && a.N % 256 == 0) return launch_f8<EPI, CfgF8W4>(a, s);
    return launch_f8<EPI, CfgF8Sq>(a, s);
  }
  const int tile = pick_tile(a.M, a.N);
  if (prec == PREC_F16X3) {
    if (a.nseg == 1 && a.seg[0].w_exact16) {
      if (tile == 256) return launch_one<3, 32, EPI, CfgW4, true, true>(a, s);
      if (tile == 128) return launch_one<3, 32, EPI, Cfg128, true, true>(a, s);
      return launch_one<3, 64, EPI, Cfg64, true, true>(a, s);
    }
    if (tile == 256) return launch_one<3, 32, EPI, CfgW4, true>(a, s);
    if (tile == 128) return launch_one<3, 32, EPI, Cfg128, true>(a, s);
    return launch_one<3, 64, EPI, Cfg64, true>(a, s);
  }
  if (prec == PREC_F16) {
    if (tile == 256) return launch_one<1, 64, EPI, CfgW4, true>(a, s);
    if (tile == 128) return launch_one<1, 64, EPI, Cfg128, true>(a, s);
    return launch_one<1, 64, EPI, Cfg64, true>(a, s);
  }
  const int terms = prec_products(prec);
  if (tile == 256) return terms == 3 ? launch_one<3, 32, EPI, CfgW4>(a, s) : launch_one<1, 64, EPI, CfgW4>(a, s);
  if (tile == 128) return terms == 3 ? launch_one<3, 32, EPI, Cfg128>(a, s) : launch_one<1, 64, EPI, Cfg128>(a, s);
  return terms == 3 ? launch_one<3, 64, EPI, Cfg64>(a, s) : launch_one<1, 64, EPI, Cfg64>(a, s);
}


template <int EPI>
int launch_batched_epi(GemmArgs a, int batch, hipStream_t s) {
  const int tail = a.M % 128;
  const int tile = (!g_force_tile && tail > 0 && tail <= 64 && a.M < 1024) ? 64 : pick_tile(a.M, a.N, batch);
  if (tile == 256) return launch_batched_one<3, 32, EPI, CfgW4>(a, batch, s);
  if (tile == 128) return launch_batched_one<3, 32, EPI, Cfg128>(a, batch, s);
  return launch_batched_one<3, 64, EPI, Cfg64>(a, batch, s);
}

}

int launch_gemm_batched(awt_ctx* c, int batch, int M, int N, int K, const bf16_t* a_hi, const bf16_t* a_lo, int64_t lda, int64_t bs_a, const bf16_t* w_hi,
                        const bf16_t* w_lo, int64_t bs_w, float* out, const float* resid, int64_t ldo, int64_t bs_o, int n_valid, hipStream_t s) {
  AWT_REQUIRE(c && c->zeros && batch > 0 && batch <= 65535 && M > 0 && N > 0 && N % 128 == 0 && K > 0 && K % 64 == 0, AWT_ERR_INVALID,
              "gemm (batched): 1..65535 matrices, N % 128 == 0 and K % 64 == 0 required");
  AWT_REQUIRE(a_hi && a_lo && w_hi && w_lo && out && lda % 8 == 0 && lda >= K && ldo % 4 == 0 && n_valid > 0 && n_valid <= N && n_valid % 4 == 0 && ldo >= n_valid, AWT_ERR_INVALID,
              "gemm (batched): null plane, lda not a multiple of 8, or output columns / pitch not a multiple of 4");
  AWT_REQUIRE(bs_a % 8 == 0 && bs_w % 8 == 0 && bs_o % 4 == 0, AWT_ERR_INVALID, "gemm (batched): matrix strides must keep 16-byte alignment");
  GemmArgs a{};
  a.M = M; a.N = N; a.nseg = 1; a.zeros = (const bf16_t*)c->zeros;
  GemmSeg& sg = a.seg[0];
  sg.a_hi = a_hi; sg.a_lo = a_lo; sg.lda = lda; sg.w_hi = w_hi; sg.w_lo = w_lo; sg.w_ksteps = K / 32; sg.w_k0 = 0; sg.K = K;
  sg.rows_out = sg.rows_in = M; sg.row_mul = 1; sg.row_add = 0;
  a.out.f32 = out; a.out.resid = resid; a.out.ldo = ldo; a.out.n_valid = n_valid;
  a.bs_a = bs_a; a.bs_w = bs_w; a.bs_o = bs_o;
  ProfScope prof(c, AWT_PROF_GEMM, s, 2.0 * (double)batch * (double)M * (double)n_valid * (double)K);
  return resid ? launch_batched_epi<EPI_F32_RESID>(a, batch, s) : launch_batched_epi<EPI_F32>(a, batch, s);
}

int g_pp_mode = 1;
int awt_gemm_pp_mode() { return g_pp_mode; }
void awt_gemm_set_pp_mode(int v) { g_pp_mode = v; }
int gemm_pp_slots() {
  static int n_cu[64] = {};
  int dev = 0;
  if (hipGetDevice(&dev) != hipSuccess) return 0;
  if (!n_cu[dev & 63]) { hipDeviceProp_t p; if (hipGetDeviceProperties(&p, dev) != hipSuccess) return 0; n_cu[dev & 63] = p.multiProcessorCount > 0 ? p.multiProcessorCount : 256; }
  return n_cu[dev & 63];
}
bool gemm_pp_supported(int M, int N, int K, int epi) {
  return M > 0 && N > 0 && N % 256 == 0 && K >= 128 && K % 64 == 0 &&
         (epi == EPI_F32 || epi == EPI_F32_RESID || epi == EPI_BF16 || epi == EPI_BF16_GELU || epi == EPI_QKV);
}
int launch_gemm_pp(awt_ctx* c, int M, int N, const GemmSeg& seg, GemmEpilogue epi, const GemmOut& out, hipStream_t s) {
  AWT_REQUIRE(c && gemm_pp_supported(M, N, seg.K, epi), AWT_ERR_INVALID, "gemm (ping-pong): N % 256 == 0, K % 64 == 0, K >= 128 and a supported epilogue required");
  AWT_REQUIRE(seg.a_ilv && seg.w_pp && seg.rows_out == M && seg.rows_in == M && seg.row_mul == 1 && seg.row_add == 0 && seg.w_k0 == 0 && seg.w_ksteps == seg.K / 32 && seg.lda == seg.K,
              AWT_ERR_INVALID, "gemm (ping-pong): one plain, dense K segment over split-line activations and a packed weight image");
  AWT_REQUIRE(!out.ilv || ((epi == EPI_BF16 || epi == EPI_BF16_GELU) && out.ldo == N && out.n_valid == N), AWT_ERR_INVALID, "gemm (ping-pong): a split-line output is a dense [M, N] activation");
  pp::Args a{};
  a.A = seg.a_ilv; a.a_row_bytes = (int64_t)seg.lda * 4; a.W = seg.w_pp;
  a.M = M; a.N = N; a.K = seg.K; a.nk = seg.K / 32;
  a.tiles_m = (M + pp::BM - 1) / pp::BM; a.tiles_n = N / pp::BN; a.ntiles = a.tiles_m * a.tiles_n; a.gm = g_gm;
  const int grid = std::min(a.ntiles, gemm_pp_slots());
  ProfScope prof(c, AWT_PROF_GEMM, s, 2.0 * (double)M * (double)out.n_valid * (double)seg.K);
  switch (epi) {
    case EPI_F32: return launch_pp<EPI_F32, false>(a, out, grid, s);
    case EPI_F32_RESID: return launch_pp<EPI_F32_RESID, false>(a, out, grid, s);
    case EPI_BF16: return out.ilv ? launch_pp<EPI_BF16, true>(a, out, grid, s) : launch_pp<EPI_BF16, false>(a, out, grid, s);
    case EPI_BF16_GELU: return out.ilv ? launch_pp<EPI_BF16_GELU, true>(a, out, grid, s) : launch_pp<EPI_BF16_GELU, false>(a, out, grid, s);
    case EPI_QKV: return launch_pp<EPI_QKV, false>(a, out, grid, s);
    default: break;
  }
  return awt_fail(AWT_ERR_INVALID, "gemm (ping-pong): unsupported epilogue");
}

void awt_gemm_set_mfma16(int v) { g_mfma16 = v; }
void awt_gemm_force_tile(int t) { g_force_tile = t; }
void awt_gemm_set_gm(int v) { g_gm = v > 0 ? v : AWT_GEMM_GM; }

int launch_gemm(awt_ctx* c, int M, int N, const GemmSeg* segs, int nseg, int prec, GemmEpilogue epi, const GemmOut& out,
                hipStream_t s) {
  AWT_REQUIRE(M > 0 && N > 0 && N % 128 == 0, AWT_ERR_INVALID, "gemm: N must be a positive multiple of 128");
  AWT_REQUIRE(nseg >= 1 && nseg <= kMaxSeg, AWT_ERR_INVALID, "gemm: 1..3 K-segments");
  AWT_REQUIRE(prec_known(prec), AWT_ERR_INVALID, "gemm: unknown operand precision");
  const int terms = prec_products(prec);
  AWT_REQUIRE(c && c->zeros, AWT_ERR_INVALID, "gemm: context without a zero page");
  GemmArgs a{};
  a.M = M; a.N = N; a.nseg = nseg; a.out = out; a.zeros = (const bf16_t*)c->zeros;
  double ksum = 0;
  for (int i = 0; i < nseg; ++i) {
    a.seg[i] = segs[i];
    AWT_REQUIRE(segs[i].K > 0 && segs[i].K % 64 == 0, AWT_ERR_INVALID, "gemm: every K-segment must be a positive multiple of 64");
    if (prec == PREC_F16F8) AWT_REQUIRE(segs[i].a_hi && segs[i].w_hi && (segs[i].a8 || (segs[i].w_exact16 && nseg == 1)) && segs[i].al8 && segs[i].w8 && segs[i].wl8 && segs[i].w_ksteps % 2 == 0 && segs[i].w_k0 % 2 == 0,
                                        AWT_ERR_INVALID, "gemm (f16f8): null operand plane or a K-segment that is not 64-aligned in its weight matrix");
    else AWT_REQUIRE(segs[i].a_hi && segs[i].w_hi && (terms == 1 || (segs[i].a_lo && segs[i].w_lo)), AWT_ERR_INVALID, "gemm: null operand plane");
    AWT_REQUIRE(segs[i].lda % 8 == 0 && segs[i].w_ksteps > 0 && segs[i].w_k0 >= 0 && segs[i].w_k0 + segs[i].K / 32 <= segs[i].w_ksteps, AWT_ERR_INVALID,
                "gemm: lda must be a multiple of 8 and the segment must lie inside its fragment-major weight matrix");
    AWT_REQUIRE(segs[i].rows_out > 0 && segs[i].rows_in > 0, AWT_ERR_INVALID, "gemm: bad row map");
    ksum += segs[i].K;
  }
  ProfScope prof(c, AWT_PROF_GEMM, s, 2.0 * (double)M * (double)out.n_valid * ksum);
  switch (epi) {
    case EPI_F32: return launch_epi<EPI_F32>(a, prec, s);
    case EPI_F32_RESID: return launch_epi<EPI_F32_RESID>(a, prec, s);
    case EPI_BF16: return launch_epi<EPI_BF16>(a, prec, s);
    case EPI_BF16_GELU: return launch_epi<EPI_BF16_GELU>(a, prec, s);
    case EPI_QKV: return launch_epi<EPI_QKV>(a, prec, s);
    case EPI_F32_GELU_POS: return launch_epi<EPI_F32_GELU_POS>(a, prec, s);
    case EPI_BF16_GELU_SAVE: return launch_epi<EPI_BF16_GELU_SAVE>(a, prec, s);
    case EPI_BF16_DGELU: return launch_epi<EPI_BF16_DGELU>(a, prec, s);
  }
  return awt_fail(AWT_ERR_INVALID, "gemm: unknown epilogue");
}
```

### mlx8-ws-audio-transformer_amd/csrc/logmel.hip

```cpp
#include <math.h>
#include <vector>
#include <map>
#include <tuple>
#include "common.h"

namespace {

constexpr int kThreads = 256;
constexpr int kWaves = kThreads / 64;

struct LogmelParams {
  const void* pcm; int pcm_is_i16; int64_t pcm_stride;
  const int32_t* n_valid; int max_valid;
  int L;
  int n_fft, hop, n_bins, n_bin_tiles, nbp;
  int n_mels, T_out;
  const double* basis;
  const int* mel_start; const int* mel_count; const int* mel_off; const double* mel_w;
  int log_mode;
  double log_eps;
  float* out; unsigned* clip_max;
};

__device__ __forceinline__ unsigned float_order_key(float f) {
// ... 136 lines not shown
__global__ __launch_bounds__(256) void logmel_finalize_rows_kernel(float* out, const unsigned* clip_max, const int32_t* n_valid,
                                                                   int max_valid, int L, int n_fft, int hop, int n_mels, int T_out) {
  const int b = blockIdx.y;
  int nv = n_valid ? n_valid[b] : max_valid;
  nv = nv < L ? nv : L;
  const int n_live = live_frames(nv, n_fft, hop, T_out);
  const float thr = float_from_key(clip_max[b]) - 8.0f;
  float* o = out + (int64_t)b * n_mels * T_out;
  for (int i = blockIdx.x * blockDim.x + threadIdx.x; i < n_mels * T_out; i += gridDim.x * blockDim.x) {
    const float v = (i % T_out) < n_live ? o[i] : -10.f;
    o[i] = (fmaxf(v, thr) + 4.0f) * 0.25f;
  }
}

double hz_to_mel(double f, bool slaney) {
  if (!slaney) return 2595.0 * log10(1.0 + f / 700.0);
  if (f >= 1000.0) return 15.0 + log(f / 1000.0) * (27.0 / log(6.4));
  return 3.0 * f / 200.0;
}
double mel_to_hz(double m, bool slaney) {
  if (!slaney) return 700.0 * (pow(10.0, m / 2595.0) - 1.0);
  if (m >= 15.0) return 1000.0 * exp((log(6.4) / 27.0) * (m - 15.0));
  return 200.0 * m / 3.0;
}
std::vector<double> linspace(double a, double b, int n) {
  std::vector<double> v(n);
  const double step = (b - a) / (n - 1);
  for (int i = 0; i < n; ++i) v[i] = a + i * step;
  v[n - 1] = b;
  return v;
}

struct MelTable { int* start; int* count; int* off; double* w; };
struct BasisTable { double* basis; int n_bin_tiles; };
struct ResampleTable { float* taps; int* first; int* count; int orig, out, width, K; };

}

struct awt_ctx::Table {
  std::map<int, BasisTable> basis;
  std::map<std::tuple<int, int, int, int, int, int>, MelTable> mel;
  std::map<std::pair<int, int>, ResampleTable> resample;
  std::vector<void*> allocs;
};

void awt_free_tables(awt_ctx* c) {
  if (!c->tables) return;
  for (void* p : c->tables->allocs) (void)hipFree(p);
  delete c->tables;
  c->tables = nullptr;
}

namespace {

int get_basis(awt_ctx* c, int n_fft, hipStream_t s, BasisTable* out) {
  if (!c->tables) c->tables = new awt_ctx::Table();
  auto it = c->tables->basis.find(n_fft);
  if (it != c->tables->basis.end()) { *out = it->second; return AWT_OK; }
  const int n_bins = n_fft / 2 + 1;
  const int nbt = (n_bins + 15) / 16;
  const int ksteps = n_fft / 4;
  std::vector<double> h((size_t)nbt * 2 * ksteps * 64);
  for (int bt = 0; bt < nbt; ++bt)
    for (int ks = 0; ks < ksteps; ++ks)
      for (int lane = 0; lane < 64; ++lane) {
        const int n = 4 * ks + (lane >> 4);
        const int bin = 16 * bt + (lane & 15);
        double vc = 0.0, vs = 0.0;
        if (bin < n_bins) {
          const double w = 0.5 - 0.5 * cos(2.0 * M_PI * n / n_fft);
          const long long ph = ((long long)bin * n) % n_fft;
          const double ang = 2.0 * M_PI * (double)ph / n_fft;
          vc = w * cos(ang);
          vs = -w * sin(ang);
        }
        h[((size_t)(bt * 2 + 0) * ksteps + ks) * 64 + lane] = vc;
        h[((size_t)(bt * 2 + 1) * ksteps + ks) * 64 + lane] = vs;
      }
  BasisTable t{};
  t.n_bin_tiles = nbt;
  AWT_HIP_CHECK(hipMalloc((void**)&t.basis, h.size() * sizeof(double)));
  c->tables->allocs.push_back(t.basis);
  AWT_HIP_CHECK(hipMemcpy(t.basis, h.data(), h.size() * sizeof(double), hipMemcpyHostToDevice));
  c->tables->basis[n_fft] = t;
  *out = t;
  return AWT_OK;
}

int get_mel(awt_ctx* c, int n_bins, int n_mels, double fmin, double fmax, int sr, bool slaney, MelTable* out) {
  if (!c->tables) c->tables = new awt_ctx::Table();
  auto key = std::make_tuple(n_bins, n_mels, (int)lrint(fmin * 8), (int)lrint(fmax * 8), sr, (int)slaney);
  auto it = c->tables->mel.find(key);
  if (it != c->tables->mel.end()) { *out = it->second; return AWT_OK; }
  std::vector<double> mel_f = linspace(hz_to_mel(fmin, slaney), hz_to_mel(fmax, slaney), n_mels + 2);
  std::vector<double> ff(n_mels + 2);
  for (int i = 0; i < n_mels + 2; ++i) ff[i] = mel_to_hz(mel_f[i], slaney);
  std::vector<double> fft_f = linspace(0.0, (double)(sr / 2), n_bins);
  std::vector<int> start(n_mels), count(n_mels), off(n_mels);
  std::vector<double> w;
  for (int m = 0; m < n_mels; ++m) {
    int first = -1, last = -1;
    std::vector<double> col(n_bins);
    const double enorm = slaney ? 2.0 / (ff[m + 2] - ff[m]) : 1.0;
    for (int k = 0; k < n_bins; ++k) {
      const double down = -(ff[m] - fft_f[k]) / (ff[m + 1] - ff[m]);
      const double up = (ff[m + 2] - fft_f[k]) / (ff[m + 2] - ff[m + 1]);
      double v = down < up ? down : up;
      v = v > 0.0 ? v : 0.0;
      col[k] = v * enorm;
      if (v > 0.0) { if (first < 0) first = k; last = k; }
    }
    if (first < 0) { first = 0; last = -1; }
    start[m] = first; count[m] = last - first + 1; off[m] = (int)w.size();
    for (int k = first; k <= last; ++k) w.push_back(col[k]);
  }
  if (w.empty()) w.push_back(0.0);
  MelTable t{};
  AWT_HIP_CHECK(hipMalloc((void**)&t.start, n_mels * sizeof(int)));  c->tables->allocs.push_back(t.start);
  AWT_HIP_CHECK(hipMalloc((void**)&t.count, n_mels * sizeof(int)));  c->tables->allocs.push_back(t.count);
  AWT_HIP_CHECK(hipMalloc((void**)&t.off, n_mels * sizeof(int)));    c->tables->allocs.push_back(t.off);
  AWT_HIP_CHECK(hipMalloc((void**)&t.w, w.size() * sizeof(double))); c->tables->allocs.push_back(t.w);
  AWT_HIP_CHECK(hipMemcpy(t.start, start.data(), n_mels * sizeof(int), hipMemcpyHostToDevice));
  AWT_HIP_CHECK(hipMemcpy(t.count, count.data(), n_mels * sizeof(int), hipMemcpyHostToDevice));
  AWT_HIP_CHECK(hipMemcpy(t.off, off.data(), n_mels * sizeof(int), hipMemcpyHostToDevice));
  AWT_HIP_CHECK(hipMemcpy(t.w, w.data(), w.size() * sizeof(double), hipMemcpyHostToDevice));
  c->tables->mel[key] = t;
  *out = t;
  return AWT_OK;
}

template <int FTILES>
int launch_stage1(const LogmelParams& p, int B, int max_live, hipStream_t s) {
  constexpr int FT = 16 * FTILES;
  const int span = (FT - 1) * p.hop + p.n_fft;
  const int span_pad = span + span / p.hop + 1;
  const size_t lds = (((size_t)span_pad * 4 + 15) & ~(size_t)15) + (size_t)FT * p.nbp * 8;
  AWT_REQUIRE(lds <= 160 * 1024, AWT_ERR_INVALID, "logmel: frame tile does not fit LDS");
  AWT_ONCE_PER_DEVICE(AWT_HIP_CHECK(hipFuncSetAttribute((const void*)logmel_stage1_kernel<FTILES>, hipFuncAttributeMaxDynamicSharedMemorySize, 160 * 1024)));
  dim3 grid((max_live + FT - 1) / FT, B);
  if (grid.x == 0) return AWT_OK;
  hipLaunchKernelGGL(logmel_stage1_kernel<FTILES>, grid, dim3(kThreads), lds, s, p);
  AWT_HIP_CHECK(hipGetLastError());
  return AWT_OK;
}

int host_live_frames(int n_valid, int n_fft, int hop, int T_out) {
  if (n_valid <= 0) return 0;
  int n = (n_valid + n_fft / 2 + hop - 1) / hop;
  return n < T_out ? n : T_out;
}

}

size_t awt_logmel_workspace_bytes(int B) { return (((size_t)(B > 0 ? B : 1) * sizeof(unsigned)) + 255) & ~(size_t)255; }

int logmel_prepare_impl(awt_ctx* c, int n_fft, int n_mels, double f_min, double f_max, int sample_rate, int slaney) {
  AWT_REQUIRE(c, AWT_ERR_INVALID, "logmel_prepare: null context");
  AWT_REQUIRE(n_fft == 400 || n_fft == 512 || n_fft == 1024, AWT_ERR_INVALID, "logmel_prepare: n_fft must be 400, 512 or 1024");
  AWT_REQUIRE(n_mels > 0 && n_mels <= 128 && sample_rate > 0, AWT_ERR_INVALID, "logmel_prepare: n_mels must be in 1..128");
  BasisTable bt; MelTable mt;
  int rc = get_basis(c, n_fft, nullptr, &bt); if (rc) return rc;
  return get_mel(c, n_fft / 2 + 1, n_mels, f_min, f_max, sample_rate, slaney != 0, &mt);
}
int resample_prepare_impl(awt_ctx* c, int sr_in, int sr_out);

int logmel_whisper_impl(awt_ctx* c, const void* pcm, int pcm_is_i16, int64_t pcm_stride, const int32_t* n_valid,
                        int max_valid, int B, int n_frames_out, int n_mels, float* out, void* workspace, size_t ws_bytes, hipStream_t s,
                        int n_signal) {
  AWT_REQUIRE(c && pcm && out && workspace, AWT_ERR_INVALID, "logmel_whisper: null argument");
  if (n_signal > 0) {
    AWT_REQUIRE(n_signal > 200, AWT_ERR_INVALID, "logmel_whisper: the signal must be longer than n_fft / 2 = 200 samples (reflect padding)");
    n_frames_out = n_signal / 160;
  }
  AWT_REQUIRE(B > 0 && n_frames_out > 0 && (n_signal > 0 || n_frames_out % 4 == 0), AWT_ERR_INVALID,
              "logmel_whisper: B > 0 and n_frames_out % 4 == 0 required");
  AWT_REQUIRE(max_valid >= 0 && (pcm_stride >= max_valid || B == 1), AWT_ERR_INVALID, "logmel_whisper: pcm_stride < max_valid");
  AWT_REQUIRE(ws_bytes >= awt_logmel_workspace_bytes(B), AWT_ERR_WORKSPACE, "logmel_whisper: workspace too small");
  AWT_REQUIRE(((uintptr_t)out & 15) == 0, AWT_ERR_INVALID, "logmel_whisper: out must be 16-byte aligned");
  AWT_REQUIRE(n_mels == 80 || n_mels == 128, AWT_ERR_INVALID, "logmel_whisper: n_mels must be 80 (tiny .. large-v2) or 128 (large-v3)");
  const int n_fft = 400, hop = 160;
  BasisTable bt; MelTable mt;
  int rc = get_basis(c, n_fft, s, &bt); if (rc) return rc;
  rc = get_mel(c, n_fft / 2 + 1, n_mels, 0.0, 8000.0, 16000, true, &mt); if (rc) return rc;
  LogmelParams p{};
  p.pcm = pcm; p.pcm_is_i16 = pcm_is_i16; p.pcm_stride = pcm_stride; p.n_valid = n_valid; p.max_valid = max_valid;
  p.L = n_signal > 0 ? n_signal : n_frames_out * hop; p.n_fft = n_fft; p.hop = hop; p.n_bins = n_fft / 2 + 1; p.n_bin_tiles = bt.n_bin_tiles;
  p.nbp = bt.n_bin_tiles * 16 + 1; p.n_mels = n_mels; p.T_out = n_frames_out; p.basis = bt.basis;
  p.mel_start = mt.start; p.mel_count = mt.count; p.mel_off = mt.off; p.mel_w = mt.w;
  p.log_mode = 0; p.log_eps = 0.0; p.out = out; p.clip_max = reinterpret_cast<unsigned*>(workspace);
  const int mv = max_valid < p.L ? max_valid : p.L;
  const int max_live = host_live_frames(mv, n_fft, hop, n_frames_out);
  ProfScope prof(c, AWT_PROF_LOGMEL, s, 2.0 * 2.0 * n_fft * p.n_bins * (double)max_live * B);
  hipLaunchKernelGGL(logmel_init_max_kernel, dim3((B + 255) / 256), dim3(256), 0, s, p.clip_max, B);
  AWT_HIP_CHECK(hipGetLastError());
  rc = launch_stage1<2>(p, B, max_live, s); if (rc) return rc;
  if (n_frames_out % 4 == 0) {
    const int work = n_mels * (n_frames_out / 4);
    int gx = (work + 255) / 256; if (gx > 64) gx = 64;
    hipLaunchKernelGGL(logmel_finalize_kernel, dim3(gx, B), dim3(256), 0, s, out, p.clip_max, n_valid, max_valid, p.L, n_fft, hop,
                       n_mels, n_frames_out);
  } else {
    const int work = n_mels * n_frames_out;
    int gx = (work + 255) / 256; if (gx > 256) gx = 256;
    hipLaunchKernelGGL(logmel_finalize_rows_kernel, dim3(gx, B), dim3(256), 0, s, out, p.clip_max, n_valid, max_valid, p.L, n_fft, hop,
                       n_mels, n_frames_out);
  }
  AWT_HIP_CHECK(hipGetLastError());
  return AWT_OK;
}

int logmel_generic_impl(awt_ctx* c, const float* pcm, int64_t pcm_stride, int B, int n_samples, int sample_rate, int n_fft,
                        int hop, int n_mels, float f_min, float f_max, float log_eps, float* out, hipStream_t s) {
  AWT_REQUIRE(c && pcm && out, AWT_ERR_INVALID, "logmel_generic: null argument");
  AWT_REQUIRE(B > 0 && n_samples > n_fft / 2, AWT_ERR_INVALID, "logmel_generic: need B > 0 and n_samples > n_fft / 2 (reflect padding)");
  AWT_REQUIRE(n_fft == 400 || n_fft == 512 || n_fft == 1024, AWT_ERR_INVALID, "logmel_generic: n_fft must be 400, 512 or 1024");
  AWT_REQUIRE(hop > 0 && hop % 4 == 0 && hop <= n_fft, AWT_ERR_INVALID, "logmel_generic: hop must be a multiple of 4 and <= n_fft");
  AWT_REQUIRE(n_mels > 0 && n_mels <= 128, AWT_ERR_INVALID, "logmel_generic: n_mels must be in 1..128");
  AWT_REQUIRE(f_min >= 0 && f_max > f_min && f_max <= sample_rate / 2, AWT_ERR_INVALID, "logmel_generic: need 0 <= f_min < f_max <= sr/2");
  BasisTable bt; MelTable mt;
  int rc = get_basis(c, n_fft, s, &bt); if (rc) return rc;
  rc = get_mel(c, n_fft / 2 + 1, n_mels, f_min, f_max, sample_rate, false, &mt); if (rc) return rc;
  LogmelParams p{};
  p.pcm = pcm; p.pcm_is_i16 = 0; p.pcm_stride = pcm_stride; p.n_valid = nullptr; p.max_valid = n_samples;
  p.L = n_samples; p.n_fft = n_fft; p.hop = hop; p.n_bins = n_fft / 2 + 1; p.n_bin_tiles = bt.n_bin_tiles;
  p.nbp = bt.n_bin_tiles * 16 + 1; p.n_mels = n_mels; p.T_out = 1 + n_samples / hop; p.basis = bt.basis;
  p.mel_start = mt.start; p.mel_count = mt.count; p.mel_off = mt.off; p.mel_w = mt.w;
  p.log_mode = 1; p.log_eps = (double)log_eps; p.out = out; p.clip_max = nullptr;
  ProfScope prof(c, AWT_PROF_LOGMEL, s, 2.0 * 2.0 * n_fft * p.n_bins * (double)p.T_out * B);
  return launch_stage1<1>(p, B, p.T_out, s);
}

namespace {

template <bool I16>
__global__ __launch_bounds__(256) void resample_mono_kernel(const void* pcm, int channels, int64_t cstride, int64_t sstride,
                                                            int n_in, ResampleTable t, int n_res, float* out, int n_out) {
  const int n = blockIdx.x * 256 + threadIdx.x;
  if (n >= n_out) return;
  if (n >= n_res) { out[n] = 0.f; return; }
  auto sample = [&](int m) {
    float sum = 0.f;
    for (int c = 0; c < channels; ++c) {
      const int64_t off = c * cstride + m * sstride;
      sum += I16 ? (float)reinterpret_cast<const int16_t*>(pcm)[off] * (1.0f / 32768.0f) : reinterpret_cast<const float*>(pcm)[off];
    }
    return channels > 1 ? sum / (float)channels : sum;
  };
  if (t.taps == nullptr) { out[n] = sample(n); return; }
  const int j = n / t.out, ph = n - j * t.out;
  const int base = j * t.orig - t.width;
  const float* taps = t.taps + (int64_t)ph * t.K;
  const int k0 = t.first[ph], k1 = k0 + t.count[ph];
  float acc = 0.f;
  for (int k = max(k0, -base); k < k1; ++k) {
    const int m = base + k;
    if (m >= n_in) break;
    acc = fmaf(taps[k], sample(m), acc);
  }
  out[n] = acc;
}

int get_resample(awt_ctx* c, int sr_in, int sr_out, ResampleTable* out) {
  if (!c->tables) c->tables = new awt_ctx::Table();
  int a = sr_in, b = sr_out;
  while (b) { const int r = a % b; a = b; b = r; }
  const int orig = sr_in / a, outp = sr_out / a;
  auto it = c->tables->resample.find({orig, outp});
  if (it != c->tables->resample.end()) { *out = it->second; return AWT_OK; }
  const double lpw = 6.0, rolloff = 0.99;
  const double basef = (double)(orig < outp ? orig : outp) * rolloff;
  const int width = (int)ceil(lpw * orig / basef);
  const int K = 2 * width + orig;
  std::vector<float> taps((size_t)outp * K);
  std::vector<int> first(outp), count(outp);
  for (int i = 0; i < outp; ++i) {
    const double phase = (double)((float)(-i) / (float)outp);
    int lo = K, hi = -1;
    for (int k = 0; k < K; ++k) {
      double t = (phase + (double)(k - width) / (double)orig) * basef;
      t = t < -lpw ? -lpw : (t > lpw ? lpw : t);
      const double cw = cos(t * M_PI / lpw / 2.0);
      const double window = cw * cw;
      const double tp = t * M_PI;
      const double sinc = tp == 0.0 ? 1.0 : sin(tp) / tp;
      const float v = (float)(sinc * window * (basef / (double)orig));
      taps[(size_t)i * K + k] = v;
      if (v != 0.f) { if (k < lo) lo = k; hi = k; }
    }
    first[i] = hi < 0 ? 0 : lo; count[i] = hi < 0 ? 0 : hi - lo + 1;
  }
  ResampleTable t{}; t.orig = orig; t.out = outp; t.width = width; t.K = K;
  AWT_HIP_CHECK(hipMalloc((void**)&t.taps, taps.size() * sizeof(float))); c->tables->allocs.push_back(t.taps);
  AWT_HIP_CHECK(hipMalloc((void**)&t.first, outp * sizeof(int)));         c->tables->allocs.push_back(t.first);
  AWT_HIP_CHECK(hipMalloc((void**)&t.count, outp * sizeof(int)));         c->tables->allocs.push_back(t.count);
  AWT_HIP_CHECK(hipMemcpy(t.taps, taps.data(), taps.size() * sizeof(float), hipMemcpyHostToDevice));
  AWT_HIP_CHECK(hipMemcpy(t.first, first.data(), outp * sizeof(int), hipMemcpyHostToDevice));
  AWT_HIP_CHECK(hipMemcpy(t.count, count.data(), outp * sizeof(int), hipMemcpyHostToDevice));
  c->tables->resample[{orig, outp}] = t;
  *out = t;
  return AWT_OK;
}

}

int64_t resampled_length(int n_in, int sr_in, int sr_out) {
  int a = sr_in, b = sr_out;
// ... 36 lines not shown
```

Measured before the change: 1386 clips/s.

## Compute conv stem only over live mel positions, broadcast padded tail

The conv1/conv2 stem of awt_audio_encode now runs over only the positions covered by real audio plus a margin. Past that margin the zero-padded mel frames give a constant conv output, so one representative row is computed and an expand kernel copies it to the tail while adding positional embeddings. This cuts the stem's GEMM and im2col work for short clips padded to 30 s. The costs are an extra full-size pass that writes x and added correctness risk at the boundary rows; the 12 transformer layers still process all 1500 positions.

```diff
diff --git a/include/awt.h b/include/awt.h
--- a/include/awt.h
+++ b/include/awt.h
@@ -109,6 +109,8 @@
 int awt_audio_encode(awt_encoder* e, const void* pcm, int pcm_is_i16, int64_t pcm_stride, const int32_t* n_valid,
                      int max_valid, int B, float* input_features_out, float* last_hidden_state, void* workspace,
                      size_t ws_bytes, void* stream);
+
+int awt_conv_stem_positions(int n_ctx, int max_valid);
 
 int awt_op_linear(awt_ctx* c, const float* x , const float* w , const float* bias ,
                   float* y , int M, int N, int K, int terms, void* workspace, size_t ws_bytes, void* stream);
diff --git a/mlx8-ws-audio-transformer_amd/_lib.py b/mlx8-ws-audio-transformer_amd/_lib.py
--- a/mlx8-ws-audio-transformer_amd/_lib.py
+++ b/mlx8-ws-audio-transformer_amd/_lib.py
@@ -76,6 +76,7 @@
     "awt_encoder_set_comm": (_i, [_vp, _vp, _i]),
     "awt_audio_encode_workspace_bytes": (_sz, [_vp, _i]),
     "awt_audio_encode": (_i, [_vp, _vp, _i, _i64, _vp, _i, _i, _vp, _vp, _vp, _sz, _vp]),
+    "awt_conv_stem_positions": (_i, [_i, _i]),
     "awt_op_linear": (_i, [_vp, _vp, _vp, _vp, _vp, _i, _i, _i, _i, _vp, _sz, _vp]),
     "awt_op_linear_workspace_bytes": (_sz, [_i, _i, _i]),
     "awt_op_layernorm": (_i, [_vp, _vp, _vp, _vp, _vp, _i, _i, _f, _vp]),
@@ -208,3 +209,7 @@
 
 def tuning_set(key: str, value: int) -> None:
     check(lib().awt_tuning_set(key.encode(), int(value)))
+
+
+def conv_stem_positions(n_ctx: int, max_valid: int) -> int:
+    return int(lib().awt_conv_stem_positions(int(n_ctx), int(max_valid)))
diff --git a/mlx8-ws-audio-transformer_amd/csrc/awt_api.hip b/mlx8-ws-audio-transformer_amd/csrc/awt_api.hip
--- a/mlx8-ws-audio-transformer_amd/csrc/awt_api.hip
+++ b/mlx8-ws-audio-transformer_amd/csrc/awt_api.hip
@@ -36,6 +36,7 @@
   p->spans[klass].push_back(p->open[klass]);
 }
 
+static int g_conv_live = 1;
 static int g_pp_mask = 12;
 extern "C" int awt_tuning_set(const char* key, int value) {
   AWT_REQUIRE(key, AWT_ERR_INVALID, "tuning_set: null key");
@@ -62,6 +63,11 @@
   if (!strcmp(key, "gemm_mfma16")) {
     AWT_REQUIRE(value == 0 || value == 1, AWT_ERR_INVALID, "tuning_set: gemm_mfma16 must be 1 (default: the f16f8 GEMM's 16 x 16 MFMA form where it applies) or 0 (32 x 32 only)");
     awt_gemm_set_mfma16(value);
+    return AWT_OK;
+  }
+  if (!strcmp(key, "conv_live")) {
+    AWT_REQUIRE(value == 0 || value == 1, AWT_ERR_INVALID, "tuning_set: conv_live must be 1 (default: the conv stem of awt_audio_encode computes the live positions only) or 0 (every position)");
+    g_conv_live = value;
     return AWT_OK;
   }
   if (!strcmp(key, "attn_shape")) {
@@ -218,6 +224,7 @@
   int prec = PREC_BF16X3;
   Linear conv1, conv2;
   float* pos = nullptr;
+  float* zero_row = nullptr;
   float *lnf_g = nullptr, *lnf_b = nullptr;
   std::vector<Layer> layers;
   std::vector<void*> allocs;
@@ -447,26 +454,31 @@
   return w;
 }
 
-int conv_stem(awt_encoder* e, const float* mel, int Bc, bf16_t* const a1[2], bf16_t* const h1[2], float* x, hipStream_t s, bf16_t* const* pre1 = nullptr) {
+int conv_stem(awt_encoder* e, const float* mel, int Bc, bf16_t* const a1[2], bf16_t* const h1[2], float* x, hipStream_t s, bf16_t* const* pre1 = nullptr,
+              int Sc = 0, float* g = nullptr) {
   const awt_encoder_cfg& c = e->cfg;
   const int S = c.n_ctx, T = 2 * S, d = c.d_model, terms = e->prec;
-  const int M = Bc * S, Mt = Bc * T;
+  const bool compact = Sc > 0 && Sc < S && g && !pre1;
+  const int So = compact ? Sc : S, To = 2 * So;
+  const int M = Bc * So, Mt = Bc * To;
   const int k1 = conv1_k(c.n_mels);
   const Act aa1 = make_act(a1[0], a1[1], (size_t)Mt * k1, terms), ah1 = make_act(h1[0], h1[1], (size_t)Mt * d, terms);
-  int rc = launch_im2col_conv1(e->ctx, mel, Bc, c.n_mels, T, k1, aa1, terms, s); if (rc) return rc;
+  int rc = launch_im2col_conv1(e->ctx, mel, Bc, c.n_mels, T, To, k1, aa1, terms, s); if (rc) return rc;
   {
     GemmSeg sg = seg_plain(aa1, k1, e->conv1.w, 0, k1, Mt);
-    GemmOut o{}; set_out(o, ah1); o.ldo = d; o.bias = e->conv1.bias; o.n_valid = d;
+    GemmOut o{}; set_out(o, ah1); o.ldo = d; o.bias = e->conv1.bias; o.n_valid = d; o.m_pick = Bc * T;
     if (pre1) { o.hi2 = pre1[0]; o.lo2 = pre1[1]; }
     rc = launch_gemm(e->ctx, Mt, d, &sg, 1, terms, pre1 ? EPI_BF16_GELU_SAVE : EPI_BF16_GELU, o, s); if (rc) return rc;
   }
   GemmSeg sg[3];
   for (int dt = 0; dt < 3; ++dt) {
     sg[dt] = seg_plain(ah1, d, e->conv2.w, (int64_t)dt * d, d, M);
-    sg[dt].rows_out = S; sg[dt].rows_in = T; sg[dt].row_mul = 2; sg[dt].row_add = dt - 1;
-  }
-  GemmOut o{}; o.f32 = x; o.ldo = d; o.bias = e->conv2.bias; o.n_valid = d; o.pos = e->pos; o.rows_pos = S;
-  return launch_gemm(e->ctx, M, d, sg, 3, terms, EPI_F32_GELU_POS, o, s);
+    sg[dt].rows_out = So; sg[dt].rows_in = To; sg[dt].row_mul = 2; sg[dt].row_add = dt - 1;
+  }
+  GemmOut o{}; o.f32 = compact ? g : x; o.ldo = d; o.bias = e->conv2.bias; o.n_valid = d; o.m_pick = Bc * S;
+  if (compact) { o.pos = e->zero_row; o.rows_pos = 1; } else { o.pos = e->pos; o.rows_pos = S; }
+  rc = launch_gemm(e->ctx, M, d, sg, 3, terms, EPI_F32_GELU_POS, o, s); if (rc || !compact) return rc;
+  return launch_expand_conv_rows(e->ctx, g, e->pos, Bc, S, Sc, d, x, s);
 }
 
 int encoder_layer(awt_encoder* e, Layer& L, const LayerBufs& b, int Bc, bool save, hipStream_t s) {
@@ -524,14 +536,26 @@
   return pp_fc2 ? linear_pp(e, b.ff[0], L.fc2, M, EPI_F32_RESID, o, s) : linear_with_lora(e, b.u2, b.ff, f, L.fc2, L.l2, M, EPI_F32_RESID, o, s);
 }
 
-int forward_chunk(awt_encoder* e, const float* mel, int Bc, float* hidden, char* ws_base, hipStream_t s) {
+int forward_chunk(awt_encoder* e, const float* mel, int Bc, float* hidden, char* ws_base, hipStream_t s, int Sc = 0) {
   const awt_encoder_cfg& c = e->cfg;
   const int M = Bc * c.n_ctx, d = c.d_model;
   const bool two = e->planes == 2;
   Workspace w = carve(e, ws_base, Bc);
   bf16_t* a1[2] = {w.a1[0], two ? w.a1[1] : nullptr};
   bf16_t* h1[2] = {w.h1[0], two ? w.h1[1] : nullptr};
-  int rc = conv_stem(e, mel, Bc, a1, h1, w.x, s); if (rc) return rc;
+  float* g = nullptr;
+  if (Sc > 0 && Sc < c.n_ctx) {
+    char* const base = (char*)w.a1[0];
+    const size_t room = (size_t)(ws_base + w.bytes - base), Mt = (size_t)Bc * 2 * Sc;
+    size_t off = 0;
+    auto take = [&](size_t bytes) { char* p = base + off; off += align_up(bytes); return p; };
+    bf16_t *ca1[2] = {nullptr, nullptr}, *ch1[2] = {nullptr, nullptr};
+    for (int p = 0; p < e->planes; ++p) ca1[p] = (bf16_t*)take(Mt * conv1_k(c.n_mels) * 2);
+    for (int p = 0; p < e->planes; ++p) ch1[p] = (bf16_t*)take(Mt * d * 2);
+    float* cg = (float*)take((size_t)Bc * Sc * d * 4);
+    if (off <= room) { g = cg; for (int p = 0; p < 2; ++p) { a1[p] = ca1[p]; h1[p] = ch1[p]; } }
+  }
+  int rc = conv_stem(e, mel, Bc, a1, h1, w.x, s, nullptr, g ? Sc : 0, g); if (rc) return rc;
   LayerBufs b{};
   b.x_in = b.x_mid = b.x_out = w.x;
   for (int p = 0; p < 2; ++p) {
@@ -650,6 +674,7 @@
   for (int dt = 0; dt < 3 && !rc && e->train_base; ++dt) rc = alloc_planes(e, &e->conv2T[dt], d, d);
   if (!rc) rc = alloc_linear(e, &e->conv2, d, 3 * d);
   if (!rc) rc = dev_alloc(e, (void**)&e->pos, (size_t)cfg->n_ctx * d * 4);
+  if (!rc) rc = dev_alloc(e, (void**)&e->zero_row, (size_t)d * 4);
   if (!rc) rc = dev_alloc(e, (void**)&e->lnf_g, (size_t)d * 4);
   if (!rc) rc = dev_alloc(e, (void**)&e->lnf_b, (size_t)d * 4);
   e->layers.resize(cfg->n_layers);
@@ -846,6 +871,7 @@
   hipStream_t s = (hipStream_t)stream;
   const int T = 2 * e->cfg.n_ctx;
   const int chunk = std::min(B, e->chunk);
+  const int Sc = g_conv_live ? conv_stem_positions(e->cfg.n_ctx, max_valid) : 0;
   char* base = (char*)workspace;
   const size_t enc_bytes = carve(e, nullptr, chunk).bytes;
   float* mel_buf = (float*)(base + enc_bytes);
@@ -857,11 +883,13 @@
     rc = logmel_whisper_impl(e->ctx, (const char*)pcm + (size_t)b0 * pcm_stride * esz, pcm_is_i16, pcm_stride,
                              n_valid ? n_valid + b0 : nullptr, max_valid, Bc, T, e->cfg.n_mels, mel, lm_ws, awt_logmel_workspace_bytes(Bc), s);
     if (rc) return rc;
-    rc = forward_chunk(e, mel, Bc, hidden + (size_t)b0 * e->cfg.n_ctx * e->cfg.d_model, base, s);
+    rc = forward_chunk(e, mel, Bc, hidden + (size_t)b0 * e->cfg.n_ctx * e->cfg.d_model, base, s, Sc);
     if (rc) return rc;
   }
   return AWT_OK;
 }
+
+extern "C" int awt_conv_stem_positions(int n_ctx, int max_valid) { return conv_stem_positions(n_ctx, max_valid); }
 
 extern "C" size_t awt_op_linear_workspace_bytes(int M, int N, int K) {
   const size_t npad = ((size_t)N + 255) / 256 * 256;
diff --git a/mlx8-ws-audio-transformer_amd/csrc/common.h b/mlx8-ws-audio-transformer_amd/csrc/common.h
--- a/mlx8-ws-audio-transformer_amd/csrc/common.h
+++ b/mlx8-ws-audio-transformer_amd/csrc/common.h
@@ -276,6 +276,7 @@
   int S, H;
   int64_t plane_stride;
   int skip_v8;
+  int m_pick;
 };
 
 int launch_gemm(awt_ctx* c, int M, int N, const GemmSeg* segs, int nseg, int prec, GemmEpilogue epi, const GemmOut& out,
@@ -303,7 +304,9 @@
 int launch_pack_weight(awt_ctx* c, const float* src, int N, int C, int taps, int64_t ld, int row_off, int col_off, float scale,
                        bf16_t* hi, bf16_t* lo, uint8_t* lo8, int prec, hipStream_t s, int* inexact = nullptr,
                        bf16_t* s16 = nullptr, uint8_t* s8 = nullptr);
-int launch_im2col_conv1(awt_ctx* c, const float* mel, int B, int C, int T, int K_dst, const Act& out, int prec, hipStream_t s);
+int launch_im2col_conv1(awt_ctx* c, const float* mel, int B, int C, int T_mel, int T, int K_dst, const Act& out, int prec, hipStream_t s);
+int launch_expand_conv_rows(awt_ctx* c, const float* g, const float* pos, int B, int S, int Sc, int d, float* x, hipStream_t s);
+int conv_stem_positions(int n_ctx, int max_valid);
 
 int logmel_whisper_impl(awt_ctx* c, const void* pcm, int pcm_is_i16, int64_t pcm_stride, const int32_t* n_valid,
                         int max_valid, int B, int n_frames_out, int n_mels, float* out, void* workspace, size_t ws_bytes, hipStream_t s,
diff --git a/mlx8-ws-audio-transformer_amd/csrc/elementwise.hip b/mlx8-ws-audio-transformer_amd/csrc/elementwise.hip
--- a/mlx8-ws-audio-transformer_amd/csrc/elementwise.hip
+++ b/mlx8-ws-audio-transformer_amd/csrc/elementwise.hip
@@ -147,16 +147,16 @@
 
 constexpr int kImTile = 64;
 template <int PREC>
-__global__ __launch_bounds__(256) void im2col_conv1_kernel(const float* __restrict__ mel, int C, int T, int K_dst, Act out) {
+__global__ __launch_bounds__(256) void im2col_conv1_kernel(const float* __restrict__ mel, int C, int T_mel, int T, int K_dst, Act out) {
   extern __shared__ __attribute__((aligned(16))) char smem[];
   float* tile = reinterpret_cast<float*>(smem);
   const int pitch = kImTile + 3;
   const int b = blockIdx.y, t0 = blockIdx.x * kImTile;
-  const float* mb = mel + (int64_t)b * C * T;
+  const float* mb = mel + (int64_t)b * C * T_mel;
   for (int i = threadIdx.x; i < C * (kImTile + 2); i += 256) {
     const int c = i / (kImTile + 2), tt = i - c * (kImTile + 2);
     const int t = t0 + tt - 1;
-    tile[c * pitch + tt] = (t >= 0 && t < T) ? mb[(int64_t)c * T + t] : 0.f;
+    tile[c * pitch + tt] = (t >= 0 && t < T) ? mb[(int64_t)c * T_mel + t] : 0.f;
   }
   __syncthreads();
   const int groups = K_dst / 8;
@@ -172,6 +172,29 @@
     const int64_t off = ((int64_t)b * T + t) * K_dst + g * 8;
     store_act4<PREC>(out, off, v[0]);
     store_act4<PREC>(out, off + 4, v[1]);
+  }
+}
+
+__global__ __launch_bounds__(256) void expand_conv_rows_kernel(const float4* __restrict__ g, const float4* __restrict__ pos, int rows, int S, int Sc, int d4,
+                                                                float4* __restrict__ x) {
+  const int lane = threadIdx.x & 63;
+  const int row = blockIdx.x * 4 + (threadIdx.x >> 6);
+  if (row >= rows) return;
+  const int b = row / S, p = row - b * S;
+  const int src = p < Sc - 1 ? p : (p == S - 1 ? Sc - 1 : Sc - 2);
+  const float4* gr = g + ((int64_t)b * Sc + src) * d4;
+  const float4* pr = pos + (int64_t)p * d4;
+  float4* xr = x + (int64_t)row * d4;
+  float4 v[kLnMaxChunks], q[kLnMaxChunks];
+#pragma unroll
+  for (int i = 0; i < kLnMaxChunks; ++i) {
+    const int c = lane + 64 * i;
+    if (c < d4) { v[i] = gr[c]; q[i] = pr[c]; }
+  }
+#pragma unroll
+  for (int i = 0; i < kLnMaxChunks; ++i) {
+    const int c = lane + 64 * i;
+    if (c < d4) xr[c] = make_float4(v[i].x + q[i].x, v[i].y + q[i].y, v[i].z + q[i].z, v[i].w + q[i].w);
   }
 }
 
@@ -430,15 +453,25 @@
   return AWT_OK;
 }
 
-int launch_im2col_conv1(awt_ctx* c, const float* mel, int B, int C, int T, int K_dst, const Act& out, int prec, hipStream_t s) {
-  AWT_REQUIRE(mel && out.p16 && B > 0 && C > 0 && C % 8 == 0 && T > 0 && K_dst % 8 == 0 && K_dst >= 3 * C, AWT_ERR_INVALID, "im2col: bad shape");
+int launch_im2col_conv1(awt_ctx* c, const float* mel, int B, int C, int T_mel, int T, int K_dst, const Act& out, int prec, hipStream_t s) {
+  AWT_REQUIRE(mel && out.p16 && B > 0 && C > 0 && C % 8 == 0 && T > 0 && T <= T_mel && K_dst % 8 == 0 && K_dst >= 3 * C, AWT_ERR_INVALID, "im2col: bad shape");
   AWT_REQUIRE(prec != PREC_F16F8 || (out.hi8 && out.lo8), AWT_ERR_INVALID, "im2col: f16f8 output needs both e4m3 planes");
   ProfScope prof(c, AWT_PROF_OTHER, s, 0.0);
   const size_t lds = (size_t)C * (kImTile + 3) * sizeof(float);
   const dim3 grid((T + kImTile - 1) / kImTile, B), block(256);
-  if (prec == PREC_F16F8) hipLaunchKernelGGL(im2col_conv1_kernel<PREC_F16F8>, grid, block, lds, s, mel, C, T, K_dst, out);
-  else if (prec == PREC_F16X3 || prec == PREC_F16) hipLaunchKernelGGL(im2col_conv1_kernel<PREC_F16X3>, grid, block, lds, s, mel, C, T, K_dst, out);
-  else hipLaunchKernelGGL(im2col_conv1_kernel<PREC_BF16X3>, grid, block, lds, s, mel, C, T, K_dst, out);
+  if (prec == PREC_F16F8) hipLaunchKernelGGL(im2col_conv1_kernel<PREC_F16F8>, grid, block, lds, s, mel, C, T_mel, T, K_dst, out);
+  else if (prec == PREC_F16X3 || prec == PREC_F16) hipLaunchKernelGGL(im2col_conv1_kernel<PREC_F16X3>, grid, block, lds, s, mel, C, T_mel, T, K_dst, out);
+  else hipLaunchKernelGGL(im2col_conv1_kernel<PREC_BF16X3>, grid, block, lds, s, mel, C, T_mel, T, K_dst, out);
+  AWT_HIP_CHECK(hipGetLastError());
+  return AWT_OK;
+}
+
+int launch_expand_conv_rows(awt_ctx* c, const float* g, const float* pos, int B, int S, int Sc, int d, float* x, hipStream_t s) {
+  AWT_REQUIRE(g && pos && x && B > 0 && Sc >= 2 && Sc < S && d > 0 && d % 4 == 0 && d <= 64 * 4 * kLnMaxChunks, AWT_ERR_INVALID, "expand_conv_rows: bad shape (2 <= Sc < S, d % 4 == 0, d <= 1280)");
+  AWT_REQUIRE((int64_t)B * S < (int64_t)1 << 30, AWT_ERR_INVALID, "expand_conv_rows: more than 2^30 rows");
+  ProfScope prof(c, AWT_PROF_OTHER, s, 0.0);
+  const int rows = B * S;
+  hipLaunchKernelGGL(expand_conv_rows_kernel, dim3((rows + 3) / 4), dim3(256), 0, s, (const float4*)g, (const float4*)pos, rows, S, Sc, d / 4, (float4*)x);
   AWT_HIP_CHECK(hipGetLastError());
   return AWT_OK;
 }
diff --git a/mlx8-ws-audio-transformer_amd/csrc/gemm.hip b/mlx8-ws-audio-transformer_amd/csrc/gemm.hip
--- a/mlx8-ws-audio-transformer_amd/csrc/gemm.hip
+++ b/mlx8-ws-audio-transformer_amd/csrc/gemm.hip
@@ -1077,18 +1077,19 @@
 
 template <int EPI>
 int launch_epi(GemmArgs a, int prec, hipStream_t s) {
+  const int Mp = a.out.m_pick > 0 ? a.out.m_pick : a.M;
   if (prec == PREC_F16F8) {
     const int n256 = (a.N + 255) / 256 * 256;
     const bool f8s_ok = g_mfma16 && a.nseg == 1 && a.seg[0].ws16 && a.seg[0].ws8 && a.seg[0].a8 && !a.seg[0].w_exact16 &&
                         (a.N % 256 == 0 || (a.seg[0].ws_rows >= n256 && (int64_t)n256 * 3 <= (int64_t)a.N * 4));
-    const int64_t t256f = (int64_t)((a.M + 127) / 128) * (f8s_ok ? n256 / 256 : a.N / 256);
+    const int64_t t256f = (int64_t)((Mp + 127) / 128) * (f8s_ok ? n256 / 256 : a.N / 256);
     int tile = g_force_tile;
     if (!tile) tile = ((a.N % 256 == 0 || f8s_ok) && t256f >= kSlots) ? 256 : 128;
     if (tile == 256 && f8s_ok) return launch_f8s<EPI>(a, s);
     if (tile == 256 && a.N % 256 == 0) return launch_f8<EPI, CfgF8W4>(a, s);
     return launch_f8<EPI, CfgF8Sq>(a, s);
   }
-  const int tile = pick_tile(a.M, a.N);
+  const int tile = pick_tile(Mp, a.N);
   if (prec == PREC_F16X3) {
     if (a.nseg == 1 && a.seg[0].w_exact16) {
       if (tile == 256) return launch_one<3, 32, EPI, CfgW4, true, true>(a, s);
@@ -1198,7 +1199,8 @@
     else AWT_REQUIRE(segs[i].a_hi && segs[i].w_hi && (terms == 1 || (segs[i].a_lo && segs[i].w_lo)), AWT_ERR_INVALID, "gemm: null operand plane");
     AWT_REQUIRE(segs[i].lda % 8 == 0 && segs[i].w_ksteps > 0 && segs[i].w_k0 >= 0 && segs[i].w_k0 + segs[i].K / 32 <= segs[i].w_ksteps, AWT_ERR_INVALID,
                 "gemm: lda must be a multiple of 8 and the segment must lie inside its fragment-major weight matrix");
-    AWT_REQUIRE(segs[i].rows_out > 0 && segs[i].rows_in > 0, AWT_ERR_INVALID, "gemm: bad row map");
+    AWT_REQUIRE(segs[i].rows_out > 0 && segs[i].rows_in > 0 && segs[i].row_mul > 0 && (int64_t)segs[i].row_mul * segs[i].rows_out == segs[i].rows_in, AWT_ERR_INVALID,
+                "gemm: bad row map (rows_in must be row_mul * rows_out)");
     ksum += segs[i].K;
   }
   ProfScope prof(c, AWT_PROF_GEMM, s, 2.0 * (double)M * (double)out.n_valid * ksum);
diff --git a/mlx8-ws-audio-transformer_amd/csrc/logmel.hip b/mlx8-ws-audio-transformer_amd/csrc/logmel.hip
--- a/mlx8-ws-audio-transformer_amd/csrc/logmel.hip
+++ b/mlx8-ws-audio-transformer_amd/csrc/logmel.hip
@@ -312,6 +312,15 @@
 
 }
 
+int conv_stem_positions(int n_ctx, int max_valid) {
+  if (n_ctx <= 0) return 0;
+  const int n_fft = 400, hop = 160, T = 2 * n_ctx;
+  const int64_t L = (int64_t)T * hop;
+  const int live = host_live_frames((int)(max_valid < L ? max_valid : L), n_fft, hop, T);
+  const int Sc = (live + 3) / 2 + 2;
+  return Sc < n_ctx ? Sc : n_ctx;
+}
+
 size_t awt_logmel_workspace_bytes(int B) { return (((size_t)(B > 0 ? B : 1) * sizeof(unsigned)) + 255) & ~(size_t)255; }
 
 int logmel_prepare_impl(awt_ctx* c, int n_fft, int n_mels, double f_min, double f_max, int sample_rate, int slaney) {
```

Result: faster. 1405 clips/s, median of 6 (+1.4%).
